# sujeetv/parquet-go

Hardware: AMD Instinct MI355X
Metric: decoded GB/s (uncompressed output) per GPU & node at 1/2/4/8; % HBM roofline (higher is better)
Workload: dtype int32; 1 GPU; C2: optional INT32, 100000000 rows x 7 dictionary widths (b=1,2,4,8,12,16,20), ~10% nulls, RLE_DICTIONARY (uniform indices), V1, UNCOMPRESSED, 20000 rows/page; bytes_in=821696760, bytes_out=3220121800, streams=2, parallelism=single GPU

## Files before the change

### parquet-go_amd/csrc/pqg_common.h

```cpp
#pragma once
#include <stdint.h>

#ifndef __HIPCC__
#ifndef __host__
#define __host__
#define __device__
#define __forceinline__ inline
#endif
#endif

namespace pqg {

enum : int32_t {
  kOK = 0,
  kEOF = -1,
  kTHRIFT = -2,
  kPAGE_HEADER = -3,
  kSIZE = -4,
  kSNAPPY = -5,
  kRLE = -6,
  kDICT_INDEX = -7,
  kBIT_WIDTH = -8,
  kDELTA = -9,
  kUNSUPPORTED = -10,
  kDICT_PAGE = -11,
  kBYTE_ARRAY = -12,
  kLEVELS = -13,
  kFIXED_LEN = -14,
  kGZIP = -15,
  kCAPACITY = -20,
  kCOMPLEX = -30,
};

struct PageHdr {
  int32_t type, usize, csize;
  int32_t num_values, encoding, def_enc, rep_enc;
  int32_t v2_def_len, v2_rep_len;
  int32_t has_dph, has_dict, has_v2;
  int32_t hlen;
};

struct PageDev {
  int64_t header_offset;
  int64_t payload_offset;
  int64_t slot_offset;
  int64_t value_offset;
  int64_t scratch_offset;
  const uint8_t* block;
  int64_t block_len;
  const uint8_t* rep;  int64_t rep_n;
  const uint8_t* def;  int64_t def_n;
  const uint8_t* val;  int64_t val_n;
  int32_t page_type, encoding, num_values, csize, usize;
  int32_t def_len, rep_len, def_enc, rep_enc;
  int32_t job;
  int32_t read_status;
  int32_t decode_status;
  int32_t not_null;
  int32_t flags;
  int32_t dict_width;
  int32_t hs_rep, hs_def, hs_val;
  int32_t vmode;
  int64_t run_off, blk_off;
  int64_t chars;
  int64_t char_offset;
  int64_t cstart;
  int32_t sn_hdr, sn_nsub, sn_sub_base, sn_nseg, sn_seg_base, sn_fallback;
  int64_t gz_len;
};
constexpr int32_t kPageBareBlock = 1 << 4;
constexpr int32_t kPageInflateRedo = 1 << 6;
constexpr int32_t kCodecSnappy = 1, kCodecGzip = 2;

constexpr int kSnapSub = 65536;
constexpr int kSnapSeg = 4096;
struct SnapSub {
  int32_t page;
  int32_t j;
  int32_t pos;
  int32_t out;
};

struct HStream {
  const uint8_t* p;
  int64_t n;
  int64_t run_base;
  int64_t blk_base;
  int32_t page;
  int32_t kind;
  int32_t w;
  int32_t count;
  int32_t n_runs;
  int32_t produced;
  int32_t status;
  int32_t n_blocks;
};

struct BlockDesc {
  uint32_t v0;
  uint32_t r0;
  uint32_t lo;
  uint16_t nbytes;
  uint16_t nr;
};

struct RunEnt {
  uint32_t start;
  uint32_t src;
};
constexpr uint32_t kRunBP = 0x80000000u;
constexpr int kHBlock = 512;
constexpr int kHBlockRuns = 64;
constexpr int kHBlockBytes = 1008;

struct VRec {
  uint8_t* out;
  const uint8_t* p;
  const RunEnt* runs;
  const BlockDesc* blks;
  const uint8_t* dict;
  int32_t n;
  int32_t w;
  int32_t nn;
  int32_t count;
  int32_t n_blocks;
  int32_t dcount;
  int32_t job;
  int32_t pidx;
  int32_t serr;
  int32_t produced;
};

struct JobDev {
  const uint8_t* data;
  int64_t data_len, tcs, data_page_offset;
  int32_t type, type_length, max_def, max_rep, codec, has_dict_off;
  int32_t value_width;
  int32_t page_cap;
  int64_t page_base;
  int64_t slot_cap, slot_base;
  int64_t value_cap, value_base;
  int64_t scratch_cap, scratch_base;
  int64_t offs_cap, offs_base;
  int32_t num_pages;
  int32_t dict_page;
  int32_t scan_status;
  int32_t status;
  int32_t error_page;
  int32_t n_out_pages;
  int64_t num_slots, num_values, values_bytes;
  int64_t need_scratch;
  const uint8_t* dict_data;
  int64_t dict_count, dict_len;
  const int64_t* dict_offs;
  int32_t flags;
  int32_t no_prewalk;
  int64_t doffs_cap, doffs_base;
  int64_t need_doffs;
  int64_t tile_base;
  int32_t n_tiles;
  int32_t scan_fallback;
  int32_t n_cands;
  int32_t n_ok;
  int32_t brk;
  int32_t first_dict;
  int64_t run_cap, run_base;
  int64_t blk_cap, blk_base;
  int64_t run_used, blk_used;
  int64_t item_base;
  int32_t n_items, pad2;
};

constexpr int kSplitMin = 65536;
constexpr int kPart = 4096;
constexpr int kLongLev = 32768;
constexpr int kLevPiece = 16384;
constexpr int kLongWalk = 16384;
constexpr int kCtrItems = 48;
constexpr int kCtrLongLev = 49;
constexpr int kCtrLevPieces = 50;
constexpr int kCtrLongWalk = 51;
constexpr int kCtrPartsCap = 52;

struct PartRec {
  int32_t pidx;
  int32_t p, np;
  uint32_t v0;
  int32_t b0;
  int32_t vmode;
  int64_t chars;
  int64_t cstart;
  int64_t prel;
};

struct LongLev {
  uint8_t* out;
  const uint8_t* p;
  const uint8_t* end;
  uint32_t count;
  uint32_t value;
  int32_t w;
  int32_t maxl;
  int32_t pidx;
  int32_t pad;
};
struct LevPiece {
  int32_t run;
  uint32_t v0, v1;
};

struct LongWalk {
  int64_t blk;
  uint32_t v0;
  uint32_t take;
  uint32_t run;
  uint32_t src;
  int32_t w, K;
};

#ifndef PQG_WALK_THREADS
#define PQG_WALK_THREADS 64
#endif
constexpr int kWalkThreads = PQG_WALK_THREADS;
#ifndef PQG_PW_THREADS
#define PQG_PW_THREADS 256
#endif
constexpr int kPwThreads = PQG_PW_THREADS;

constexpr int kQShards = 8;
constexpr int kQStride = 32;
constexpr int kQueueInts = kQShards * kQStride;
constexpr int kModePresentOff = 1024 + 9 * kQueueInts;
constexpr int kQueueSnapSerial = 10;
constexpr int kQueueStrDelta = 11;
constexpr int kQueueStrDba = 12;
constexpr int kQueueLevLong = 13;
constexpr int kQueueInflate = 14;
constexpr int kQueueLevGen = 15;
constexpr int kQueueDictBig = 16;
constexpr int kQueueInflateRedo = 17;
constexpr int kQueueSlots = 18;
constexpr int kPresentBigDict = 8;

constexpr int kScanTile = 16384;
constexpr int kPrewalkPages = 4;
constexpr int kCandPerTile = 64;

struct Cand {
  int64_t pos, next, payload;
  int64_t comp;
  int32_t type, encoding, num_values, csize, usize;
  int32_t def_len, rep_len, def_enc, rep_enc;
  int32_t status;
};

}
```

### parquet-go_amd/csrc/pqg_levels.hip

```cpp
#include <hip/hip_runtime.h>

#include "pqg_common.h"
#include "pqg_device.h"
#include "pqg_hybrid.h"
#include "pqg_levdec.h"
#include "pqg_lev1.h"
#include <type_traits>

namespace pqg {

#ifndef PQG_LEVELS_WPE
#define PQG_LEVELS_WPE 6
#endif

#ifdef PQG_PROFILE
int prof_read_levels(unsigned long long* out) {
  unsigned long long z[64] = {0};
  if (hipMemcpyFromSymbol(out, HIP_SYMBOL(pqg_prof), sizeof(z)) != hipSuccess) return -1;
  hipMemcpyToSymbol(HIP_SYMBOL(pqg_prof), z, sizeof(z));
  return 0;
}
#endif


#ifndef PQG_LANE_WIN
#define PQG_LANE_WIN 8
#endif
constexpr int kLaneWinG = PQG_LANE_WIN;
struct LaneWin {
  gcu8 p;
  uint32_t n;
  uint32_t base;
  PQG_L uint32_t* r;
  __device__ __forceinline__ void fill(uint32_t pos) {
    const uint32_t mis = (uint32_t)((uintptr_t)(p + pos) & 15);
    base = pos - mis;
    const uintptr_t a0 = (uintptr_t)(p + pos) - mis;
    const uintptr_t last = ((uintptr_t)(p + n) - 1) & ~(uintptr_t)15;
    uint4 g[kLaneWinG];
#pragma unroll
    for (int k = 0; k < kLaneWinG; k++) {
      const uintptr_t a = a0 + 16 * k;
      g[k] = ldg16(a <= last ? a : last);
    }
#pragma unroll
    for (int k = 0; k < kLaneWinG; k++) {
      const uint4 v = mask_tail(g[k], (int64_t)pos - mis + 16 * k, n);
      r[64 * (4 * k + 0)] = v.x;
      r[64 * (4 * k + 1)] = v.y;
      r[64 * (4 * k + 2)] = v.z;
      r[64 * (4 * k + 3)] = v.w;
    }
  }
  __device__ __forceinline__ void ensure(uint32_t pos) {
    if (pos - base > 16 * kLaneWinG - 16) fill(pos);
  }
  __device__ __forceinline__ void read12(uint32_t pos, uint32_t& a, uint32_t& b, uint32_t& c) const {
    const uint32_t off = pos - base;
    const uint32_t d = off >> 2, sh = (off & 3) * 8;
    const uint32_t x0 = r[64 * d], x1 = r[64 * (d + 1)], x2 = r[64 * (d + 2)], x3 = r[64 * (d + 3)];
    a = __builtin_amdgcn_alignbit(x1, x0, sh);
    b = __builtin_amdgcn_alignbit(x2, x1, sh);
    c = __builtin_amdgcn_alignbit(x3, x2, sh);
  }
  __device__ __forceinline__ void peek12(uint32_t pos, uint32_t& a, uint32_t& b, uint32_t& c) {
    ensure(pos);
    read12(pos, a, b, c);
  }
};

__device__ __forceinline__ void sync_ensure(LaneWin& w, bool reads, uint32_t rp) {
  const bool need = reads && rp - w.base > 16 * kLaneWinG - 16;
  if (__ballot(need) != 0 && reads) w.fill(rp);
}

__global__ void __launch_bounds__(kWalkThreads) k_hybrid_walk(const PageDev* pages, const int* list, const int* total,
                                                              HStream* streams, RunEnt* runs, BlockDesc* blks,
                                                              LongWalk* longs, int long_cap) {
  static_assert(kWalkThreads == 64, "LaneWin: dword k of lane L at buf[64 k + L]");
  __shared__ uint32_t buf[4 * kLaneWinG * kWalkThreads];
  const int nt = *total;
  int* const n_long = const_cast<int*>(total) + kCtrLongWalk;
  for (int g = blockIdx.x * kWalkThreads + threadIdx.x; g < nt; g += gridDim.x * kWalkThreads) {
    const PageDev& pg = pages[list[g]];
    const int hs = pg.hs_val;
    if (hs < 0) continue;
    HStream& S = streams[hs];
    const uint32_t w = (uint32_t)S.w;
    const uint32_t n = (uint32_t)S.n, count = (uint32_t)S.count;
    const uint32_t rb = (w + 7) >> 3;
    const uint64_t vmask = rb >= 4 ? 0xffffffffull : ((1ull << (8 * rb)) - 1);
    PQG_G uint32_t* R = (PQG_G uint32_t*)(gmut(runs) + S.run_base);
    PQG_G uint32_t* B = (PQG_G uint32_t*)(gmut(blks) + S.blk_base);
    LaneWin rd{gconst(S.p), n, 0xfffffff0u, lds_ptr(buf) + threadIdx.x};
    if (n > 0) rd.fill(0);
    uint32_t pos = 0, produced = 0, nr = 0;
    int status = kOK;
    uint32_t nb = 0, bv0 = 0, br0 = 0, bn = 0;
    uint64_t blo = ~0ull, bhi = 0;
    auto close_block = [&]() {
      if (bn == 0) return;
      const uint32_t lo = blo == ~0ull ? 0u : (uint32_t)blo;
      const uint32_t nbytes = blo == ~0ull ? 0u : (uint32_t)(bhi - blo);
      PQG_G uint32_t* d = B + 4 * nb;
      stg16((uintptr_t)d, make_uint4(bv0, br0, lo, (nbytes & 0xffff) | (bn << 16)));
      nb++;
    };
    while (produced < count) {
      if (pos >= n) { status = kEOF; break; }
      sync_ensure(rd, true, pos);
      uint32_t xa, xb, xc;
      rd.read12(pos, xa, xb, xc);
      uint64_t x = (uint64_t)xa | (uint64_t)xb << 32;
      uint32_t h, hl;
      if ((x & 0x80) == 0) {
        h = (uint32_t)x & 0x7f;
        hl = 1;
      } else {
        uint64_t v = 0;
        unsigned sft = 0;
        int e = kOK;
        hl = 0;
        for (uint32_t i = 0;; i++) {
          if (pos + i >= n) { e = kEOF; break; }
          uint32_t b;
          if (i < 8) {
            b = (uint32_t)(x >> (8 * i)) & 0xff;
          } else {
            uint32_t ya, yb, yc;
            rd.peek12(pos + i, ya, yb, yc);
            b = ya & 0xff;
          }
          if (b < 0x80) {
            if (i > 9 || (i == 9 && b > 1)) e = kRLE;
            else {
              v |= sft < 64 ? (uint64_t)b << sft : 0;
              if (v > 0x7fffffffull) e = kRLE;
            }
            hl = i + 1;
            break;
          }
          if (sft < 64) v |= (uint64_t)(b & 0x7f) << sft;
          sft += 7;
        }
        if (e) { status = e; break; }
        h = (uint32_t)v;
        {
          uint32_t ya, yb, yc;
          rd.peek12(pos + hl, ya, yb, yc);
          x = ((uint64_t)ya | (uint64_t)yb << 32) << 8;
        }
      }
      pos += hl;
      uint32_t take, st, src;
      const uint32_t left = count - produced;
      if (h & 1) {
        const uint32_t groups = h >> 1;
        if (groups == 0) { status = kRLE; break; }
        take = groups >= (left + 7) >> 3 ? left : groups * 8;
        const uint32_t need = (take + 7) >> 3;
        if ((uint64_t)pos + (uint64_t)(need - 1) * w >= n) {
          const uint32_t ok = pos < n ? (n - pos + w - 1) / w : 0;
          take = ok * 8;
          status = kEOF;
        }
        st = produced | kRunBP;
        src = pos;
        pos = (uint64_t)pos + (uint64_t)groups * w > 0xffffffffull ? 0xffffffffu : pos + groups * w;
      } else {
        const uint32_t cnt = h >> 1;
        if (cnt == 0) { status = kRLE; break; }
        if (pos >= n || n - pos < rb) { status = kEOF; break; }
        src = (uint32_t)((x >> 8) & vmask);
        pos += rb;
        if (w < 32 && (src >> w) != 0) { status = kRLE; break; }
        take = cnt < left ? cnt : left;
        st = produced;
      }
      if (take > 0) {
        stg8((uintptr_t)(R + 2 * nr), st, src);
        const uint32_t rend = produced + take;
        if ((st & kRunBP) && take > (uint32_t)kLongWalk) {
          const uint32_t K = min((uint32_t)kHBlock, ((8u * kHBlockBytes - 14u) / w) & ~7u);
          const uint32_t R = (take + K - 1) / K;
          const int li = atomicAdd(n_long, 1);
          if (li < long_cap) {
            close_block();
            LongWalk L;
            L.blk = S.blk_base + nb;
            L.v0 = produced;
            L.take = take;
            L.run = nr;
            L.src = src;
            L.w = (int32_t)w;
            L.K = (int32_t)K;
            longs[li] = L;
            nb += R;
            bv0 = rend;
            br0 = nr + 1;
            bn = 0;
            blo = ~0ull;
            bhi = 0;
            produced = rend;
            nr++;
            if (status) break;
            continue;
          }
        }
        for (uint32_t v = produced; v < rend;) {
          if (bn == kHBlockRuns || v >= bv0 + kHBlock) {
            close_block();
            bv0 = v;
            br0 = nr;
            bn = 0;
            blo = ~0ull;
            bhi = 0;
          }
          uint32_t pe = rend < bv0 + kHBlock ? rend : bv0 + kHBlock;
          if (st & kRunBP) {
            const uint64_t rbit = (uint64_t)src * 8;
            const uint64_t b0 = (rbit + (uint64_t)(v - produced) * w) >> 3;
            const uint64_t org = blo < b0 ? blo : b0;
            const uint64_t lim = (org + kHBlockBytes) * 8;
            const uint64_t fit = lim > rbit ? (lim - rbit) / w : 0;
            if (produced + fit <= v) {
              close_block();
              bv0 = v;
              br0 = nr;
              bn = 0;
              blo = ~0ull;
              bhi = 0;
              continue;
            }
            if (produced + fit < pe) pe = (uint32_t)(produced + fit);
            const uint64_t b1 = (rbit + (uint64_t)(pe - produced) * w + 7) >> 3;
            blo = org;
            bhi = b1 > bhi ? b1 : bhi;
          }
          bn++;
          v = pe;
        }
        produced = rend;
        nr++;
      }
      if (status) break;
    }
    close_block();
    S.n_runs = (int32_t)nr;
    S.produced = (int32_t)produced;
    S.status = status;
    S.n_blocks = (int32_t)nb;
  }
}

__global__ void __launch_bounds__(256) k_walk_long(const int* ctr, const LongWalk* longs, int long_cap,
                                                   BlockDesc* blks) {
  const int n = min(ctr[kCtrLongWalk], long_cap);
  const uint32_t tid = blockIdx.x * 256 + threadIdx.x, stride = gridDim.x * 256;
  for (int r = 0; r < n; r++) {
    const LongWalk L = longs[r];
    const uint32_t R = (L.take + (uint32_t)L.K - 1) / (uint32_t)L.K;
    for (uint32_t j = tid; j < R; j += stride) {
      const uint32_t a = j * (uint32_t)L.K;
      const uint32_t cnt = min((uint32_t)L.K, L.take - a);
      const uint64_t bit0 = (uint64_t)L.src * 8 + (uint64_t)a * (uint32_t)L.w;
      const uint64_t lo = bit0 >> 3, hi = (bit0 + (uint64_t)cnt * (uint32_t)L.w + 7) >> 3;
      stg16((uintptr_t)(blks + L.blk + j),
            make_uint4(L.v0 + a, L.run, (uint32_t)lo, (uint32_t)(hi - lo) | (1u << 16)));
    }
  }
}

__global__ void __launch_bounds__(64) k_level_long(PageDev* pages, const int* ctr, const LongLev* longs, int long_cap,
                                                   const LevPiece* pieces, int piece_cap, int* queue) {
  const int lane = lane_id();
  const int np = min(ctr[kCtrLevPieces], piece_cap);
  for (;;) {
    const int t = queue_next(queue);
    if (t >= np) return;
    const LevPiece pc = pieces[t];
    if (pc.run < 0 || pc.run >= long_cap) continue;
    const LongLev L = longs[pc.run];
    if (pages[L.pidx].decode_status != kOK) continue;
    const uintptr_t ob = (uintptr_t)L.out;
    const uint32_t mask = (1u << L.w) - 1;
    const int64_t navail = L.p ? (int64_t)(L.end - L.p) : 0;
    uint32_t nn = 0;
    const uintptr_t a0 = (ob + pc.v0) & ~(uintptr_t)15;
    for (uintptr_t a = a0 + 16 * (uintptr_t)lane; a < ob + pc.v1; a += 1024) {
      const int64_t i0 = (int64_t)(a - ob);
      uint32_t v[16];
      if (L.p) {
        const int64_t ib = i0 < 0 ? 0 : i0;
        const int64_t bit = ib * L.w;
        const gcu8 p = gconst(L.p);
        const uint64_t x0 = load_u64_masked(p, navail, bit >> 3, navail);
        const uint64_t x1 = load_u64_masked(p, navail, (bit >> 3) + 8, navail);
        const uint32_t sh = (uint32_t)(bit & 7);
        const int64_t shift0 = (i0 < 0 ? -i0 : 0) * L.w;
#pragma unroll
        for (int k = 0; k < 16; k++) {
          const int64_t b = (int64_t)sh + (int64_t)k * L.w - shift0;
          uint32_t x = 0;
          if (b >= 0) {
            x = b < 64 ? (uint32_t)(x0 >> b) | (b > 56 ? (uint32_t)(x1 << (64 - b)) : 0u) : (uint32_t)(x1 >> (b - 64));
          }
          v[k] = x & mask;
        }
      } else {
#pragma unroll
        for (int k = 0; k < 16; k++) v[k] = L.value;
      }
      uint32_t wv[4];
#pragma unroll
      for (int k = 0; k < 4; k++) wv[k] = v[4 * k] | v[4 * k + 1] << 8 | v[4 * k + 2] << 16 | v[4 * k + 3] << 24;
      if (i0 >= (int64_t)pc.v0 && i0 + 16 <= (int64_t)pc.v1) {
        stg16o(a, make_uint4(wv[0], wv[1], wv[2], wv[3]));
#pragma unroll
        for (int k = 0; k < 16; k++) nn += v[k] == (uint32_t)L.maxl;
      } else {
#pragma unroll
        for (int k = 0; k < 16; k++) {
          if (i0 + k >= (int64_t)pc.v0 && i0 + k < (int64_t)pc.v1) {
            *(PQG_G uint8_t*)(a + k) = (uint8_t)v[k];
            nn += v[k] == (uint32_t)L.maxl;
          }
        }
      }
    }
    const int64_t tot = wave_sum((int64_t)nn);
    if (lane == 0 && L.maxl <= 255 && tot) atomicAdd(&pages[L.pidx].not_null, (int32_t)tot);
  }
}

__device__ __forceinline__ bool w1_job(const JobDev& job) { return job.max_rep == 0 && job.max_def <= 1; }

union LevW1Shared {
  LevShared lev;
  Lev1Shared l1;
};
template <bool kW1>
using LevelsShared = typename std::conditional<kW1, LevW1Shared, LevShared>::type;
__device__ __forceinline__ LevShared& lev_sh(LevShared& s) { return s; }
__device__ __forceinline__ LevShared& lev_sh(LevW1Shared& s) { return s.lev; }

template <bool kW1>
__device__ __forceinline__ void page_levels(JobDev* jobs, PageDev* pages, const int* list, const int* total, int* queue,
                                            uint8_t* scratch, HStream* streams, uint8_t* def_arena, uint8_t* rep_arena,
                                            LongLev* longs, int long_cap, LevPiece* pieces, int piece_cap, int split_flags) {
  __shared__ __attribute__((aligned(16))) LevelsShared<kW1> shu;
  LevShared& sh = lev_sh(shu);
  const int split = split_flags & 1;
  const bool whole = kW1 && (split_flags & 2);
  const int lane = lane_id();
  const LongTables lt{longs, pieces, const_cast<int*>(total), long_cap, piece_cap};
  for (;;) {
    const int t = queue_next(queue);
    if (t >= *total) return;
    const int pidx = __builtin_amdgcn_readfirstlane(list[t]);
    const PageDev pg = pages[pidx];
    const JobDev job = jobs[pg.job];
    if (split && w1_job(job) != kW1) continue;
    if (lane == 0) {
      pages[pidx].hs_rep = pages[pidx].hs_def = pages[pidx].hs_val = -1;
      pages[pidx].vmode = -1;
    }
    if (pg.read_status != kOK || (pg.page_type != 0 && pg.page_type != 3)) continue;
    if (job.status == kCAPACITY) continue;
    const PageStreams ps = page_setup(job, pg, pidx, pages, streams, total, scratch, lane == 0);
    if (ps.e != kOK) continue;
    const int64_t n = pg.num_values;
    int64_t nn = 0;
    int de = kOK;
    if (n > 0) {
      if (!kW1 && job.max_rep > 0) {
        if (ps.rep_n < 0) de = kLEVELS;
        else {
          uint32_t unused;
          de = level_stream<kW1>(ps.rep, ps.rep_n, bits_len((uint32_t)job.max_rep), (uint32_t)n,
                                 gmut(rep_arena) + job.slot_base + pg.slot_offset, 0x100u, sh, &unused, lt, pidx);
        }
      }
      if (de == kOK) {
        if (job.max_def > 0) {
          if (ps.def_n < 0) de = kLEVELS;
          else {
            uint32_t c = 0;
            bool done = false;
            if constexpr (kW1) {
              if (whole && job.max_def == 1 && ps.def_n <= kL1MaxN)
                done = lev1_page(ps.def, (uint32_t)ps.def_n, (uint32_t)n,
                                 gmut(def_arena) + job.slot_base + pg.slot_offset, shu.l1, &c);
            }
            if (done) de = kOK;
            else
              de = level_stream<kW1>(ps.def, ps.def_n, bits_len((uint32_t)job.max_def), (uint32_t)n,
                                     gmut(def_arena) + job.slot_base + pg.slot_offset, (uint32_t)job.max_def, sh, &c,
                                     lt, pidx);
            nn = c;
          }
        } else {
          nn = n;
        }
      }
    }
    if (lane == 0) {
      pages[pidx].not_null = de == kOK ? (int32_t)nn : 0;
      if (de != kOK) pages[pidx].decode_status = de;
    }
  }
}

__global__ void __launch_bounds__(64, PQG_LEVELS_WPE) k_page_levels(JobDev* jobs, PageDev* pages, const int* list, const int* total,
                                                    int* queue, uint8_t* scratch, HStream* streams,
                                                    uint8_t* def_arena, uint8_t* rep_arena, LongLev* longs,
                                                    int long_cap, LevPiece* pieces, int piece_cap, int split) {
  page_levels<false>(jobs, pages, list, total, queue, scratch, streams, def_arena, rep_arena, longs, long_cap, pieces,
                     piece_cap, split);
}

#ifndef PQG_LEVELS_W1_WPE
#define PQG_LEVELS_W1_WPE 4
#endif
__global__ void __launch_bounds__(64, PQG_LEVELS_W1_WPE) k_page_levels_w1(JobDev* jobs, PageDev* pages, const int* list,
                                                       const int* total, int* queue, uint8_t* scratch,
                                                       HStream* streams, uint8_t* def_arena, uint8_t* rep_arena,
                                                       LongLev* longs, int long_cap, LevPiece* pieces, int piece_cap,
                                                       int split) {
  page_levels<true>(jobs, pages, list, total, queue, scratch, streams, def_arena, rep_arena, longs, long_cap, pieces,
                    piece_cap, split);
}

__device__ void plan_parts(JobDev& job, int np, bool fail, const PageDev* pp, const HStream* streams,
                           const BlockDesc* blks, int* ctr, PartRec* parts, int64_t cap, int64_t* part);

__device__ void resolve_dictionary(JobDev& job, PageDev* pages, uint8_t* scratch) {
  int np = job.num_pages < job.page_cap ? job.num_pages : job.page_cap;
  if (job.status == kCAPACITY) np = 0;
  if (job.dict_page < 0 || job.dict_page >= np) return;
  PageDev& dp = pages[job.page_base + job.dict_page];
  if (dp.read_status != kOK) return;
  const uint8_t* blk =
      dp.scratch_offset >= 0 ? scratch + job.scratch_base + dp.scratch_offset : job.data + dp.payload_offset;
  const int64_t blen = dp.usize;
  const int64_t cnt = dp.num_values;
  const int w = job.value_width;
  dp.block = blk;
  dp.block_len = blen;
  int st = kOK;
  int flags = 0;
  if (w > 0) {
    if (job.type == 3) {
      const int64_t full = blen / 12, rem = blen % 12;
      if (cnt > full + (rem > 0 ? 1 : 0)) st = kEOF;
      else if (cnt == full + 1 && rem > 0) flags = 1;
    } else if (cnt * w > blen) {
      st = kEOF;
    }
  } else {
    flags = 2;
    job.need_doffs = (cnt < blen / 4 ? cnt : blen / 4) + 2;
    if (job.need_doffs > job.doffs_cap) job.status = kCAPACITY;
  }
  if (st == kOK) {
    job.flags |= flags;
    job.dict_data = blk;
    job.dict_count = (flags & 2) ? 0 : cnt;
    job.dict_len = blen;
  } else {
    dp.read_status = st;
  }
}

__global__ void __launch_bounds__(256) k_dict_resolve(JobDev* jobs, int n_jobs, PageDev* pages, uint8_t* scratch) {
  const int j = blockIdx.x * 256 + threadIdx.x;
  if (j < n_jobs) resolve_dictionary(jobs[j], pages, scratch);
}

__device__ int nn_job_tail(JobDev& job, PageDev* pages, uint8_t* scratch, int np, int64_t carry, bool fail0) {
  int cap = fail0 || job.status == kCAPACITY;
  job.num_values = carry;
  const int64_t vb = job.value_width > 0 ? carry * job.value_width : 0;
  if (job.value_width > 0 && vb > job.value_cap) job.status = kCAPACITY, cap = 1;
  job.values_bytes = vb;
  return cap;
}

__device__ int64_t part_n(const PageDev& pg, const HStream* streams, int64_t* count, bool* hyb);
__device__ void plan_split_pages(JobDev& job, const PageDev* pp, const HStream* streams, const BlockDesc* blks,
                                 PartRec* parts, int64_t base, int nbig, const int* big, const int64_t* boff);
__device__ void plan_parts_from(JobDev& job, int np, const PageDev* pp, const HStream* streams, const BlockDesc* blks,
                                PartRec* parts, int64_t base);

constexpr int kNnFastSeg = 12;

__global__ void __launch_bounds__(1024) k_nn_scan(JobDev* jobs, PageDev* pages, uint8_t* scratch,
                                                  const HStream* streams, const BlockDesc* blks, int* ctr,
                                                  PartRec* parts, int64_t parts_cap) {
  __shared__ int64_t part[17];
  __shared__ int s_cap;
  JobDev& job = jobs[blockIdx.x];
  int np = job.num_pages < job.page_cap ? job.num_pages : job.page_cap;
  if (job.status == kCAPACITY) np = 0;
  if (np <= kNnFastSeg * 1024) {
    __shared__ int64_t s_base, s_res;
    __shared__ int s_big[256];
    __shared__ int64_t s_boff[256];
    __shared__ int s_nbig;
    const int seg = (np + 1023) / 1024;
    const int s0 = (int)threadIdx.x * seg;
    PageDev* pp = pages + job.page_base;
    int32_t nnv[kNnFastSeg], kv[kNnFastSeg];
    int8_t vm[kNnFastSeg];
    int64_t nsum = 0, ksum = 0;
    int32_t f_type[kNnFastSeg], f_nn[kNnFastSeg], f_rs[kNnFastSeg], f_ds[kNnFastSeg], f_enc[kNnFastSeg];
#pragma unroll
    for (int j = 0; j < kNnFastSeg; j++) {
      const int i = np > 0 ? (s0 + j < np ? s0 + j : np - 1) : 0;
      const PageDev& pg = pp[i];
      f_type[j] = pg.page_type;
      f_nn[j] = pg.not_null;
      f_rs[j] = pg.read_status;
      f_ds[j] = pg.decode_status;
      f_enc[j] = pg.encoding;
      vm[j] = (int8_t)pg.vmode;
    }
#pragma unroll
    for (int j = 0; j < kNnFastSeg; j++) {
      nnv[j] = kv[j] = 0;
      if (j < seg && s0 + j < np) {
        const bool data = f_type[j] == 0 || f_type[j] == 3;
        nnv[j] = data ? f_nn[j] : 0;
        int32_t k = 0;
        if (!data || vm[j] < 0) k = 0;
        else if (f_rs[j] != kOK || f_ds[j] != kOK || vm[j] == 3) k = 1;
        else if (vm[j] == 2 && f_enc[j] != 0 && f_enc[j] != 8) k = 1;
        else if (f_nn[j] <= kSplitMin) k = 1;
        else {
          int64_t c;
          bool h;
          k = (int32_t)part_n(pp[s0 + j], streams, &c, &h);
        }
        kv[j] = k;
      }
      nsum += nnv[j];
      ksum += kv[j];
    }
    int64_t carry, ktot;
    int64_t run = block_excl_scan<1024>(nsum, &carry, part);
    int64_t koff = block_excl_scan<1024>(ksum, &ktot, part);
    const bool fail0 = job.status == kCAPACITY;
    if (threadIdx.x == 0) {
      int cap = nn_job_tail(job, pages, scratch, np, carry, fail0);
      int64_t base = 0;
      if (!cap) {
        base = atomicAdd(ctr + kCtrItems, (int)ktot);
        if (base + ktot > parts_cap) {
          job.status = kCAPACITY;
          cap = 1;
        }
      }
      job.item_base = base;
      job.n_items = cap ? 0 : (int32_t)ktot;
      s_base = base;
      s_cap = cap;
      s_nbig = 0;
      s_res = fail0 ? 0 : ktot;
      if (blockIdx.x == 0) ctr[kCtrPartsCap] = (int)(parts_cap < INT32_MAX ? parts_cap : INT32_MAX);
    }
    __syncthreads();
    if (s_cap) {
      for (int64_t k = s_base + threadIdx.x; k < s_base + s_res && k < parts_cap; k += 1024) parts[k].vmode = -1;
    }
#pragma unroll
    for (int j = 0; j < kNnFastSeg; j++)
      if (j < seg && s0 + j < np) {
        pp[s0 + j].value_offset = run;
        run += nnv[j];
      }
    if (s_cap) return;
    const int64_t base = s_base;
    bool more = false;
#pragma unroll
    for (int j = 0; j < kNnFastSeg; j++) {
      if (j < seg && s0 + j < np) {
        if (kv[j] == 1) {
          PartRec r;
          r.pidx = (int32_t)(job.page_base + s0 + j);
          r.p = 0;
          r.np = 1;
          r.v0 = 0;
          r.b0 = 0;
          r.vmode = vm[j];
          r.chars = r.cstart = r.prel = 0;
          parts[base + koff] = r;
        } else if (kv[j] > 1) {
          const int slot = atomicAdd(&s_nbig, 1);
          if (slot < 256) {
            s_big[slot] = s0 + j;
            s_boff[slot] = koff;
          } else {
            more = true;
          }
        }
        koff += kv[j];
      }
    }
    const bool any_more = __syncthreads_or(more);
    const int nbig = s_nbig < 256 ? s_nbig : 256;
    if (!any_more) {
      plan_split_pages(job, pp, streams, blks, parts, base, nbig, s_big, s_boff);
      return;
    }
    __syncthreads();
    plan_parts_from(job, np, pp, streams, blks, parts, base);
    return;
  }
  const int seg = (np + 1023) / 1024;
  const int s0 = (int)threadIdx.x * seg, s1 = s0 + seg < np ? s0 + seg : np;
  PageDev* pp = pages + job.page_base;
  auto nn_of = [&](int i) -> int64_t {
    const PageDev& pg = pp[i];
    return (pg.page_type == 0 || pg.page_type == 3) ? (int64_t)pg.not_null : 0;
  };
  int64_t sum = 0;
#pragma unroll 8
  for (int i = s0; i < s1; i++) sum += nn_of(i);
  int64_t carry;
  int64_t run = block_excl_scan<1024>(sum, &carry, part);
#pragma unroll 8
  for (int i = s0; i < s1; i++) {
    pp[i].value_offset = run;
    run += nn_of(i);
  }
  const bool fail0 = job.status == kCAPACITY;
  if (threadIdx.x == 0) s_cap = nn_job_tail(job, pages, scratch, np, carry, fail0);
  __syncthreads();
  plan_parts(job, np, s_cap != 0, pp, streams, blks, ctr, parts, parts_cap, part);
}

}

namespace pqg {

__device__ __forceinline__ int64_t part_count(const PageDev& pg, const HStream* streams, bool* hyb) {
  *hyb = false;
  if ((pg.page_type != 0 && pg.page_type != 3) || pg.vmode < 0) return -1;
  if (pg.read_status != kOK || pg.decode_status != kOK || pg.vmode == 3) return 0;
  const int enc = pg.encoding;
  if (pg.vmode == 2 && enc != 0 && enc != 8) return 0;
  const int64_t nn = pg.not_null;
  if (enc == 0 || nn <= kSplitMin) return nn;
  if ((enc == 8 || enc == 3) && pg.hs_val >= 0) {
    const HStream& S = streams[pg.hs_val];
    *hyb = true;
    return nn < S.produced ? nn : S.produced;
  }
  return 0;
}

__device__ int64_t part_n(const PageDev& pg, const HStream* streams, int64_t* count, bool* hyb) {
  const int64_t c = part_count(pg, streams, hyb);
  *count = c;
  if (c < 0) return 0;
  return c > kSplitMin ? (c + kPart - 1) / kPart : 1;
}

__device__ void plan_split_pages(JobDev& job, const PageDev* pp, const HStream* streams, const BlockDesc* blks,
                                 PartRec* parts, int64_t base, int nbig, const int* big, const int64_t* boff) {
  for (int q = 0; q < nbig; q++) {
    const int pi = big[q];
    const int64_t poff = boff[q];
    int64_t cnt;
    bool hyb;
    const PageDev& pg = pp[pi];
    const int64_t P = part_n(pg, streams, &cnt, &hyb);
    PartRec r;
    r.pidx = (int32_t)(job.page_base + pi);
    r.np = (int32_t)P;
    r.vmode = pg.vmode;
    r.chars = r.cstart = r.prel = 0;
    if (!hyb) {
      for (int64_t p = threadIdx.x; p < P; p += blockDim.x) {
        r.p = (int32_t)p;
        r.v0 = (uint32_t)(p * kPart);
        r.b0 = 0;
        parts[base + poff + p] = r;
      }
    } else {
      const HStream& S = streams[pg.hs_val];
      const BlockDesc* B = blks + S.blk_base;
      const int nb = S.n_blocks;
      auto f = [&](int bi) -> int64_t {
        if (bi < 0) return -1;
        if (bi >= nb || (int64_t)B[bi].v0 >= cnt) return P;
        return (int64_t)B[bi].v0 / kPart;
      };
      for (int bi = threadIdx.x; bi <= nb; bi += blockDim.x) {
        const int64_t f1 = f(bi), f0 = f(bi - 1);
        for (int64_t p = f0 + 1; p <= f1 && p < P; p++) {
          r.p = (int32_t)p;
          r.v0 = p == 0 ? 0u : (bi < nb && (int64_t)B[bi].v0 < cnt ? B[bi].v0 : (uint32_t)cnt);
          r.b0 = bi;
          parts[base + poff + p] = r;
        }
      }
    }
  }
}

constexpr int kBigList = 256;
__device__ void plan_parts_from(JobDev& job, int np, const PageDev* pp, const HStream* streams, const BlockDesc* blks,
                                PartRec* parts, int64_t base) {
  __shared__ int64_t part2[17];
  __shared__ int s_big[kBigList];
  __shared__ int64_t s_boff[kBigList];
  __shared__ int s_nbig;
  const int seg = (np + 1023) / 1024;
  const int s0 = (int)threadIdx.x * seg, s1 = s0 + seg < np ? s0 + seg : np;
  int64_t sum = 0;
  for (int i = s0; i < s1; i++) {
    int64_t c;
    bool h;
    sum += part_n(pp[i], streams, &c, &h);
  }
  int64_t tot;
  int64_t off = block_excl_scan<1024>(sum, &tot, part2);
  int cur = s0;
  for (;;) {
    if (threadIdx.x == 0) s_nbig = 0;
    __syncthreads();
    for (; cur < s1; cur++) {
      int64_t c;
      bool h;
      const int64_t k = part_n(pp[cur], streams, &c, &h);
      if (k == 1) {
        PartRec r;
        r.pidx = (int32_t)(job.page_base + cur);
        r.p = 0;
        r.np = 1;
        r.v0 = 0;
        r.b0 = 0;
        r.vmode = pp[cur].vmode;
        r.chars = r.cstart = r.prel = 0;
        parts[base + off] = r;
      } else if (k > 1) {
        const int slot = atomicAdd(&s_nbig, 1);
        if (slot >= kBigList) break;
        s_big[slot] = cur;
        s_boff[slot] = off;
      }
      off += k;
    }
    __syncthreads();
    plan_split_pages(job, pp, streams, blks, parts, base, s_nbig < kBigList ? s_nbig : kBigList, s_big, s_boff);
    if (!__syncthreads_or(cur < s1)) break;
  }
}

__device__ void plan_parts(JobDev& job, int np, bool fail, const PageDev* pp, const HStream* streams,
                           const BlockDesc* blks, int* ctr, PartRec* parts, int64_t cap, int64_t* part) {
  __shared__ int64_t s_base;
  __shared__ int s_fail;
  if (fail) np = 0;
  const int seg = (np + 1023) / 1024;
  const int s0 = (int)threadIdx.x * seg, s1 = s0 + seg < np ? s0 + seg : np;
  int64_t sum = 0;
  for (int i = s0; i < s1; i++) {
    int64_t c;
    bool h;
    sum += part_n(pp[i], streams, &c, &h);
  }
  int64_t tot;
  block_excl_scan<1024>(sum, &tot, part);
  if (threadIdx.x == 0) {
    const int64_t base = fail ? 0 : atomicAdd(ctr + kCtrItems, (int)tot);
    s_fail = fail || base + tot > cap;
    if (!fail && s_fail) job.status = kCAPACITY;
    job.item_base = base;
    job.n_items = s_fail ? 0 : (int32_t)tot;
    s_base = base;
    if (blockIdx.x == 0) ctr[kCtrPartsCap] = (int)(cap < INT32_MAX ? cap : INT32_MAX);
  }
  __syncthreads();
  if (s_fail) {
    if (!fail)
      for (int64_t k = s_base + threadIdx.x; k < s_base + tot && k < cap; k += 1024) parts[k].vmode = -1;
    return;
  }
  plan_parts_from(job, np, pp, streams, blks, parts, s_base);
}

}
```

### parquet-go_amd/csrc/pqg_runtime.hip

```cpp
#include <hip/hip_runtime.h>
#include <cstdlib>

#include <algorithm>
#include <cstdio>
#include <map>
#include <cstring>
#include <mutex>
#include <vector>

#include "../../include/pqgpu.h"
#include "pqg_common.h"

namespace pqg {
int assemble_launch(hipStream_t s, const pqg_assemble_args* a, int64_t* seg_scratch, int64_t* tot);
int list_count_launch(hipStream_t s, const pqg_list_args* a, int64_t* seg_scratch, int64_t* tot);
int list_write_launch(hipStream_t s, const pqg_list_args* a, int64_t* seg_scratch);
int pack_levels_launch(hipStream_t s, const uint8_t* levels, int64_t n, int bw, uint8_t* packed);
}

namespace pqg {
__global__ void k_tile_jobs(const JobDev* jobs, int* tile_job);
__global__ void k_page_cands(JobDev* jobs, const int* tile_job, int* tile_count, int* tile_okc, int64_t* cand_pos,
                             int* cand_list, int* cand_total, int region);
__global__ void k_cand_parse(JobDev* jobs, const int* tile_job, const int* cand_list, const int* cand_total, int region,
                             int* tile_okc,
                             const int64_t* cand_pos, Cand* cands);
__global__ void k_tile_scan(JobDev* jobs, const int* tile_count, const int* tile_okc, int* tile_off, int* tile_okoff);
__global__ void k_cand_link(JobDev* jobs, const int* tile_job, int64_t total_tiles, const int* tile_count,
                            const int* tile_off, const int* tile_okoff, const Cand* cands, int* succ, int* idx2slot,
                            int* ok2slot);
__global__ void k_page_chain(JobDev* jobs, PageDev* pages, const Cand* cands, const int* succ,
                             const int* idx2slot, const int* ok2slot, int* order);
__global__ void k_scan_pages(JobDev* jobs, PageDev* pages, int n_jobs, int prewalk, int stride);
__global__ void k_page_list(JobDev* jobs, PageDev* pages, int n_jobs, int* list, int list_cap, int* total,
                            int* queues);
__global__ void k_snappy(JobDev* jobs, PageDev* pages, const int* list, const int* total, int* queue,
                         uint8_t* scratch);
__global__ void k_inflate(JobDev* jobs, PageDev* pages, const int* list, const int* total, int* queue,
                          uint8_t* scratch, int mode);
__global__ void k_inflate_s(JobDev* jobs, PageDev* pages, const int* list, const int* total, int* queue,
                            uint8_t* scratch);
__global__ void k_snap_plan(const JobDev* jobs, PageDev* pages, const int* list, const int* total, int* ctr,
                            SnapSub* subs, int sub_cap, int* seg_page, int seg_cap);
__global__ void k_snap_seg(const JobDev* jobs, const PageDev* pages, const int* seg_page, const int* seg_total,
                           int seg_cap, uint2* F);
__global__ void k_snap_link(const JobDev* jobs, PageDev* pages, const int* list, const int* total, SnapSub* subs,
                            const uint2* F);
__global__ void k_snap_decode(const JobDev* jobs, PageDev* pages, const SnapSub* subs, const int* sub_total,
                              int sub_cap, int* queue, uint8_t* scratch);
__global__ void k_page_levels(JobDev* jobs, PageDev* pages, const int* list, const int* total, int* queue,
                              uint8_t* scratch, HStream* streams, uint8_t* def_arena, uint8_t* rep_arena,
                              LongLev* longs, int long_cap, LevPiece* pieces, int piece_cap, int split);
__global__ void k_page_levels_w1(JobDev* jobs, PageDev* pages, const int* list, const int* total, int* queue,
                              uint8_t* scratch, HStream* streams, uint8_t* def_arena, uint8_t* rep_arena,
                              LongLev* longs, int long_cap, LevPiece* pieces, int piece_cap, int split);
__global__ void k_dict_resolve(JobDev* jobs, int n_jobs, PageDev* pages, uint8_t* scratch);
__global__ void k_level_long(PageDev* pages, const int* ctr, const LongLev* longs, int long_cap,
                             const LevPiece* pieces, int piece_cap, int* queue);
__global__ void k_hybrid_walk(const PageDev* pages, const int* list, const int* total, HStream* streams,
                              RunEnt* runs, BlockDesc* blks, LongWalk* longs, int long_cap);
__global__ void k_walk_long(const int* ctr, const LongWalk* longs, int long_cap, BlockDesc* blks);
__global__ void k_nn_scan(JobDev* jobs, PageDev* pages, uint8_t* scratch, const HStream* streams, const BlockDesc* blks,
                          int* ctr, PartRec* parts, int64_t parts_cap);
template <int Mode>
__global__ void k_values(JobDev* jobs, PageDev* pages, const PartRec* parts, const int* total, int* queue,
                         uint8_t* value_arena, const HStream* streams, const RunEnt* runs, const BlockDesc* blks);
__global__ void k_dict_plan(JobDev* jobs, PageDev* pages, const PartRec* parts, const int* total,
                            uint8_t* value_arena, const HStream* streams, const RunEnt* runs, const BlockDesc* blks,
                            VRec* recs);
__global__ void k_dict4(PageDev* pages, const int* total, int* queue, const VRec* recs, int big);
__global__ void k_dict4_big(PageDev* pages, const int* total, int* queue, const VRec* recs);
constexpr int kBigDictThreads = 512;
__global__ void k_finalize(JobDev* jobs, int n_jobs, PageDev* pages);
__global__ void k_str_dict(JobDev* jobs, PageDev* pages, int64_t* doffs_arena);
__global__ void k_str_count(JobDev* jobs, PageDev* pages, PartRec* parts, const int* total, int* queue,
                            int64_t* offs_arena, const HStream* streams, const RunEnt* runs, const BlockDesc* blks);
__global__ void k_str_plain(JobDev* jobs, PageDev* pages, const int* list, const int* total, int* queue,
                            int64_t* offs_arena);
__global__ void k_char_scan(JobDev* jobs, PageDev* pages, PartRec* parts, int64_t* offs_arena);
__global__ void k_str_delta(JobDev* jobs, PageDev* pages, const int* list, const int* total, int* queue,
                            int64_t* offs_arena);
__global__ void k_str_dba(JobDev* jobs, PageDev* pages, const int* list, const int* total, int* queue,
                          uint8_t* value_arena, int64_t* offs_arena);
__global__ void k_str_copy(JobDev* jobs, PageDev* pages, const PartRec* parts, const int* total, int* queue,
                           uint8_t* value_arena, int64_t* offs_arena);
}

#ifdef PQG_PROFILE
namespace pqg {
int prof_read_values(unsigned long long* out);
int prof_read_levels(unsigned long long* out);
int prof_read_strings(unsigned long long* out);
int prof_read_snappy(unsigned long long* out);
int prof_read_dict(unsigned long long* out);
int prof_read_inflate(unsigned long long* out);
}
#endif

using namespace pqg;

namespace {

struct DevBuf {
  void* p = nullptr;
  size_t cap = 0;
  int grow(size_t bytes) {
    if (bytes <= cap) return 0;
    if (p) hipFree(p);
    p = nullptr;
    cap = 0;
    size_t want = std::max(bytes, (size_t)256);
    want = (want + 0xFFFFF) & ~(size_t)0xFFFFF;
    if (hipMalloc(&p, want) != hipSuccess) {
      p = nullptr;
      return -1;
    }
    cap = want;
    return 0;
  }
  void release() {
    if (p) hipFree(p);
    p = nullptr;
    cap = 0;
  }
};

constexpr int kStages = 10;
constexpr int kWalkLanes = kWalkThreads;
constexpr int kMaxAttempts = 6;

struct Caps {
  int64_t pages = 0, slots = 0, scratch = 0, values = 0, runs = 0, blks = 0, doffs = 0;
};
struct JobKey {
  uintptr_t data;
  int64_t tcs, hint;
  bool operator<(const JobKey& o) const {
    return data != o.data ? data < o.data : tcs != o.tcs ? tcs < o.tcs : hint < o.hint;
  }
};

int64_t align_up(int64_t v, int64_t a) { return (v + a - 1) / a * a; }

unsigned qgrid(int64_t blocks) { return (unsigned)std::max<int64_t>(blocks, kQShards); }

int value_width_of(const pqg_column_desc& c) {
  switch (c.physical_type) {
    case PQG_BOOLEAN: return 1;
    case PQG_INT32: case PQG_FLOAT: return 4;
    case PQG_INT64: case PQG_DOUBLE: return 8;
    case PQG_INT96: return 12;
    case PQG_FIXED_LEN_BYTE_ARRAY: return c.type_length > 0 ? c.type_length : 0;
  }
  return 0;
}

}

struct pqg_ctx {
  int device = 0;
  hipStream_t stream = nullptr;
  int num_cus = 256;
  DevBuf vrecs;
  int dict4_per_cu = 2;
  int dict4_threads = 256;
  bool dict4 = true;
  bool stride = true;
  bool dict_big = true;
  bool lev1 = true;
  int seg_waves = 31;
  int levlong_waves = 28;
  int link_waves = 16;
  int snappy_per_cu = 2;
  int inflate_per_cu = 8;
  DevBuf jobs, pages, list, counters, def_arena, rep_arena, value_arena, scratch;
  DevBuf tile_job;
  DevBuf tile_count, tile_okc, tile_off, tile_okoff, cand_pos, cands, succ, idx2slot, ok2slot, order;
  DevBuf streams, runs, blks;
  DevBuf cand_list, vlists;
  DevBuf asm_seg;
  DevBuf offs_arena, doffs_arena;
  DevBuf page_stage;
  DevBuf blk_src, blk_dst, blk_meta, blk_subs, blk_segpage, blk_F;
  DevBuf sn_subs, sn_segpage, sn_F;
  int64_t sn_sub_cap = 0, sn_seg_cap = 0;
  DevBuf parts, lev_long, lev_pieces, walk_long;
  int64_t parts_cap = 0, lev_long_cap = 0, lev_piece_cap = 0, walk_long_cap = 0;
  int64_t total_tiles = 0;
  JobDev* h_jobs = nullptr;
  int h_jobs_cap = 0;
  std::vector<pqg_chunk_job> cur;
  std::vector<JobDev> plan;
  std::vector<Caps> force;
  std::map<JobKey, Caps> learned;
  std::map<JobKey, bool> many_pages;
  bool prewalk = true;
  int launches = 0;
  bool any_var = false;
  bool any_fixed_other = false;
  bool any_w4 = false;
  bool any_levels = false;
  int n_jobs = 0;
  int64_t list_cap = 0;
  hipEvent_t ev[kStages + 1];
  hipEvent_t ev_k8[4];
  float k8_ms = 0.f;
  bool timed = true;
  bool last_timed = false;
};

static int hip_ok(hipError_t e) { return e == hipSuccess ? PQG_OK : PQG_ERR_HIP; }

extern "C" {

const char* pqg_status_string(int s) {
  switch (s) {
    case PQG_OK: return "ok";
    case PQG_ERR_EOF: return "unexpected end of stream";
    case PQG_ERR_THRIFT: return "page header: thrift decode failed";
    case PQG_ERR_PAGE_HEADER: return "page header: missing or negative field";
    case PQG_ERR_SIZE: return "page size mismatch";
    case PQG_ERR_SNAPPY: return "snappy: corrupt input";
    case PQG_ERR_RLE: return "rle: invalid run";
    case PQG_ERR_DICT_INDEX: return "dict: invalid index";
    case PQG_ERR_BIT_WIDTH: return "invalid bit width";
    case PQG_ERR_DELTA: return "delta: invalid stream";
    case PQG_ERR_UNSUPPORTED: return "unsupported encoding/codec/type";
    case PQG_ERR_DICT_PAGE: return "there should be only one dictionary";
    case PQG_ERR_BYTE_ARRAY: return "bytearray/plain: len is negative";
    case PQG_ERR_LEVELS: return "level reader is not initialized";
    case PQG_ERR_FIXED_LEN: return "bytearray/delta: value length is not the fixed length";
    case PQG_ERR_GZIP: return "gzip: invalid data";
    case PQG_ERR_CAPACITY: return "capacity";
    case PQG_ERR_INVALID_ARG: return "invalid argument";
    case PQG_ERR_HIP: return "HIP runtime error";
    case PQG_ERR_METADATA: return "invalid file metadata";
  }
  return "unknown";
}

int pqg_ctx_create(int device, pqg_ctx** out) {
  if (!out) return PQG_ERR_INVALID_ARG;
  *out = nullptr;
  int n = 0;
  if (hipGetDeviceCount(&n) != hipSuccess || device < 0 || device >= n) return PQG_ERR_HIP;
  if (hipSetDevice(device) != hipSuccess) return PQG_ERR_HIP;
  pqg_ctx* c = new pqg_ctx();
  c->device = device;
  hipDeviceProp_t prop;
  if (hipGetDeviceProperties(&prop, device) == hipSuccess) c->num_cus = prop.multiProcessorCount;
  if (hipStreamCreateWithFlags(&c->stream, hipStreamNonBlocking) != hipSuccess) {
    delete c;
    return PQG_ERR_HIP;
  }
  for (auto& e : c->ev) hipEventCreate(&e);
  for (auto& e : c->ev_k8) hipEventCreate(&e);
  if (const char* e = getenv("PQG_DICT4")) c->dict4 = atoi(e) != 0;
  if (const char* e = getenv("PQG_DICT_BIG")) c->dict_big = atoi(e) != 0;
  if (const char* e = getenv("PQG_STRIDE")) c->stride = atoi(e) != 0;
  if (const char* e = getenv("PQG_LEV1")) c->lev1 = atoi(e) != 0;
  if (const char* e = getenv("PQG_SEG_WAVES")) c->seg_waves = atoi(e) > 0 ? atoi(e) : c->seg_waves;
  if (const char* e = getenv("PQG_LEVLONG_WAVES")) c->levlong_waves = atoi(e) > 0 ? atoi(e) : c->levlong_waves;
  if (const char* e = getenv("PQG_LINK_WAVES")) c->link_waves = atoi(e) > 0 ? atoi(e) : c->link_waves;
  {
    hipFuncAttributes fa;
    if (hipFuncGetAttributes(&fa, reinterpret_cast<const void*>(&k_dict4)) == hipSuccess && fa.maxThreadsPerBlock > 0)
      c->dict4_threads = fa.maxThreadsPerBlock;
    int o = 0;
    if (hipOccupancyMaxActiveBlocksPerMultiprocessor(&o, reinterpret_cast<const void*>(&k_dict4), c->dict4_threads, 0) ==
            hipSuccess && o > 0)
      c->dict4_per_cu = o;
  }
  int occ = 0;
  if (hipOccupancyMaxActiveBlocksPerMultiprocessor(&occ, reinterpret_cast<const void*>(&k_snappy), 64, 0) ==
          hipSuccess &&
      occ > 0)
    c->snappy_per_cu = occ;
  occ = 0;
  if (hipOccupancyMaxActiveBlocksPerMultiprocessor(&occ, reinterpret_cast<const void*>(&k_inflate_s), 64, 0) ==
          hipSuccess && occ > 0)
    c->inflate_per_cu = occ;
  if (c->counters.grow(sizeof(int) * (size_t)(1024 + kQueueSlots * kQueueInts))) {
    pqg_ctx_destroy(c);
    return PQG_ERR_HIP;
  }
  *out = c;
  return PQG_OK;
}

void pqg_ctx_destroy(pqg_ctx* c) {
  if (!c) return;
  hipSetDevice(c->device);
  hipStreamSynchronize(c->stream);
  for (auto& e : c->ev) hipEventDestroy(e);
  for (auto& e : c->ev_k8) hipEventDestroy(e);
  for (DevBuf* b : {&c->jobs, &c->pages, &c->list, &c->counters, &c->def_arena, &c->rep_arena, &c->value_arena,
                    &c->scratch, &c->streams, &c->runs, &c->blks, &c->cand_list, &c->vlists, &c->tile_count, &c->tile_okc, &c->tile_off, &c->tile_okoff, &c->cand_pos, &c->cands, &c->succ, &c->idx2slot,
                    &c->ok2slot, &c->order, &c->asm_seg, &c->offs_arena, &c->doffs_arena, &c->page_stage,
                    &c->blk_src, &c->blk_dst, &c->blk_meta, &c->tile_job, &c->sn_subs, &c->sn_segpage, &c->sn_F,
                    &c->blk_subs, &c->blk_segpage, &c->blk_F, &c->vrecs, &c->parts, &c->lev_long, &c->lev_pieces,
                    &c->walk_long})
    b->release();
  if (c->h_jobs) hipHostFree(c->h_jobs);
  hipStreamDestroy(c->stream);
  delete c;
}

int pqg_device_alloc(pqg_ctx* c, int64_t bytes, void** dptr) {
  if (!c || !dptr) return PQG_ERR_INVALID_ARG;
  hipSetDevice(c->device);
  return hip_ok(hipMalloc(dptr, (size_t)std::max<int64_t>(bytes, 1)));
}
int pqg_device_free(pqg_ctx* c, void* dptr) {
  if (!c) return PQG_ERR_INVALID_ARG;
  hipSetDevice(c->device);
  return hip_ok(hipFree(dptr));
}
int pqg_memcpy_h2d(pqg_ctx* c, void* dst, const void* src, int64_t bytes) {
  if (!c) return PQG_ERR_INVALID_ARG;
  hipSetDevice(c->device);
  int e = hip_ok(hipMemcpyAsync(dst, src, (size_t)bytes, hipMemcpyHostToDevice, c->stream));
  if (e) return e;
  return hip_ok(hipStreamSynchronize(c->stream));
}
int pqg_memcpy_d2h(pqg_ctx* c, void* dst, const void* src, int64_t bytes) {
  if (!c) return PQG_ERR_INVALID_ARG;
  hipSetDevice(c->device);
  int e = hip_ok(hipMemcpyAsync(dst, src, (size_t)bytes, hipMemcpyDeviceToHost, c->stream));
  if (e) return e;
  return hip_ok(hipStreamSynchronize(c->stream));
}

static int plan_batch(pqg_ctx* c) {
  const int n = c->n_jobs;
  if (c->h_jobs_cap < n) {
    if (c->h_jobs) hipHostFree(c->h_jobs);
    c->h_jobs_cap = std::max(n, 64);
    if (hipHostMalloc((void**)&c->h_jobs, sizeof(JobDev) * (size_t)c->h_jobs_cap) != hipSuccess) return PQG_ERR_HIP;
  }
  int64_t page_total = 0, slot_total = 0, value_total = 0, scratch_total = 0, tile_total = 0, run_total = 0,
          blk_total = 0, offs_total = 0, doffs_total = 0, seg_total = 0;
  c->plan.resize((size_t)n);
  for (int i = 0; i < n; i++) {
    const pqg_chunk_job& in = c->cur[(size_t)i];
    const Caps& f = c->force[(size_t)i];
    JobDev d;
    memset(&d, 0, sizeof(d));
    d.data = in.data;
    d.data_len = in.data_len;
    d.tcs = in.total_compressed_size;
    d.data_page_offset = in.data_page_offset;
    d.type = in.col.physical_type;
    d.type_length = in.col.type_length;
    d.max_def = in.col.max_def;
    d.max_rep = in.col.max_rep;
    d.codec = in.col.codec;
    d.has_dict_off = in.has_dict_page_offset;
    d.value_width = value_width_of(in.col);
    d.no_prewalk = c->many_pages.count(JobKey{(uintptr_t)in.data, in.total_compressed_size, in.num_values_hint}) ? 1 : 0;
    int64_t pcap = in.total_compressed_size / 256 + 16;
    if (f.pages > 0) pcap = f.pages;
    pcap = std::min<int64_t>(pcap, (int64_t)1 << 30);
    d.page_cap = (int32_t)pcap;
    d.page_base = page_total;
    page_total += pcap;
    int64_t scap = std::max<int64_t>(in.num_values_hint, 0) + 64;
    if (f.slots > 0) scap = f.slots;
    d.slot_cap = scap;
    d.slot_base = slot_total;
    slot_total += align_up(scap, 256);
    int64_t vcap = d.value_width > 0 ? scap * d.value_width
                                     : std::max<int64_t>(in.total_uncompressed_size, in.total_compressed_size) + 1024;
    if (f.values > 0) vcap = f.values;
    d.value_cap = vcap;
    d.value_base = value_total;
    value_total += align_up(vcap, 256);
    int64_t xcap = 0;
    if (in.col.codec != PQG_CODEC_UNCOMPRESSED)
      xcap = std::max<int64_t>(in.total_uncompressed_size, in.total_compressed_size) + pcap * 16 + 1024;
    if (f.scratch > 0) xcap = f.scratch;
    d.scratch_cap = xcap;
    d.scratch_base = scratch_total;
    scratch_total += align_up(xcap, 256);
    if (in.col.codec != PQG_CODEC_UNCOMPRESSED) seg_total += in.total_compressed_size / kSnapSeg + pcap;
    d.dict_page = -1;
    d.error_page = -1;
    const int64_t lim = std::max<int64_t>(0, std::min(in.total_compressed_size, in.data_len));
    int64_t rcap = (in.total_compressed_size + xcap) / 2 + 6 * pcap + 64;
    if (f.runs > 0) rcap = f.runs;
    d.run_cap = rcap;
    d.run_base = run_total;
    run_total += rcap;
    int64_t bcap = 3 * (scap / kHBlock + 3 * pcap) + rcap / kHBlockRuns + 2 * rcap / (kHBlockBytes / 2) + 64;
    if (f.blks > 0) bcap = f.blks;
    d.blk_cap = bcap;
    d.blk_base = blk_total;
    blk_total += bcap;
    if (d.value_width == 0 || d.type == PQG_FIXED_LEN_BYTE_ARRAY) {
      d.offs_cap = scap + 1;
      d.offs_base = offs_total;
      offs_total += align_up(scap + 1, 32);
    }
    if (d.value_width == 0) {
      int64_t dcap = std::min<int64_t>(std::max<int64_t>(in.total_uncompressed_size, 0) / 4, 1 << 17) + 64;
      if (f.doffs > 0) dcap = f.doffs;
      d.doffs_cap = dcap;
      d.doffs_base = doffs_total;
      doffs_total += align_up(dcap, 32);
    }
    d.tile_base = tile_total;
    d.n_tiles = (int32_t)((lim + kScanTile - 1) / kScanTile);
    tile_total += d.n_tiles;
    c->plan[(size_t)i] = d;
    c->h_jobs[i] = d;
  }
  c->list_cap = page_total;
  c->parts_cap = page_total + slot_total / kPart + n + 64;
  c->lev_long_cap = 2 * slot_total / kLongLev + 64;
  c->lev_piece_cap = 2 * slot_total / kLevPiece + 2 * c->lev_long_cap + 64;
  c->walk_long_cap = slot_total / kLongWalk + 64;
  if (c->parts.grow(sizeof(PartRec) * (size_t)c->parts_cap) || c->lev_long.grow(sizeof(LongLev) * (size_t)c->lev_long_cap) ||
      c->lev_pieces.grow(sizeof(LevPiece) * (size_t)c->lev_piece_cap) ||
      c->walk_long.grow(sizeof(LongWalk) * (size_t)c->walk_long_cap))
    return PQG_ERR_HIP;
  c->sn_sub_cap = scratch_total / kSnapSub + page_total + 64;
  c->sn_seg_cap = seg_total + 64;
  if (c->sn_subs.grow(sizeof(SnapSub) * (size_t)c->sn_sub_cap) || c->sn_segpage.grow(sizeof(int) * (size_t)c->sn_seg_cap) ||
      c->sn_F.grow(sizeof(uint2) * 64 * (size_t)c->sn_seg_cap))
    return PQG_ERR_HIP;
  if (c->jobs.grow(sizeof(JobDev) * (size_t)n) || c->pages.grow(sizeof(PageDev) * (size_t)page_total) ||
      c->list.grow(sizeof(int) * (size_t)std::max<int64_t>(page_total, 1)) || c->def_arena.grow((size_t)slot_total + 64) ||
      c->rep_arena.grow((size_t)slot_total + 64) || c->value_arena.grow((size_t)value_total + 64) ||
      c->scratch.grow((size_t)scratch_total + 64) || c->tile_count.grow(sizeof(int) * (size_t)tile_total + 64) ||
      c->tile_off.grow(sizeof(int) * (size_t)tile_total + 64) || c->tile_okc.grow(sizeof(int) * (size_t)tile_total + 64) ||
      c->tile_okoff.grow(sizeof(int) * (size_t)tile_total + 64) || c->tile_job.grow(sizeof(int) * (size_t)tile_total + 64) ||
      c->ok2slot.grow(sizeof(int) * (size_t)tile_total * kCandPerTile + 64) ||
      c->cand_pos.grow(sizeof(int64_t) * (size_t)tile_total * kCandPerTile + 64) ||
      c->cand_list.grow(sizeof(int) * (size_t)(tile_total + kQShards) * kCandPerTile + 64) ||
      c->vlists.grow(sizeof(int) * 3 * (size_t)page_total + 64) ||
      c->cands.grow(sizeof(Cand) * (size_t)tile_total * kCandPerTile + 64) ||
      c->succ.grow(sizeof(int) * (size_t)tile_total * kCandPerTile + 64) ||
      c->idx2slot.grow(sizeof(int) * (size_t)tile_total * kCandPerTile + 64) ||
      c->order.grow(sizeof(int) * (size_t)page_total + 64) ||
      c->streams.grow(sizeof(HStream) * 3 * (size_t)page_total + 64) ||
      c->runs.grow(sizeof(RunEnt) * (size_t)run_total + 8192) || c->blks.grow(sizeof(BlockDesc) * (size_t)blk_total + 8192) ||
      c->vrecs.grow(sizeof(VRec) * (size_t)std::max<int64_t>(c->parts_cap, 1)) ||
      c->offs_arena.grow(sizeof(int64_t) * (size_t)offs_total + 64) ||
      c->doffs_arena.grow(sizeof(int64_t) * (size_t)doffs_total + 64))
    return PQG_ERR_HIP;
  c->total_tiles = tile_total;
  return hip_ok(hipMemcpyAsync(c->jobs.p, c->h_jobs, sizeof(JobDev) * (size_t)n, hipMemcpyHostToDevice, c->stream));
}

struct SnapTables {
  SnapSub* subs;
  int sub_cap;
  int* segpage;
  int seg_cap;
  uint2* F;
};
static void launch_snappy(pqg_ctx* c, hipStream_t s, JobDev* jobs, PageDev* pages, const int* list, const int* total,
                          int64_t list_cap, int* sctr, int* q_split, int* q_serial, uint8_t* scratch,
                          const SnapTables& T) {
  const int waves = c->num_cus * c->snappy_per_cu;
  hipMemsetAsync(sctr, 0, 2 * sizeof(int), s);
  hipLaunchKernelGGL(k_snap_plan, dim3((unsigned)std::max<int64_t>(1, std::min<int64_t>((list_cap + 255) / 256, c->num_cus * 4))),
                     dim3(256), 0, s, jobs, pages, list, total, sctr, T.subs, T.sub_cap, T.segpage, T.seg_cap);
  hipLaunchKernelGGL(k_snap_seg, dim3(c->num_cus * c->seg_waves), dim3(64), 0, s, jobs, pages, T.segpage, sctr + 1, T.seg_cap, T.F);
  hipLaunchKernelGGL(k_snap_link, dim3(c->num_cus * c->link_waves), dim3(64), 0, s, jobs, pages, list, total, T.subs, T.F);
  hipLaunchKernelGGL(k_snap_decode, dim3(qgrid(waves)), dim3(64), 0, s, jobs, pages, T.subs, sctr, T.sub_cap, q_split,
                     scratch);
  hipLaunchKernelGGL(k_snappy, dim3(qgrid(waves)), dim3(64), 0, s, jobs, pages, list, total, q_serial, scratch);
}

static int launch_pipeline(pqg_ctx* c) {
  const int n = c->n_jobs;
  c->launches++;
  c->last_timed = c->timed;
  JobDev* jobs = (JobDev*)c->jobs.p;
  PageDev* pages = (PageDev*)c->pages.p;
  int* list = (int*)c->list.p;
  int* ctr = (int*)c->counters.p;
  auto Q = [&](int k) { return ctr + 1024 + k * kQueueInts; };
  uint8_t* scratch = (uint8_t*)c->scratch.p;
  const int waves = c->num_cus * 20;
  hipStream_t s = c->stream;
  if (c->timed) hipEventRecord(c->ev[0], s);
  hipMemsetAsync(Q(0), 0, sizeof(int) * kQueueSlots * kQueueInts, s);
  const int64_t nt = c->total_tiles;
  int* tcount = (int*)c->tile_count.p;
  int* toff = (int*)c->tile_off.p;
  Cand* cands = (Cand*)c->cands.p;
  int* tokc = (int*)c->tile_okc.p;
  int* tokoff = (int*)c->tile_okoff.p;
  if (c->prewalk) hipLaunchKernelGGL(k_scan_pages, dim3(n), dim3(64), 0, s, jobs, pages, n, kPrewalkPages, (int)c->stride);
  if (nt > 0) {
    int64_t* cpos = (int64_t*)c->cand_pos.p;
    int* clist = (int*)c->cand_list.p;
    const int region = (int)((nt + kQShards - 1) / kQShards) * kCandPerTile;
    hipLaunchKernelGGL(k_tile_jobs, dim3(n), dim3(256), 0, s, jobs, (int*)c->tile_job.p);
    hipLaunchKernelGGL(k_page_cands, dim3((unsigned)nt), dim3(256), 0, s, jobs, (const int*)c->tile_job.p, tcount, tokc,
                       cpos, clist, Q(7),
                       region);
    hipLaunchKernelGGL(k_cand_parse, dim3((unsigned)std::min<int64_t>((nt * kCandPerTile + 255) / 256, c->num_cus * 4)),
                       dim3(256), 0, s, jobs, (const int*)c->tile_job.p, clist, Q(7), region, tokc, cpos, cands);
  }
  hipLaunchKernelGGL(k_tile_scan, dim3(n), dim3(1024), 0, s, jobs, tcount, tokc, toff, tokoff);
  if (nt > 0)
    hipLaunchKernelGGL(k_cand_link, dim3((unsigned)((nt * kCandPerTile + 255) / 256)), dim3(256), 0, s, jobs,
                       (const int*)c->tile_job.p, nt,
                       tcount, toff, tokoff, cands, (int*)c->succ.p, (int*)c->idx2slot.p, (int*)c->ok2slot.p);
  hipLaunchKernelGGL(k_page_chain, dim3(n), dim3(1024), 0, s, jobs, pages, cands, (const int*)c->succ.p,
                     (const int*)c->idx2slot.p, (const int*)c->ok2slot.p, (int*)c->order.p);
  hipLaunchKernelGGL(k_scan_pages, dim3(n), dim3(64), 0, s, jobs, pages, n, 0, 0);
  if (c->timed) hipEventRecord(c->ev[1], s);
  hipLaunchKernelGGL(k_page_list, dim3(n), dim3(1024), 0, s, jobs, pages, n, list,
                     (int)std::min<int64_t>(c->list_cap, INT32_MAX), ctr, ctr + 8);
  if (c->timed) hipEventRecord(c->ev[2], s);
  bool any_snappy = false, any_gzip = false;
  for (int i = 0; i < n; i++) {
    any_snappy |= c->cur[(size_t)i].col.codec == PQG_CODEC_SNAPPY;
    any_gzip |= c->cur[(size_t)i].col.codec == PQG_CODEC_GZIP;
  }
  if (any_snappy) {
    const SnapTables T{(SnapSub*)c->sn_subs.p, (int)std::min<int64_t>(c->sn_sub_cap, INT32_MAX), (int*)c->sn_segpage.p,
                       (int)std::min<int64_t>(c->sn_seg_cap, INT32_MAX), (uint2*)c->sn_F.p};
    launch_snappy(c, s, jobs, pages, list, ctr, c->list_cap, ctr + 32, Q(0), Q(kQueueSnapSerial), scratch, T);
  }
  if (any_gzip) {
    hipLaunchKernelGGL(k_inflate_s, dim3(qgrid(c->num_cus * c->inflate_per_cu)), dim3(64), 0, s, jobs, pages, list, ctr,
                       Q(kQueueInflate), scratch);
    hipLaunchKernelGGL(k_inflate, dim3(qgrid(c->num_cus * 4)), dim3(64), 0, s, jobs, pages, list, ctr,
                       Q(kQueueInflateRedo), scratch, 1);
  }
  if (c->timed) hipEventRecord(c->ev[3], s);
  HStream* streams = (HStream*)c->streams.p;
  RunEnt* runs = (RunEnt*)c->runs.p;
  BlockDesc* blks = (BlockDesc*)c->blks.p;
  LongLev* llong = (LongLev*)c->lev_long.p;
  LevPiece* lpieces = (LevPiece*)c->lev_pieces.p;
  const int llc = (int)std::min<int64_t>(c->lev_long_cap, INT32_MAX), lpc = (int)std::min<int64_t>(c->lev_piece_cap, INT32_MAX);
  hipLaunchKernelGGL(k_dict_resolve, dim3((unsigned)((n + 255) / 256)), dim3(256), 0, s, jobs, n, pages, scratch);
  bool any_w1 = false, any_gen = false;
  for (int i = 0; i < n; i++) {
    const pqg_column_desc& d = c->cur[(size_t)i].col;
    (d.max_rep == 0 && d.max_def <= 1 ? any_w1 : any_gen) = true;
  }
  const int split = any_w1 && any_gen;
  if (any_w1)
    hipLaunchKernelGGL(k_page_levels_w1, dim3(qgrid(c->num_cus * 32)), dim3(64), 0, s, jobs, pages, list, ctr, Q(1),
                       scratch, streams, (uint8_t*)c->def_arena.p, (uint8_t*)c->rep_arena.p, llong, llc, lpieces, lpc,
                       split | (c->lev1 ? 2 : 0));
  if (any_gen)
    hipLaunchKernelGGL(k_page_levels, dim3(qgrid(c->num_cus * 24)), dim3(64), 0, s, jobs, pages, list, ctr,
                       Q(split ? kQueueLevGen : 1), scratch, streams, (uint8_t*)c->def_arena.p,
                       (uint8_t*)c->rep_arena.p, llong, llc, lpieces, lpc, split);
  if (c->any_levels)
    hipLaunchKernelGGL(k_level_long, dim3(qgrid(c->num_cus * c->levlong_waves)), dim3(64), 0, s, pages, ctr, llong, llc, lpieces, lpc,
                       Q(kQueueLevLong));
  if (c->timed) hipEventRecord(c->ev[4], s);
  const unsigned walk_blocks = (unsigned)std::max<int64_t>(
      1, std::min<int64_t>((c->list_cap + kWalkLanes - 1) / kWalkLanes, c->num_cus * (2048 / kWalkLanes)));
  LongWalk* wlong = (LongWalk*)c->walk_long.p;
  const int wlc = (int)std::min<int64_t>(c->walk_long_cap, INT32_MAX);
  hipLaunchKernelGGL(k_hybrid_walk, dim3(walk_blocks), dim3(kWalkLanes), 0, s, pages, list, ctr, streams, runs, blks,
                     wlong, wlc);
  hipLaunchKernelGGL(k_walk_long, dim3(c->num_cus * 2), dim3(256), 0, s, ctr, wlong, wlc, blks);
  if (c->timed) hipEventRecord(c->ev[5], s);
  if (c->timed) hipEventRecord(c->ev[6], s);
  PartRec* parts = (PartRec*)c->parts.p;
  hipLaunchKernelGGL(k_nn_scan, dim3(n), dim3(1024), 0, s, jobs, pages, scratch, streams, blks, ctr, parts, c->parts_cap);
  if (c->timed) hipEventRecord(c->ev[7], s);
  const int64_t items_cap = c->parts_cap;
  if (!c->any_w4) {
  } else if (c->dict4) {
    VRec* recs = (VRec*)c->vrecs.p;
    hipLaunchKernelGGL(k_dict_plan, dim3((unsigned)std::max<int64_t>(1, std::min<int64_t>((items_cap + 255) / 256, c->num_cus * 4))),
                       dim3(256), 0, s, jobs, pages, parts, ctr, (uint8_t*)c->value_arena.p, streams, runs, blks, recs);
    hipLaunchKernelGGL(k_dict4, dim3(qgrid(c->num_cus * c->dict4_per_cu)), dim3(c->dict4_threads), 0, s, pages, ctr, Q(3),
                       recs, (int)c->dict_big);
    if (c->dict_big)
      hipLaunchKernelGGL(k_dict4_big, dim3(qgrid(c->num_cus)), dim3(kBigDictThreads), 0, s, pages, ctr,
                         Q(kQueueDictBig), recs);
  } else
    hipLaunchKernelGGL(k_values<1>, dim3(qgrid(waves)), dim3(64), 0, s, jobs, pages, parts, ctr, Q(3),
                       (uint8_t*)c->value_arena.p, streams, runs, blks);
  if (c->any_fixed_other) {
    hipLaunchKernelGGL(k_values<0>, dim3(qgrid(waves)), dim3(64), 0, s, jobs, pages, parts, ctr, Q(2),
                       (uint8_t*)c->value_arena.p, streams, runs, blks);
    hipLaunchKernelGGL(k_values<3>, dim3(qgrid(waves)), dim3(64), 0, s, jobs, pages, parts, ctr, Q(8),
                       (uint8_t*)c->value_arena.p, streams, runs, blks);
  }
  if (c->timed) hipEventRecord(c->ev[8], s);
  if (c->any_var) {
    int64_t* offs = (int64_t*)c->offs_arena.p;
    hipLaunchKernelGGL(k_str_dict, dim3(n), dim3(512), 0, s, jobs, pages, (int64_t*)c->doffs_arena.p);
    hipLaunchKernelGGL(k_str_plain, dim3(qgrid(c->num_cus * 4 * 512 / kPwThreads)), dim3(kPwThreads), 0, s, jobs, pages, list, ctr, Q(5), offs);
    hipLaunchKernelGGL(k_str_count, dim3(qgrid(waves)), dim3(64), 0, s, jobs, pages, parts, ctr, Q(4), offs, streams,
                       runs, blks);
    hipLaunchKernelGGL(k_str_delta, dim3(qgrid(c->num_cus * 8)), dim3(64), 0, s, jobs, pages, list, ctr,
                       Q(kQueueStrDelta), offs);
    hipLaunchKernelGGL(k_char_scan, dim3(n), dim3(256), 0, s, jobs, pages, parts, offs);
    hipLaunchKernelGGL(k_str_copy, dim3(qgrid(c->num_cus * 4)), dim3(512), 0, s, jobs, pages, parts, ctr, Q(6),
                       (uint8_t*)c->value_arena.p, offs);
    hipLaunchKernelGGL(k_str_dba, dim3(qgrid(c->num_cus * 6)), dim3(64), 0, s, jobs, pages, list, ctr,
                       Q(kQueueStrDba), (uint8_t*)c->value_arena.p, offs);
  }
  if (c->timed) hipEventRecord(c->ev[9], s);
  hipLaunchKernelGGL(k_finalize, dim3(n), dim3(1024), 0, s, jobs, n, pages);
  if (c->timed) hipEventRecord(c->ev[10], s);
  return hip_ok(hipGetLastError());
}

int pqg_decode_chunks_async(pqg_ctx* c, const pqg_chunk_job* jobs, int n_jobs) {
  if (!c || (!jobs && n_jobs) || n_jobs < 0) return PQG_ERR_INVALID_ARG;
  hipSetDevice(c->device);
  for (int i = 0; i < n_jobs; i++) {
    const pqg_column_desc& d = jobs[i].col;
    if (d.max_def < 0 || d.max_def > 255 || d.max_rep < 0 || d.max_rep > 255) return PQG_ERR_INVALID_ARG;
    if (jobs[i].data_len < 0 || jobs[i].total_compressed_size < 0 || (!jobs[i].data && jobs[i].data_len > 0))
      return PQG_ERR_INVALID_ARG;
    if (jobs[i].quirks != 0) return PQG_ERR_INVALID_ARG;
  }
  c->cur.assign(jobs, jobs + n_jobs);
  c->n_jobs = n_jobs;
  c->launches = 0;
  c->force.assign((size_t)n_jobs, Caps());
  c->any_var = false;
  c->any_fixed_other = false;
  c->any_w4 = false;
  c->any_levels = false;
  c->prewalk = false;
  for (int i = 0; i < n_jobs; i++) {
    const JobKey key{(uintptr_t)jobs[i].data, jobs[i].total_compressed_size, jobs[i].num_values_hint};
    auto it = c->learned.find(key);
    if (it != c->learned.end()) c->force[(size_t)i] = it->second;
    c->prewalk |= c->many_pages.find(key) == c->many_pages.end();
    c->any_var |= value_width_of(jobs[i].col) == 0 || jobs[i].col.physical_type == PQG_FIXED_LEN_BYTE_ARRAY;
    c->any_fixed_other |= value_width_of(jobs[i].col) != 0;
    c->any_w4 |= value_width_of(jobs[i].col) == 4;
    c->any_levels |= jobs[i].col.max_def > 0 || jobs[i].col.max_rep > 0;
  }
  if (n_jobs == 0) return PQG_OK;
  int e = plan_batch(c);
  if (e) return e;
  return launch_pipeline(c);
}

int pqg_sync(pqg_ctx* c, pqg_chunk_result* results, int n_jobs) {
  if (!c || n_jobs != c->n_jobs) return PQG_ERR_INVALID_ARG;
  hipSetDevice(c->device);
  const int n = c->n_jobs;
  if (n == 0) return PQG_OK;
  for (int attempt = 0;; attempt++) {
    if (hipMemcpyAsync(c->h_jobs, c->jobs.p, sizeof(JobDev) * (size_t)n, hipMemcpyDeviceToHost, c->stream) !=
            hipSuccess ||
        hipStreamSynchronize(c->stream) != hipSuccess)
      return PQG_ERR_HIP;
    bool retry = false;
    for (int i = 0; i < n; i++) {
      const JobDev& d = c->h_jobs[i];
      if (d.status != PQG_ERR_CAPACITY) continue;
      retry = true;
      Caps& f = c->force[(size_t)i];
      f.pages = std::max<int64_t>((int64_t)d.num_pages + 16, d.page_cap);
      f.slots = std::max<int64_t>(d.num_slots + 64, d.slot_cap);
      f.scratch = std::max<int64_t>(d.need_scratch + 1024, d.scratch_cap);
      if (d.value_width > 0) {
        const int64_t nv = std::max<int64_t>(d.num_values, d.num_slots);
        f.values = std::max<int64_t>(nv * d.value_width + 64, d.value_cap);
      } else {
        f.values = std::max<int64_t>(d.values_bytes + 1024, d.value_cap);
      }
      f.runs = std::max<int64_t>(d.run_used + 64, d.run_cap);
      f.blks = std::max<int64_t>(d.blk_used + 64, d.blk_cap);
      f.doffs = std::max<int64_t>(d.need_doffs + 64, d.doffs_cap);
      const pqg_chunk_job& in = c->cur[(size_t)i];
      c->learned[JobKey{(uintptr_t)in.data, in.total_compressed_size, in.num_values_hint}] = f;
    }
    if (!retry || attempt + 1 >= kMaxAttempts) break;
    int e = plan_batch(c);
    if (e) return e;
    e = launch_pipeline(c);
    if (e) return e;
  }
  for (int i = 0; i < n; i++) {
    const JobDev& d = c->h_jobs[i];
    if (d.status != PQG_ERR_CAPACITY && d.scan_fallback != 2) {
      if (c->many_pages.size() >= 65536) c->many_pages.clear();
      const pqg_chunk_job& in = c->cur[(size_t)i];
      c->many_pages[JobKey{(uintptr_t)in.data, in.total_compressed_size, in.num_values_hint}] = true;
    }
    pqg_chunk_result& r = results[i];
    memset(&r, 0, sizeof(r));
    r.status = d.status;
    r.error_page = d.error_page;
    r.num_pages = d.status == PQG_ERR_CAPACITY ? 0 : d.n_out_pages;
    r.value_width = d.value_width;
    r.col_flags = c->cur[(size_t)i].col.flags;
    r.num_slots = d.num_slots;
    r.num_values = d.num_values;
    r.values_bytes = d.values_bytes;
    r.def_levels = d.max_def > 0 ? (uint8_t*)c->def_arena.p + d.slot_base : nullptr;
    r.rep_levels = d.max_rep > 0 ? (uint8_t*)c->rep_arena.p + d.slot_base : nullptr;
    r.values = (uint8_t*)c->value_arena.p + d.value_base;
    r.offsets = d.value_width == 0 ? (int64_t*)c->offs_arena.p + d.offs_base : nullptr;
  }
  return PQG_OK;
}

int pqg_assemble(pqg_ctx* c, pqg_assemble_args* a) {
  if (!c || !a || a->num_slots < 0 || a->max_def < 0 || a->max_def > 255 || a->boundary_level < 0)
    return PQG_ERR_INVALID_ARG;
  if (a->values_spaced && (a->value_width <= 0 || (!a->values && a->num_slots > 0))) return PQG_ERR_INVALID_ARG;
  hipSetDevice(c->device);
  const int64_t nseg = (a->num_slots + 4095) / 4096;
  if (c->asm_seg.grow((size_t)(2 * nseg + 2) * sizeof(int64_t))) return PQG_ERR_HIP;
  int64_t* seg = (int64_t*)c->asm_seg.p;
  int64_t* tot = seg + 2 * nseg;
  hipEventRecord(c->ev_k8[0], c->stream);
  int e = pqg::assemble_launch(c->stream, a, seg, tot);
  if (e) return e;
  hipEventRecord(c->ev_k8[1], c->stream);
  int64_t h[2] = {0, 0};
  if (hipMemcpyAsync(h, tot, sizeof(h), hipMemcpyDeviceToHost, c->stream) != hipSuccess ||
      hipStreamSynchronize(c->stream) != hipSuccess)
    return PQG_ERR_HIP;
  hipEventElapsedTime(&c->k8_ms, c->ev_k8[0], c->ev_k8[1]);
  a->num_valid = h[0];
  a->null_count = a->num_slots - h[0];
  a->num_boundaries = h[1];
  return PQG_OK;
}

int pqg_assemble_list(pqg_ctx* c, pqg_list_args* a) {
  if (!c || !a || a->num_slots < 0 || !a->def_levels || a->max_def < 0 || a->max_def > 255 || a->value_width < 0)
    return PQG_ERR_INVALID_ARG;
  if (a->elem_values && (a->value_width <= 0 || (!a->values && a->num_slots > 0))) return PQG_ERR_INVALID_ARG;
  hipSetDevice(c->device);
  const int64_t nseg = (a->num_slots + 4095) / 4096;
  if (c->asm_seg.grow((size_t)(4 * nseg + 4) * sizeof(int64_t))) return PQG_ERR_HIP;
  int64_t* seg = (int64_t*)c->asm_seg.p;
  int64_t* tot = seg + 4 * nseg;
  hipEventRecord(c->ev_k8[0], c->stream);
  int e = pqg::list_count_launch(c->stream, a, seg, tot);
  if (e) return e;
  hipEventRecord(c->ev_k8[1], c->stream);
  int64_t h[4] = {0, 0, 0, 0};
  if (hipMemcpyAsync(h, tot, sizeof(h), hipMemcpyDeviceToHost, c->stream) != hipSuccess ||
      hipStreamSynchronize(c->stream) != hipSuccess)
    return PQG_ERR_HIP;
  a->num_rows = h[0];
  a->num_elements = h[1];
  a->num_valid = h[2];
  a->null_lists = h[3];
  if (h[1] > INT32_MAX) return PQG_ERR_INVALID_ARG;
  hipEventRecord(c->ev_k8[2], c->stream);
  e = pqg::list_write_launch(c->stream, a, seg);
  if (e) return e;
  hipEventRecord(c->ev_k8[3], c->stream);
  e = hip_ok(hipStreamSynchronize(c->stream));
  float m0 = 0.f, m1 = 0.f;
  hipEventElapsedTime(&m0, c->ev_k8[0], c->ev_k8[1]);
  hipEventElapsedTime(&m1, c->ev_k8[2], c->ev_k8[3]);
  c->k8_ms = m0 + m1;
  return e;
}

int pqg_last_assemble_ms(pqg_ctx* c, float* ms) {
  if (!c || !ms) return PQG_ERR_INVALID_ARG;
  *ms = c->k8_ms;
  return PQG_OK;
}

int pqg_decode_chunks(pqg_ctx* c, const pqg_chunk_job* jobs, int n_jobs, pqg_chunk_result* results) {
  int e = pqg_decode_chunks_async(c, jobs, n_jobs);
  if (e) return e;
  return pqg_sync(c, results, n_jobs);
}

int pqg_decode_page(pqg_ctx* c, const pqg_page_job* pj, pqg_chunk_result* result) {
  if (!c || !pj || !result || !pj->page || pj->page_len <= 0 || pj->dict_page_len < 0 ||
      (pj->dict_page_len > 0 && !pj->dict_page))
    return PQG_ERR_INVALID_ARG;
  hipSetDevice(c->device);
  const int64_t dl = pj->dict_page ? pj->dict_page_len : 0, total = dl + pj->page_len;
  if (c->page_stage.grow((size_t)total + 64)) return PQG_ERR_HIP;
  uint8_t* st = (uint8_t*)c->page_stage.p;
  if ((dl && hipMemcpyAsync(st, pj->dict_page, (size_t)dl, hipMemcpyDeviceToDevice, c->stream) != hipSuccess) ||
      hipMemcpyAsync(st + dl, pj->page, (size_t)pj->page_len, hipMemcpyDeviceToDevice, c->stream) != hipSuccess)
    return PQG_ERR_HIP;
  pqg_chunk_job job;
  memset(&job, 0, sizeof(job));
  job.col = pj->col;
  job.data = st;
  job.data_len = total;
  job.total_compressed_size = total;
  job.data_page_offset = dl;
  job.total_uncompressed_size = total;
  return pqg_decode_chunks(c, &job, 1, result);
}

static int inflate_pass(pqg_ctx* c, int64_t n, int64_t store, PageDev* out) {
  if (c->blk_dst.grow((size_t)store + 64)) return PQG_ERR_HIP;
  JobDev jd;
  memset(&jd, 0, sizeof(jd));
  jd.data = (const uint8_t*)c->blk_src.p;
  jd.data_len = n;
  jd.tcs = n;
  jd.codec = PQG_CODEC_GZIP;
  jd.scratch_cap = store + 16;
  PageDev pd;
  memset(&pd, 0, sizeof(pd));
  pd.page_type = PQG_PAGE_DICTIONARY;
  pd.flags = kPageBareBlock;
  pd.csize = (int32_t)n;
  pd.usize = (int32_t)store;
  pd.read_status = kOK;
  uint8_t* meta = (uint8_t*)c->blk_meta.p;
  JobDev* djob = (JobDev*)meta;
  PageDev* dpage = (PageDev*)(meta + sizeof(JobDev));
  int* ints = (int*)(meta + sizeof(JobDev) + sizeof(PageDev));
  int hi[2] = {0, 1};
  if (hipMemcpyAsync(djob, &jd, sizeof(jd), hipMemcpyHostToDevice, c->stream) != hipSuccess ||
      hipMemcpyAsync(dpage, &pd, sizeof(pd), hipMemcpyHostToDevice, c->stream) != hipSuccess ||
      hipMemcpyAsync(ints, hi, sizeof(hi), hipMemcpyHostToDevice, c->stream) != hipSuccess ||
      hipMemsetAsync(ints + 4, 0, sizeof(int) * kQueueInts, c->stream) != hipSuccess)
    return PQG_ERR_HIP;
  hipLaunchKernelGGL(k_inflate, dim3(qgrid(1)), dim3(64), 0, c->stream, djob, dpage, ints, ints + 1, ints + 4,
                     (uint8_t*)c->blk_dst.p, 0);
  if (hipGetLastError() != hipSuccess) return PQG_ERR_HIP;
  if (hipMemcpyAsync(out, dpage, sizeof(PageDev), hipMemcpyDeviceToHost, c->stream) != hipSuccess ||
      hipStreamSynchronize(c->stream) != hipSuccess)
    return PQG_ERR_HIP;
  return PQG_OK;
}

static int block_inflate(pqg_ctx* c, const uint8_t* src, int64_t n, uint8_t* dst, int64_t cap, int64_t* out_len) {
  constexpr int64_t kInflateFirst = 64 << 20;
  hipSetDevice(c->device);
  if (c->blk_src.grow((size_t)n + 64) ||
      c->blk_meta.grow(sizeof(JobDev) + sizeof(PageDev) + (4 + 2 * kQueueInts) * sizeof(int)))
    return PQG_ERR_HIP;
  if (n && hipMemcpyAsync(c->blk_src.p, src, (size_t)n, hipMemcpyHostToDevice, c->stream) != hipSuccess)
    return PQG_ERR_HIP;
  int64_t store = std::min<int64_t>(std::max<int64_t>(cap, 0), kInflateFirst);
  PageDev pd;
  int e = inflate_pass(c, n, store, &pd);
  if (e) return e;
  if (pd.read_status != kOK) return pd.read_status;
  *out_len = pd.gz_len;
  if (pd.gz_len > cap) return PQG_ERR_CAPACITY;
  if (pd.gz_len > INT32_MAX) return PQG_ERR_UNSUPPORTED;
  if (pd.gz_len > store) {
    store = pd.gz_len;
    e = inflate_pass(c, n, store, &pd);
    if (e) return e;
    if (pd.read_status != kOK) return pd.read_status;
    if (pd.gz_len != store) return PQG_ERR_HIP;
  }
  if (pd.gz_len && (hipMemcpyAsync(dst, c->blk_dst.p, (size_t)pd.gz_len, hipMemcpyDeviceToHost, c->stream) != hipSuccess ||
                    hipStreamSynchronize(c->stream) != hipSuccess))
    return PQG_ERR_HIP;
  return PQG_OK;
}

int pqg_block_decompress(pqg_ctx* c, int codec, const uint8_t* src, int64_t n, uint8_t* dst, int64_t cap,
                         int64_t* out_len) {
  if (!c || (!src && n > 0) || n < 0 || n > INT32_MAX || !out_len) return PQG_ERR_INVALID_ARG;
  *out_len = 0;
  if (codec == PQG_CODEC_UNCOMPRESSED) {
    *out_len = n;
    if (n > cap) return PQG_ERR_CAPACITY;
    if (n) memcpy(dst, src, (size_t)n);
    return PQG_OK;
  }
  if (codec == PQG_CODEC_GZIP) return block_inflate(c, src, n, dst, cap, out_len);
  if (codec != PQG_CODEC_SNAPPY) return PQG_ERR_UNSUPPORTED;
  uint64_t v = 0;
  int hl = 0;
  for (unsigned sft = 0;; hl++, sft += 7) {
    if (hl >= n) return PQG_ERR_SNAPPY;
    const uint8_t b = src[hl];
    if (b < 0x80) {
      if (hl > 9 || (hl == 9 && b > 1)) return PQG_ERR_SNAPPY;
      v |= sft < 64 ? (uint64_t)b << sft : 0;
      hl++;
      break;
    }
    if (sft < 64) v |= (uint64_t)(b & 0x7f) << sft;
  }
  if (v > 0xffffffffull || v > (uint64_t)INT32_MAX) return PQG_ERR_SNAPPY;
  *out_len = (int64_t)v;
  if ((int64_t)v > cap) return PQG_ERR_CAPACITY;
  hipSetDevice(c->device);
  if (c->blk_src.grow((size_t)n + 64) || c->blk_dst.grow((size_t)v + 64) ||
      c->blk_meta.grow(sizeof(JobDev) + sizeof(PageDev) + (4 + 2 * kQueueInts) * sizeof(int)))
    return PQG_ERR_HIP;
  const int64_t bsub = (int64_t)v / kSnapSub + 2, bseg = n / kSnapSeg + 2;
  if (c->blk_subs.grow(sizeof(SnapSub) * (size_t)bsub) || c->blk_segpage.grow(sizeof(int) * (size_t)bseg) ||
      c->blk_F.grow(sizeof(uint2) * 64 * (size_t)bseg))
    return PQG_ERR_HIP;
  JobDev jd;
  memset(&jd, 0, sizeof(jd));
  jd.data = (const uint8_t*)c->blk_src.p;
  jd.data_len = n;
  jd.tcs = n;
  jd.codec = PQG_CODEC_SNAPPY;
  jd.scratch_cap = (int64_t)v + 16;
  PageDev pd;
  memset(&pd, 0, sizeof(pd));
  pd.page_type = PQG_PAGE_DICTIONARY;
  pd.csize = (int32_t)n;
  pd.usize = (int32_t)v;
  pd.payload_offset = 0;
  pd.scratch_offset = 0;
  pd.read_status = kOK;
  uint8_t* meta = (uint8_t*)c->blk_meta.p;
  JobDev* djob = (JobDev*)meta;
  PageDev* dpage = (PageDev*)(meta + sizeof(JobDev));
  int* ints = (int*)(meta + sizeof(JobDev) + sizeof(PageDev));
  int hi[2] = {0, 1};
  if (hipMemcpyAsync(c->blk_src.p, src, (size_t)n, hipMemcpyHostToDevice, c->stream) != hipSuccess ||
      hipMemcpyAsync(djob, &jd, sizeof(jd), hipMemcpyHostToDevice, c->stream) != hipSuccess ||
      hipMemcpyAsync(dpage, &pd, sizeof(pd), hipMemcpyHostToDevice, c->stream) != hipSuccess ||
      hipMemcpyAsync(ints, hi, sizeof(hi), hipMemcpyHostToDevice, c->stream) != hipSuccess ||
      hipMemsetAsync(ints + 4, 0, sizeof(int) * 2 * kQueueInts, c->stream) != hipSuccess)
    return PQG_ERR_HIP;
  const SnapTables T{(SnapSub*)c->blk_subs.p, (int)bsub, (int*)c->blk_segpage.p, (int)bseg, (uint2*)c->blk_F.p};
  launch_snappy(c, c->stream, djob, dpage, ints, ints + 1, 1, ints + 2, ints + 4, ints + 4 + kQueueInts,
                (uint8_t*)c->blk_dst.p, T);
  if (hipGetLastError() != hipSuccess) return PQG_ERR_HIP;
  if (hipMemcpyAsync(&pd, dpage, sizeof(pd), hipMemcpyDeviceToHost, c->stream) != hipSuccess ||
      hipStreamSynchronize(c->stream) != hipSuccess)
    return PQG_ERR_HIP;
  if (pd.read_status != kOK) return pd.read_status;
  if (v && (hipMemcpyAsync(dst, c->blk_dst.p, (size_t)v, hipMemcpyDeviceToHost, c->stream) != hipSuccess ||
            hipStreamSynchronize(c->stream) != hipSuccess))
    return PQG_ERR_HIP;
  return PQG_OK;
}

int pqg_pack_levels(pqg_ctx* c, const uint8_t* levels, int64_t n, int max_level, uint8_t* packed) {
  if (!c || n < 0 || max_level < 0 || max_level > 255 || (n > 0 && (!levels || !packed))) return PQG_ERR_INVALID_ARG;
  hipSetDevice(c->device);
  int bw = 0;
  while ((max_level >> bw) != 0) bw++;
  int e = pqg::pack_levels_launch(c->stream, levels, n, bw, packed);
  if (e) return e;
  return hip_ok(hipStreamSynchronize(c->stream));
}

int pqg_get_pages(pqg_ctx* c, int job, pqg_page_info* out, int cap) {
  if (!c || job < 0 || job >= c->n_jobs) return PQG_ERR_INVALID_ARG;
  hipSetDevice(c->device);
  const JobDev& d = c->h_jobs[job];
  int np = std::min<int>(d.n_out_pages, d.page_cap);
  if (d.status == PQG_ERR_CAPACITY) np = 0;
  std::vector<PageDev> tmp((size_t)np);
  if (np > 0) {
    if (hipMemcpyAsync(tmp.data(), (PageDev*)c->pages.p + d.page_base, sizeof(PageDev) * (size_t)np,
                       hipMemcpyDeviceToHost, c->stream) != hipSuccess ||
        hipStreamSynchronize(c->stream) != hipSuccess)
      return PQG_ERR_HIP;
  }
  int k = 0;
  for (int i = 0; i < np && i < cap; i++, k++) {
    const PageDev& p = tmp[(size_t)i];
    pqg_page_info& o = out[i];
    memset(&o, 0, sizeof(o));
    o.header_offset = p.header_offset;
    o.payload_offset = p.payload_offset;
    o.slot_offset = p.slot_offset;
    o.value_offset = p.value_offset;
    o.page_type = p.page_type;
    o.encoding = p.encoding;
    o.num_values = p.num_values;
    o.not_null = p.not_null;
    o.compressed_size = p.csize;
    o.uncompressed_size = p.usize;
    o.def_len = p.def_len;
    o.rep_len = p.rep_len;
    o.def_encoding = p.def_enc;
    o.rep_encoding = p.rep_enc;
    o.status = p.read_status != PQG_OK ? p.read_status : p.decode_status;
    o.flags = p.flags | (p.sn_fallback ? PQG_PAGE_FLAG_SNAPPY_SERIAL | (p.sn_fallback << 8) : 0);
  }
  return k;
}

int pqg_debug_counters(pqg_ctx* c, uint64_t* out, int cap) {
  if (!c || !out) return PQG_ERR_INVALID_ARG;
#ifdef PQG_PROFILE
  hipSetDevice(c->device);
  hipStreamSynchronize(c->stream);
  unsigned long long a[64], b[64], c3[64], d4[64], e5[64], f6[64];
  if (pqg::prof_read_values(a) || pqg::prof_read_levels(b) || pqg::prof_read_strings(c3) ||
      pqg::prof_read_snappy(d4) || pqg::prof_read_dict(e5) || pqg::prof_read_inflate(f6))
    return PQG_ERR_HIP;
  int k = 0;
  for (; k < 192 && k < cap; k++)
    out[k] = k < 32    ? a[k]
             : k < 64  ? b[k - 32]
             : k < 96  ? c3[k - 64]
             : k < 128 ? d4[k - 96]
             : k < 160 ? e5[k - 128]
                       : f6[k - 160];
  return k;
#else
  return 0;
#endif
}

int pqg_debug_job(pqg_ctx* c, int job, int64_t* out, int cap) {
  if (!c || !out || job < 0 || job >= c->n_jobs) return PQG_ERR_INVALID_ARG;
  const JobDev& d = c->h_jobs[job];
  const int64_t v[5] = {d.scan_fallback, d.n_cands, d.num_pages, d.need_scratch, c->launches};
  int k = 0;
  for (; k < 5 && k < cap; k++) out[k] = v[k];
  return k;
}

int pqg_set_timing(pqg_ctx* c, int on) {
  if (!c) return PQG_ERR_INVALID_ARG;
  c->timed = on != 0;
  return PQG_OK;
}

int pqg_last_timings(pqg_ctx* c, float* out, int cap) {
  if (!c || !out) return PQG_ERR_INVALID_ARG;
  if (!c->last_timed) return 0;
  int k = 0;
  float tot = 0;
  hipEventElapsedTime(&tot, c->ev[0], c->ev[kStages]);
  if (k < cap) out[k++] = tot;
  for (int i = 0; i < kStages && k < cap; i++) {
    float ms = 0;
    hipEventElapsedTime(&ms, c->ev[i], c->ev[i + 1]);
    out[k++] = ms;
  }
  return k;
}

int pqg_bench_decode(pqg_ctx* c, const pqg_chunk_job* jobs, int n_jobs, int iters, float* ms_total, float* ms_stage,
                     int stage_cap) {
  if (!c || iters < 1) return PQG_ERR_INVALID_ARG;
  hipSetDevice(c->device);
  std::vector<pqg_chunk_result> res((size_t)std::max(n_jobs, 1));
  int e = pqg_decode_chunks(c, jobs, n_jobs, res.data());
  if (e) return e;
  for (int i = 0; i < n_jobs; i++) {
    Caps& f = c->force[(size_t)i];
    const JobDev& d = c->h_jobs[i];
    f.pages = d.page_cap;
    f.slots = d.slot_cap;
    f.scratch = d.scratch_cap;
    f.values = d.value_cap;
    f.runs = d.run_cap;
    f.blks = d.blk_cap;
    f.doffs = d.doffs_cap;
  }
  e = plan_batch(c);
  if (e) return e;
  hipEvent_t a, b;
  hipEventCreate(&a);
  hipEventCreate(&b);
  std::vector<float> stage_acc(kStages, 0.f);
  hipEventRecord(a, c->stream);
  for (int it = 0; it < iters; it++) {
    e = launch_pipeline(c);
    if (e) break;
  }
  hipEventRecord(b, c->stream);
  hipStreamSynchronize(c->stream);
  float ms = 0;
  hipEventElapsedTime(&ms, a, b);
  if (ms_total) *ms_total = ms / (float)iters;
  if (ms_stage) {
    for (int i = 0; i < kStages && i < stage_cap; i++) {
      float x = 0;
      hipEventElapsedTime(&x, c->ev[i], c->ev[i + 1]);
      ms_stage[i] = x;
    }
  }
  hipEventDestroy(a);
  hipEventDestroy(b);
  return e;
}

}
```

### parquet-go_amd/csrc/pqg_scan.hip

```cpp
#include <hip/hip_runtime.h>

#include "pqg_common.h"
#include "pqg_device.h"
#include "pqg_thrift.h"

namespace pqg {

struct WinSrc {
  Window w;
  __device__ __forceinline__ int get(int64_t i) { return w.get(i); }
};



__device__ __forceinline__ int classify_page(const JobDev& job, const PageHdr& h, int e, int64_t payload, bool dict_seen,
                             PageDev& pg, int64_t* next, int64_t* comp) {
  *comp = 0;
  *next = payload;
  pg.page_type = h.type;
  pg.encoding = h.encoding;
  pg.num_values = 0;
  pg.csize = h.csize;
  pg.usize = h.usize;
  pg.def_len = h.v2_def_len;
  pg.rep_len = h.v2_rep_len;
  pg.def_enc = h.def_enc;
  pg.rep_enc = h.rep_enc;
  if (e != kOK) return e;
  if (h.type == 2) {
    pg.num_values = h.has_dict ? h.num_values : 0;
    if (dict_seen) e = kDICT_PAGE;
    else if (job.type == 0 || (job.type == 7 && job.type_length < 0)) e = kUNSUPPORTED;
    else if (!h.has_dict || h.num_values < 0) e = kPAGE_HEADER;
    else if (h.encoding != 0 && h.encoding != 2) e = kUNSUPPORTED;
    else if (h.csize < 0 || h.usize < 0) e = kPAGE_HEADER;
    else if (job.data_len - payload < (int64_t)h.csize) e = kSIZE;
    else if (job.codec == 0) { if (h.csize != h.usize) e = kSIZE; }
    else if (job.codec == kCodecSnappy || job.codec == kCodecGzip) *comp = ((int64_t)h.usize + 15) & ~(int64_t)15;
    else e = kUNSUPPORTED;
    *next = payload + h.csize;
    if (e == kOK && job.has_dict_off) *next = job.data_page_offset;
    if (e != kOK) *comp = 0;
  } else if (h.type == 0) {
    pg.num_values = h.has_dph ? h.num_values : 0;
    int enc = h.encoding == 2 ? 8 : h.encoding;
    pg.encoding = enc;
    if (!h.has_dph) e = kPAGE_HEADER;
    else if (job.max_rep > 0 && h.rep_enc != 3) e = kUNSUPPORTED;
    else if (job.max_def > 0 && h.def_enc != 3) e = kUNSUPPORTED;
    else if (h.num_values < 0) e = kPAGE_HEADER;
    else if (h.csize < 0 || h.usize < 0) e = kPAGE_HEADER;
    else if (job.data_len - payload < (int64_t)h.csize) e = kSIZE;
    else if (job.codec == 0 && h.csize != h.usize) e = kSIZE;
    else if (job.codec != 0 && job.codec != kCodecSnappy && job.codec != kCodecGzip) e = kUNSUPPORTED;
    else if (job.codec == 0 && !values_supported(job.type, job.type_length, enc)) e = kUNSUPPORTED;
    if (e == kOK && job.codec != 0) *comp = ((int64_t)h.usize + 15) & ~(int64_t)15;
    *next = payload + h.csize;
  } else if (h.type == 3) {
    pg.num_values = h.has_v2 ? h.num_values : 0;
    int enc = h.encoding == 2 ? 8 : h.encoding;
    pg.encoding = enc;
    int32_t levels = (int32_t)((uint32_t)h.v2_rep_len + (uint32_t)h.v2_def_len);
    int32_t cs = (int32_t)((uint32_t)h.csize - (uint32_t)levels);
    int32_t us = (int32_t)((uint32_t)h.usize - (uint32_t)levels);
    int64_t body = payload + (levels > 0 ? levels : 0);
    if (!h.has_v2) e = kPAGE_HEADER;
    else if (h.num_values < 0 || h.v2_rep_len < 0 || h.v2_def_len < 0) e = kPAGE_HEADER;
    else if (!values_supported(job.type, job.type_length, enc)) e = kUNSUPPORTED;
    else if (levels > 0 && job.data_len - payload < (int64_t)levels) e = kEOF;
    else if (cs < 0 || us < 0) e = kPAGE_HEADER;
    else if (job.data_len - body < (int64_t)cs) e = kSIZE;
    else if (job.codec == 0 && cs != us) e = kSIZE;
    else if (job.codec != 0 && job.codec != kCodecSnappy && job.codec != kCodecGzip) e = kUNSUPPORTED;
    if (e == kOK && job.codec != 0) *comp = ((int64_t)us + 15) & ~(int64_t)15;
    *next = body + cs;
  } else {
    e = kUNSUPPORTED;
  }
  return e;
}

__device__ __forceinline__ void init_page(PageDev& pg, int j, int64_t pos, int64_t payload) {
  pg.header_offset = pos;
  pg.payload_offset = payload;
  pg.slot_offset = 0;
  pg.value_offset = 0;
  pg.scratch_offset = -1;
  pg.block = nullptr;
  pg.block_len = 0;
  pg.rep = pg.def = pg.val = nullptr;
  pg.rep_n = pg.def_n = pg.val_n = 0;
  pg.job = j;
  pg.read_status = kOK;
  pg.decode_status = kOK;
  pg.not_null = 0;
  pg.flags = 0;
  pg.dict_width = 0;
  pg.vmode = -1;
  pg.run_off = pg.blk_off = 0;
  pg.chars = 0;
  pg.char_offset = 0;
}

__device__ __forceinline__ void init_job_results(JobDev& job) {
  job.num_pages = 0;
  job.dict_page = -1;
  job.scan_status = kOK;
  job.need_scratch = 0;
  job.num_slots = 0;
  job.dict_data = nullptr;
  job.dict_count = 0;
  job.dict_len = 0;
  job.dict_offs = nullptr;
  job.need_doffs = 0;
  job.status = kOK;
  job.error_page = -1;
  job.flags = 0;
  job.run_used = 0;
  job.blk_used = 0;
}

constexpr int64_t kCandParseBytes = 1024;
struct CandSrc {
  const PQG_L uint8_t* win;
  int64_t wlo, limit, n;
  bool hit;
  __device__ __forceinline__ int get(int64_t i) {
    if (i >= limit) {
      hit |= i < n;
      return -1;
    }
    return win[i - wlo];
  }
};

__device__ __forceinline__ bool has_byte_15(uint32_t x) {
  uint32_t y = x ^ 0x15151515u;
  return ((y - 0x01010101u) & ~y & 0x80808080u) != 0;
}

constexpr int kCandFrames = 4, kCandLast = 8;
constexpr int kCandSteps = 40;

constexpr int kCandWin = 10;
__device__ __forceinline__ void parse_candidate(const JobDev& job, int64_t p, SkipFrame* frames, int16_t* lasts,
                                             PQG_L uint8_t* win, Cand* out) {
  Compact<CandSrc> c;
  {
    const uintptr_t a0 = (uintptr_t)(job.data + p) & ~(uintptr_t)15;
    const int64_t lo = p - (int64_t)((uintptr_t)(job.data + p) - a0);
    uint4 g[kCandWin];
#pragma unroll
    for (int k = 0; k < kCandWin; k++) g[k] = ldg16(lo + 16 * k < job.data_len ? a0 + 16 * k : a0);
#pragma unroll
    for (int k = 0; k < kCandWin; k++) sts16(win + 16 * k, lo + 16 * k < job.data_len ? g[k] : make_uint4(0, 0, 0, 0));
    const int64_t whi = lo + 16 * kCandWin < job.data_len ? lo + 16 * kCandWin : job.data_len;
    const int64_t lim = p + kCandParseBytes < whi ? p + kCandParseBytes : whi;
    c.src = CandSrc{win, lo, lim, job.data_len, false};
  }
  {
    int64_t q = p + 3;
    int b = 0x80;
    for (int k = 0; k < 5 && (b & 0x80); k++) b = c.src.get(q++);
    if (b < 0 || (b & 0x80) || c.src.get(q) != 0x15) {
      Cand cd;
      cd.pos = p;
      cd.next = p;
      cd.payload = p;
      cd.comp = 0;
      cd.type = cd.encoding = cd.num_values = cd.csize = cd.usize = 0;
      cd.def_len = cd.rep_len = cd.def_enc = cd.rep_enc = 0;
      cd.status = kCOMPLEX;
      *out = cd;
      return;
    }
  }
  c.pos = p;
  c.frames = frames;
  c.last = lasts;
  c.nlast = 0;
  c.last_id = 0;
  c.bool_set = c.bool_val = false;
  c.fcap = kCandFrames;
  c.lcap = kCandLast;
  c.budget = kCandSteps;
  PageHdr h;
  int e = c.read_page_header(&h);
  PageDev pg;
  int64_t next, comp;
  e = classify_page(job, h, e, c.pos, false, pg, &next, &comp);
  if (c.overflow || c.src.hit) e = kCOMPLEX;
  Cand cd;
  cd.pos = p;
  cd.next = next;
  cd.payload = c.pos;
  cd.comp = comp;
  cd.type = pg.page_type;
  cd.encoding = pg.encoding;
  cd.num_values = pg.num_values;
  cd.csize = pg.csize;
  cd.usize = pg.usize;
  cd.def_len = pg.def_len;
  cd.rep_len = pg.rep_len;
  cd.def_enc = pg.def_enc;
  cd.rep_enc = pg.rep_enc;
  cd.status = e;
  *out = cd;
}

__global__ void __launch_bounds__(256) k_tile_jobs(const JobDev* jobs, int* tile_job) {
  const JobDev& job = jobs[blockIdx.x];
  for (int64_t t = threadIdx.x; t < job.n_tiles; t += 256) tile_job[job.tile_base + t] = (int)blockIdx.x;
}

__global__ void __launch_bounds__(256) k_page_cands(JobDev* jobs, const int* tile_job, int* tile_count, int* tile_okc,
                                                    int64_t* cand_pos, int* cand_list, int* cand_total, int region) {
  __shared__ int cnt;
  __shared__ int job_s;
  __shared__ int64_t loc[kCandPerTile];
  const int tid = threadIdx.x;
  const int64_t tile = blockIdx.x;
  if (tid == 0) {
    cnt = 0;
    job_s = tile_job[tile];
  }
  __syncthreads();
  const JobDev& job = jobs[job_s];
  if (job.scan_fallback == 2) {
    if (tid == 0) {
      tile_count[tile] = 0;
      tile_okc[tile] = 0;
    }
    return;
  }
  const int64_t lim = job.tcs < job.data_len ? job.tcs : job.data_len;
  const int64_t t0 = (tile - job.tile_base) * kScanTile;
  const int64_t t1 = t0 + kScanTile < lim ? t0 + kScanTile : lim;
  const gcu8 base = gconst(job.data);
  const int64_t data_len = job.data_len;
  const uintptr_t a0 = (uintptr_t)(base + t0) & ~(uintptr_t)15;
  constexpr int kG = kScanTile / (256 * 16) + 1;
  uint4 vv[kG];
#pragma unroll
  for (int it = 0; it < kG; it++) {
    const uintptr_t a = a0 + (int64_t)tid * 16 + (int64_t)it * 256 * 16;
    const int64_t p0 = (int64_t)(a - (uintptr_t)base);
    vv[it] = ldg16(p0 < t1 ? a : a0);
  }
#pragma unroll
  for (int it = 0; it < kG; it++) {
    const uintptr_t a = a0 + (int64_t)tid * 16 + (int64_t)it * 256 * 16;
    const int64_t p0 = (int64_t)(a - (uintptr_t)base);
    if (p0 >= t1) break;
    const uint4 v = vv[it];
    if (!(has_byte_15(v.x) || has_byte_15(v.y) || has_byte_15(v.z) || has_byte_15(v.w))) continue;
    uint32_t nx = 0xffffu;
    if (((v.w >> 16) & 0xff) == 0x15 || (v.w >> 24) == 0x15) {
      const int64_t q = p0 + 16;
      nx = (q < data_len ? (uint32_t)base[q] : 0xffu) | (q + 1 < data_len ? (uint32_t)base[q + 1] : 0xffu) << 8;
    }
    const uint32_t w5[5] = {v.x, v.y, v.z, v.w, nx};
    uint32_t mask = 0;
#pragma unroll
    for (int k = 0; k < 16; k++) {
      const uint32_t c0 = (w5[k >> 2] >> (8 * (k & 3))) & 0xff;
      const uint32_t c1 = (w5[(k + 1) >> 2] >> (8 * ((k + 1) & 3))) & 0xff;
      const uint32_t c2 = (w5[(k + 2) >> 2] >> (8 * ((k + 2) & 3))) & 0xff;
      mask |= (uint32_t)(c0 == 0x15 && (c1 & 0xf9) == 0 && c2 == 0x15) << k;
    }
    while (mask) {
      const int k = __builtin_ctz(mask);
      mask &= mask - 1;
      const int64_t p = p0 + k;
      if (p < t0 || p >= t1) continue;
      const int slot = atomicAdd(&cnt, 1);
      if (slot < kCandPerTile) loc[slot] = p;
    }
  }
  __syncthreads();
  const int n = cnt;
  if (tid == 0) {
    tile_count[tile] = n > kCandPerTile ? kCandPerTile + 1 : n;
    tile_okc[tile] = 0;
  }
  __shared__ int list_base;
  if (tid == 0 && n > 0 && n <= kCandPerTile) {
    const int sh = (int)(tile & (kQShards - 1));
    list_base = sh * region + atomicAdd(cand_total + sh * kQStride, n);
  }
  __syncthreads();
  if (n <= kCandPerTile && tid < n) {
    const int64_t me = loc[tid];
    int rank = 0;
    for (int k = 0; k < n; k++) rank += loc[k] < me;
    cand_pos[tile * kCandPerTile + rank] = me;
    cand_list[list_base + tid] = (int)(tile * kCandPerTile + rank);
  }
}

__global__ void __launch_bounds__(256) k_cand_parse(JobDev* jobs, const int* tile_job, const int* cand_list,
                                                    const int* cand_total, int region, int* tile_okc,
                                                    const int64_t* cand_pos, Cand* cands) {
  __shared__ SkipFrame frames[256][kCandFrames];
  __shared__ int16_t lasts[256][kCandLast];
  __shared__ __attribute__((aligned(16))) uint8_t wins[256][16 * kCandWin];
  int pre[kQShards + 1];
  pre[0] = 0;
#pragma unroll
  for (int k = 0; k < kQShards; k++) pre[k + 1] = pre[k] + cand_total[k * kQStride];
  const int nc = pre[kQShards];
  for (int i = blockIdx.x * 256 + threadIdx.x; i < nc; i += gridDim.x * 256) {
    int sh = 0;
#pragma unroll
    for (int k = 1; k < kQShards; k++) sh += i >= pre[k];
    const int slot = cand_list[sh * region + (i - pre[sh])];
    const int64_t tile = slot / kCandPerTile;
    const int lo = tile_job[tile];
    Cand* out = &cands[slot];
    parse_candidate(jobs[lo], cand_pos[slot], frames[threadIdx.x], lasts[threadIdx.x], lds_ptr(wins[threadIdx.x]), out);
    if (out->status == kOK) atomicAdd(&tile_okc[tile], 1);
  }
}

__global__ void __launch_bounds__(1024) k_tile_scan(JobDev* jobs, const int* tile_count, const int* tile_okc,
                                                    int* tile_off, int* tile_okoff) {
  __shared__ int64_t part[17];
  __shared__ int ovf;
  JobDev& job = jobs[blockIdx.x];
  const int tid = threadIdx.x;
  if (job.scan_fallback == 2) return;
  if (tid == 0) ovf = 0;
  __syncthreads();
  const int nt = job.n_tiles;
  const int64_t tb = job.tile_base;
  const int seg = (nt + 1023) / 1024;
  const int s0 = tid * seg, s1 = min(nt, s0 + seg);
  int64_t sum = 0, oks = 0;
  bool bad = false;
  for (int t = s0; t < s1; t++) {
    int c = tile_count[tb + t];
    bad |= c > kCandPerTile;
    sum += c;
    oks += tile_okc[tb + t];
  }
  if (bad) ovf = 1;
  int64_t total, ok_total;
  int64_t ex = block_excl_scan<1024>(sum, &total, part);
  int64_t exo = block_excl_scan<1024>(oks, &ok_total, part);
  for (int t = s0; t < s1; t++) {
    tile_off[tb + t] = (int)ex;
    tile_okoff[tb + t] = (int)exo;
    ex += tile_count[tb + t];
    exo += tile_okc[tb + t];
  }
  if (tid == 0) {
    init_job_results(job);
    job.n_cands = (int32_t)min(total, (int64_t)INT32_MAX);
    job.n_ok = (int32_t)min(ok_total, (int64_t)INT32_MAX);
    job.scan_fallback = (ovf || total > INT32_MAX / 2) ? 1 : 0;
    job.brk = INT32_MAX;
    job.first_dict = INT32_MAX;
  }
}

constexpr int kSuccEnd = -1;
constexpr int kSuccTerm = -2;
constexpr int kSuccMissing = -3;
constexpr int kSuccComplex = -4;

__global__ void __launch_bounds__(256) k_cand_link(JobDev* jobs, const int* tile_job, int64_t total_tiles,
                                                   const int* tile_count, const int* tile_off,
                                                   const int* tile_okoff, const Cand* cands, int* succ,
                                                   int* idx2slot, int* ok2slot) {
  const int64_t g = (int64_t)blockIdx.x * 256 + threadIdx.x;
  const int64_t tile = g / kCandPerTile;
  const int s = (int)(g % kCandPerTile);
  if (tile >= total_tiles) return;
  const int cntv = tile_count[tile];
  if (s >= cntv || cntv > kCandPerTile) return;
  JobDev& job = jobs[tile_job[tile]];
  if (job.scan_fallback) return;
  const Cand& cd = cands[tile * kCandPerTile + s];
  const int64_t tb = job.tile_base;
  const int i = tile_off[tile] + s;
  const int slot = (int)((tile - tb) * kCandPerTile + s);
  idx2slot[tb * kCandPerTile + i] = slot;
  const bool ok = cd.status == kOK;
  int okr = 0;
  for (int k = 0; k < s; k++) okr += cands[tile * kCandPerTile + k].status == kOK;
  const int r = tile_okoff[tile] + okr;
  if (ok) ok2slot[tb * kCandPerTile + r] = slot;
  int code;
  bool next_rank = false;
  if (cd.status == kCOMPLEX) code = kSuccComplex;
  else if (!ok) code = kSuccTerm;
  else if (job.tcs - cd.next <= 0) code = kSuccEnd;
  else {
    code = kSuccMissing;
    const int64_t q = cd.next;
    const int64_t lim = job.tcs < job.data_len ? job.tcs : job.data_len;
    if (q >= 0 && q < lim) {
      const int64_t tq = tb + q / kScanTile;
      const int c2 = tile_count[tq];
      const Cand* tc = cands + tq * kCandPerTile;
      int lo2 = 0, hi2 = (c2 < kCandPerTile ? c2 : kCandPerTile) - 1;
      while (lo2 < hi2) {
        int mid = (lo2 + hi2) >> 1;
        if (tc[mid].pos < q) lo2 = mid + 1; else hi2 = mid;
      }
      if (hi2 >= 0 && tc[lo2].pos == q) {
        code = tile_off[tq] + lo2;
        if (tc[lo2].status == kOK) {
          int okt = 0;
          for (int k = 0; k < lo2; k++) okt += tc[k].status == kOK;
          next_rank = tile_okoff[tq] + okt == r + 1;
        }
      }
    }
  }
  succ[tile * kCandPerTile + s] = code;
  if (i == 0 && cd.pos != 0) atomicOr(&job.scan_fallback, 1);
  if (ok && !next_rank) atomicMin(&job.brk, r);
  if (ok && cd.type == 2) atomicMin(&job.first_dict, r);
}

__device__ __forceinline__ bool dict_again(const Cand& c, bool dict_seen) {
  return dict_seen && c.type == 2 && c.status != kTHRIFT;
}

__global__ void __launch_bounds__(1024) k_page_chain(JobDev* jobs, PageDev* pages, const Cand* cands,
                                                     const int* succ, const int* idx2slot, const int* ok2slot,
                                                     int* order) {
  __shared__ int64_t part[17];
  __shared__ int s_n, s_mode, s_cut, s_status, s_dict, s_extra, s_nok;
  const int j = blockIdx.x;
  JobDev& job = jobs[j];
  const int tid = threadIdx.x;
  const int64_t lim = job.tcs < job.data_len ? job.tcs : job.data_len;
  if (job.scan_fallback) return;
  if (job.tcs <= 0) return;
  if (lim <= 0 || job.n_cands == 0) {
    if (tid == 0) job.scan_fallback = 1;
    return;
  }
  const int64_t cb = job.tile_base * kCandPerTile;
  const int* i2s = idx2slot + cb;
  const int* o2s = ok2slot + cb;
  const int b = job.brk;
  const int d1 = job.first_dict;
  const Cand& head = cands[cb + i2s[0]];
  if (tid == 0) {
    s_cut = INT32_MAX;
    s_mode = 0;
    s_dict = -1;
    s_extra = -1;
    s_nok = 0;
  }
  __syncthreads();
  if (head.status == kOK && d1 < b) {
    for (int r = d1 + 1 + tid; r <= b; r += 1024)
      if (cands[cb + o2s[r]].type == 2) atomicMin(&s_cut, r);
  }
  __syncthreads();
  if (tid == 0) {
    int n = 0, mode = 0;
    if (head.status == kCOMPLEX) {
      mode = 2;
    } else if (head.status != kOK) {
      n = 1;
      s_extra = i2s[0];
    } else {
      if (d1 <= b) s_dict = d1;
      if (s_cut != INT32_MAX) {
        n = s_cut + 1;
        s_nok = n;
      } else {
        const int code = succ[cb + o2s[b]];
        s_nok = b + 1;
        n = b + 1;
        if (code == kSuccMissing || code == kSuccComplex) {
          mode = 2;
        } else if (code >= 0) {
          const int ts = i2s[code];
          const Cand& t = cands[cb + ts];
          if (t.status == kCOMPLEX) {
            mode = 2;
          } else if (t.status != kOK) {
            s_extra = ts;
            if (dict_again(t, d1 <= b)) s_cut = n;
            n++;
          } else {
            int* ord = order + job.page_base;
            for (int r = 0; r <= b && r < job.page_cap; r++) ord[r] = o2s[r];
            bool dict_seen = d1 <= b;
            int k = b + 1, cur = code;
            mode = 1;
            for (;;) {
              if (k >= job.page_cap) { mode = 2; break; }
              const int sl = i2s[cur];
              const Cand& cd = cands[cb + sl];
              if (cd.status == kCOMPLEX) { mode = 2; break; }
              ord[k++] = sl;
              if (dict_again(cd, dict_seen)) { s_cut = k - 1; break; }
              if (cd.type == 2 && cd.status == kOK) {
                dict_seen = true;
                s_dict = k - 1;
              }
              const int c2 = succ[cb + sl];
              if (c2 == kSuccEnd || c2 == kSuccTerm) break;
              if (c2 < 0) { mode = 2; break; }
              cur = c2;
            }
            n = k;
          }
        }
      }
    }
    if (mode == 2) job.scan_fallback = 1;
    s_n = n;
    s_mode = mode;
    s_status = kOK;
  }
  __syncthreads();
  if (s_mode == 2) return;
  const int n = s_n, mode = s_mode, cut = s_cut, nok = s_nok, extra = s_extra;
  const int nw = n < job.page_cap ? n : job.page_cap;
  int64_t slot_carry = 0, scratch_carry = 0;
  auto fetch = [&](int k, Cand& c) {
    const int kk = k < n ? k : n - 1;
    const int sl = mode == 1 ? order[job.page_base + kk] : (kk < nok ? o2s[kk] : extra);
    c = cands[cb + sl];
  };
  Cand cur;
  if (n > 0) fetch(tid, cur);
  for (int b0 = 0; b0 < n; b0 += 1024) {
    const int k = b0 + tid;
    int64_t nv = 0, cp = 0;
    int st = kOK;
    if (k < n) {
      st = (k == cut) ? kDICT_PAGE : cur.status;
      cp = (k == cut) ? 0 : cur.comp;
      if ((cur.type == 0 || cur.type == 3) && st == kOK) nv = cur.num_values;
      if (st != kOK) s_status = st;
    }
    int64_t tot_nv, tot_cp;
    const int64_t ex_nv = block_excl_scan<1024>(nv, &tot_nv, part);
    const int64_t ex_cp = block_excl_scan<1024>(cp, &tot_cp, part);
    Cand nxt;
    if (b0 + 1024 < n) fetch(b0 + 1024 + tid, nxt);
    if (k < nw) {
      PageDev pg;
      init_page(pg, j, cur.pos, cur.payload);
      pg.page_type = cur.type;
      pg.encoding = cur.encoding;
      pg.num_values = cur.num_values;
      pg.csize = cur.csize;
      pg.usize = cur.usize;
      pg.def_len = cur.def_len;
      pg.rep_len = cur.rep_len;
      pg.def_enc = cur.def_enc;
      pg.rep_enc = cur.rep_enc;
      pg.read_status = st;
      pg.slot_offset = slot_carry + ex_nv;
      if (cp > 0) pg.scratch_offset = scratch_carry + ex_cp;
      pages[job.page_base + k] = pg;
    }
    slot_carry += tot_nv;
    scratch_carry += tot_cp;
    cur = nxt;
  }
  __syncthreads();
  if (tid == 0) {
    job.num_pages = n;
    job.dict_page = s_dict;
    job.scan_status = s_status;
    job.need_scratch = scratch_carry;
    job.num_slots = slot_carry;
    if (n > job.page_cap || slot_carry > job.slot_cap || scratch_carry > job.scratch_cap) job.status = kCAPACITY;
  }
}

struct ScanShared {
  uint8_t win[kWin];
  SkipFrame frames[kMaxFrames];
  int16_t last[kMaxLast];
  __attribute__((aligned(16))) uint8_t cw[64][16 * kCandWin];
  SkipFrame cf[64][kCandFrames];
  int16_t cl[64][kCandLast];
};

__device__ bool stride_walk(JobDev& job, int j, PageDev* pages, int64_t spos, int64_t slen, int np0, int64_t slots0,
                            int64_t scratch0, ScanShared& sh) {
  const int lane = lane_id();
  const int64_t tcs = job.tcs;
  if (slen <= 0 || tcs - spos <= 0) return false;
  Cand c0;
  parse_candidate(job, spos, sh.cf[lane], sh.cl[lane], lds_ptr(sh.cw[lane]), &c0);
  const int64_t hl = c0.payload - spos;
  if (c0.status != kOK || !(c0.type == 0 || c0.type == 3) || c0.next - spos != slen || hl <= 0 || hl > 64)
    return false;
  const gcu8 base = gconst(job.data);
  constexpr int kHG = 5;
  {
    const uintptr_t a0 = (uintptr_t)(base + spos) & ~(uintptr_t)15;
    const int64_t at = (int64_t)(a0 + 16 * (uintptr_t)lane - (uintptr_t)base);
    const uint4 g = ldg16(lane < kHG && at < job.data_len ? a0 + 16 * lane : a0);
    if (lane < kHG) sts16(lds_ptr(sh.win) + 16 * lane, g);
  }
  __builtin_amdgcn_wave_barrier();
  const uint32_t off0 = (uint32_t)((uintptr_t)(base + spos) & 15);
  const int64_t npages = (tcs - spos + slen - 1) / slen;
  int64_t slots = slots0, scratch = scratch0;
  const int64_t nv0 = c0.num_values, cp0 = c0.comp;
  for (int64_t k0 = 0; k0 < npages; k0 += 64) {
    const int64_t k = k0 + lane;
    const bool live = k < npages;
    const int64_t q = spos + (live ? k : 0) * slen;
    const uintptr_t a = (uintptr_t)(base + q) & ~(uintptr_t)15;
    uint4 g[kHG];
#pragma unroll
    for (int t = 0; t < kHG; t++) {
      const int64_t at = (int64_t)(a + 16 * t - (uintptr_t)base);
      g[t] = ldg16(at < job.data_len ? a + 16 * t : a);
    }
    PQG_L uint32_t* W = (PQG_L uint32_t*)lds_ptr(sh.cw[lane]);
#pragma unroll
    for (int t = 0; t < kHG; t++) sts16((PQG_L uint8_t*)W + 16 * t, g[t]);
    __builtin_amdgcn_wave_barrier();
    const uint32_t offk = (uint32_t)((uintptr_t)(base + q) & 15);
    const PQG_L uint32_t* W0 = (const PQG_L uint32_t*)lds_ptr(sh.win);
    bool same = live;
    for (int i = 0; i < (int)hl; i += 4) {
      const uint32_t ok_ = offk + (uint32_t)i, o0 = off0 + (uint32_t)i;
      const uint32_t x = __builtin_amdgcn_alignbit(W[(ok_ >> 2) + 1], W[ok_ >> 2], (ok_ & 3) * 8);
      const uint32_t y = __builtin_amdgcn_alignbit(W0[(o0 >> 2) + 1], W0[o0 >> 2], (o0 & 3) * 8);
      const int r = (int)hl - i;
      const uint32_t m = r >= 4 ? 0xffffffffu : ((1u << (8 * r)) - 1);
      same &= ((x ^ y) & m) == 0;
    }
    same &= q + hl <= tcs;
    __builtin_amdgcn_wave_barrier();
    const bool lastp = live && k == npages - 1;
    Cand ck = c0;
    bool ok = same;
    if (live && !same) {
      if (lastp) {
        parse_candidate(job, q, sh.cf[lane], sh.cl[lane], lds_ptr(sh.cw[lane]), &ck);
        ok = ck.status == kOK && (ck.type == 0 || ck.type == 3) && ck.next >= tcs;
      }
    } else if (same) {
      ck.pos = q;
      ck.payload = c0.payload + (q - spos);
      ck.next = c0.next + (q - spos);
      ok = ck.next <= job.data_len && (!lastp || ck.next >= tcs);
    }
    const uint64_t lb = __ballot(live), okb = __ballot(live && ok);
    if (okb != lb) return false;
    const int nl = __popcll(lb);
    const bool mine = live;
    const int64_t nv = mine ? ck.num_values : 0, cp = mine ? ck.comp : 0;
    const int64_t inv = (int64_t)wave_incl_scan_u64((uint64_t)nv), icp = (int64_t)wave_incl_scan_u64((uint64_t)cp);
    if (mine && np0 + k < job.page_cap) {
      PageDev pg;
      init_page(pg, j, q, ck.payload);
      pg.page_type = ck.type;
      pg.encoding = ck.encoding;
      pg.num_values = ck.num_values;
      pg.csize = ck.csize;
      pg.usize = ck.usize;
      pg.def_len = ck.def_len;
      pg.rep_len = ck.rep_len;
      pg.def_enc = ck.def_enc;
      pg.rep_enc = ck.rep_enc;
      pg.read_status = kOK;
      pg.slot_offset = slots + inv - nv;
      if (cp > 0) pg.scratch_offset = scratch + icp - cp;
      pages[job.page_base + np0 + k] = pg;
    }
    auto lane64 = [](int64_t v, int l) {
      return (int64_t)((uint64_t)(uint32_t)__builtin_amdgcn_readlane((int)(uint32_t)v, l) |
                       (uint64_t)(uint32_t)__builtin_amdgcn_readlane((int)(uint32_t)((uint64_t)v >> 32), l) << 32);
    };
    slots += lane64(inv, nl - 1);
    scratch += lane64(icp, nl - 1);
  }
  (void)nv0;
  (void)cp0;
  if (lane == 0) {
    const int np = np0 + (int)npages;
    init_job_results(job);
    job.scan_fallback = 2;
    job.num_pages = np;
    job.scan_status = kOK;
    job.need_scratch = scratch;
    job.num_slots = slots;
    if (np > job.page_cap || slots > job.slot_cap || scratch > job.scratch_cap) job.status = kCAPACITY;
  }
  return true;
}

__global__ void __launch_bounds__(64) k_scan_pages(JobDev* jobs, PageDev* pages, int n_jobs, int prewalk, int stride) {
  __shared__ __attribute__((aligned(16))) ScanShared sh;
  int j = blockIdx.x;
  if (j >= n_jobs) return;
  JobDev& job = jobs[j];
  const int64_t tcs = job.tcs;
  if (prewalk > 0) {
    if (job.scan_fallback || tcs <= 0 || job.no_prewalk) return;
    Window win{gconst(job.data), job.data_len, kFarAway, lds_ptr(sh.win)};
    int64_t pos = 0;
    bool dict_seen = false, done = false;
    int64_t spos = -1, slen = 0;
    int snp = 0;
    for (int np = 0;; np++) {
      if (tcs - pos <= 0) {
        done = true;
        break;
      }
      if (np == prewalk) break;
      Compact<WinSrc> c;
      c.src.w = win;
      c.pos = pos;
      c.frames = sh.frames;
      c.last = sh.last;
      c.nlast = 0;
      c.last_id = 0;
      c.bool_set = false;
      c.bool_val = false;
      PageHdr h;
      int e = c.read_page_header(&h);
      win = c.src.w;
      PageDev pg;
      init_page(pg, j, pos, c.pos);
      int64_t next, comp;
      e = classify_page(job, h, e, c.pos, dict_seen, pg, &next, &comp);
      if (e != kOK) {
        done = true;
        break;
      }
      if (h.type != 2 && next - pos < tcs / 8) {
        spos = pos;
        slen = next - pos;
        snp = np;
        break;
      }
      if (h.type == 2) dict_seen = true;
      pos = next;
    }
    if (!done) {
      if (spos < 0 || !stride) return;
      Window w2{gconst(job.data), job.data_len, kFarAway, lds_ptr(sh.win)};
      int64_t p2 = 0, slots = 0, scratch = 0;
      int dict_page = -1;
      bool ds2 = false;
      for (int k = 0; k < snp; k++) {
        Compact<WinSrc> c;
        c.src.w = w2;
        c.pos = p2;
        c.frames = sh.frames;
        c.last = sh.last;
        c.nlast = 0;
        c.last_id = 0;
        c.bool_set = false;
        c.bool_val = false;
        PageHdr h;
        int e = c.read_page_header(&h);
        w2 = c.src.w;
        PageDev pg;
        init_page(pg, j, p2, c.pos);
        pg.slot_offset = slots;
        int64_t next, comp;
        e = classify_page(job, h, e, c.pos, ds2, pg, &next, &comp);
        if (comp > 0) {
          pg.scratch_offset = scratch;
          scratch += comp;
        }
        pg.read_status = e;
        if (k < job.page_cap && lane_id() == 0) pages[job.page_base + k] = pg;
        if (h.type == 0 || h.type == 3) slots += pg.num_values;
        if (h.type == 2) {
          ds2 = true;
          dict_page = k;
        }
        p2 = next;
      }
      if (stride_walk(job, j, pages, spos, slen, snp, slots, scratch, sh) && lane_id() == 0) job.dict_page = dict_page;
      return;
    }
  } else if (job.scan_fallback != 1) {
    return;
  }
  Window win{gconst(job.data), job.data_len, kFarAway, lds_ptr(sh.win)};
  int64_t pos = 0;
  int np = 0;
  int status = kOK;
  bool dict_seen = false;
  int dict_page = -1;
  int64_t scratch = 0;
  int64_t slots = 0;
  const int lane = lane_id();
  while (tcs - pos > 0) {
    Compact<WinSrc> c;
    c.src.w = win;
    c.pos = pos;
    c.frames = sh.frames;
    c.last = sh.last;
    c.nlast = 0;
    c.last_id = 0;
    c.bool_set = false;
    c.bool_val = false;
    PageHdr h;
    int e = c.read_page_header(&h);
    win = c.src.w;
    PageDev pg;
    init_page(pg, j, pos, c.pos);
    pg.slot_offset = slots;
    int64_t next, comp;
    e = classify_page(job, h, e, c.pos, dict_seen, pg, &next, &comp);
    if (comp > 0) {
      pg.scratch_offset = scratch;
      scratch += comp;
    }
    pg.read_status = e;
    if (np < job.page_cap && lane == 0) pages[job.page_base + np] = pg;
    if (h.type == 0 || h.type == 3) slots += (e == kOK) ? pg.num_values : 0;
    if (e == kOK && h.type == 2) {
      dict_seen = true;
      dict_page = np;
    }
    np++;
    if (e != kOK) {
      status = e;
      break;
    }
    pos = next;
  }
  if (lane == 0) {
    init_job_results(job);
    if (prewalk > 0) job.scan_fallback = 2;
    job.num_pages = np;
    job.dict_page = dict_page;
    job.scan_status = status;
    job.need_scratch = scratch;
    job.num_slots = slots;
    if (np > job.page_cap || slots > job.slot_cap || scratch > job.scratch_cap) job.status = kCAPACITY;
  }
}

__global__ void __launch_bounds__(1024) k_page_list(JobDev* jobs, PageDev* pages, int n_jobs, int* list, int list_cap,
                                                    int* total, int* queues) {
  __shared__ int64_t part[17];
  __shared__ int s_off;
  const int j = blockIdx.x;
  auto pages_of = [&](int i) {
    int n = jobs[i].num_pages;
    if (n > jobs[i].page_cap) n = jobs[i].page_cap;
    if (jobs[i].status == kCAPACITY) n = 0;
    return n;
  };
  if (threadIdx.x == 0) {
    int off = 0;
    for (int i = 0; i < j; i++) off += pages_of(i);
    s_off = off;
    if (j == n_jobs - 1) {
      const int all = off + pages_of(j);
      *total = all < list_cap ? all : list_cap;
      for (int q = 0; q < 16; q++) queues[q] = 0;
      for (int q = kCtrItems; q <= kCtrLongWalk; q++) queues[q - 8] = 0;
    }
  }
  __syncthreads();
  const int off = s_off;
  JobDev& job = jobs[j];
  const int n = pages_of(j);
  int64_t rc = 0, bc = 0;
  struct F { int32_t type, usize, csize, nv; int64_t so; };
  auto fetch = [&](int i, F& f) {
    const PageDev& pg = pages[job.page_base + (i < n ? i : n - 1)];
    f.type = pg.page_type;
    f.usize = pg.usize;
    f.csize = pg.csize;
    f.nv = pg.num_values;
    f.so = pg.scratch_offset;
  };
  F cur;
  if (n > 0) fetch((int)threadIdx.x, cur);
  for (int b = 0; b < n; b += 1024) {
    const int i = b + threadIdx.x;
    int64_t nr = 0, nb = 0;
    if (i < n && (cur.type == 0 || cur.type == 3)) {
      const int64_t B = cur.so >= 0 ? (int64_t)(uint32_t)cur.usize : (int64_t)(uint32_t)cur.csize;
      nr = B / 2 + 2;
      nb = (int64_t)(uint32_t)cur.nv / kHBlock + nr / kHBlockRuns + B / (kHBlockBytes / 2) + 3;
    }
    int64_t tr, tb;
    const int64_t er = block_excl_scan<1024>(nr, &tr, part);
    const int64_t eb = block_excl_scan<1024>(nb, &tb, part);
    F nxt;
    if (b + 1024 < n) fetch(b + 1024 + (int)threadIdx.x, nxt);
    if (i < n) {
      if (off + i < list_cap) list[off + i] = (int)(job.page_base + i);
      pages[job.page_base + i].run_off = rc + er;
      pages[job.page_base + i].blk_off = bc + eb;
    }
    rc += tr;
    bc += tb;
    cur = nxt;
  }
  if (threadIdx.x == 0) {
    job.run_used = rc;
    job.blk_used = bc;
    if (rc > job.run_cap || bc > job.blk_cap) job.status = kCAPACITY;
  }
}

}
```

### parquet-go_amd/csrc/pqg_values.hip

```cpp
#include <hip/hip_runtime.h>

#include "pqg_common.h"
#include "pqg_device.h"
#include "pqg_hybrid.h"

namespace pqg {

#ifndef PQG_DBP_WPE
#define PQG_DBP_WPE 4
#endif
#ifndef PQG_VALUES_WPE
#define PQG_VALUES_WPE 1
#endif

#ifdef PQG_PROFILE
int prof_read_values(unsigned long long* out) {
  unsigned long long z[64] = {0};
  if (hipMemcpyFromSymbol(out, HIP_SYMBOL(pqg_prof), sizeof(z)) != hipSuccess) return -1;
  hipMemcpyToSymbol(HIP_SYMBOL(pqg_prof), z, sizeof(z));
  return 0;
}
#endif

template <int W>
struct DictSink {
  gu8 out;
  gcu8 dict;
  int64_t count;
  int64_t bad;
  int64_t nil_key;
  int w;
  bool fast = false;
  uint32_t gv4[kGroup][8];
  __device__ __forceinline__ void prepare(const uint32_t (&v)[kGroup][8], const uint32_t (&i0)[kGroup],
                                          const int (&cnt)[kGroup]) {
    if (W != 4) return;
    uint32_t mx = 0;
#pragma unroll
    for (int b = 0; b < kGroup; b++)
#pragma unroll
      for (int q = 0; q < 8; q++) mx = q < cnt[b] && v[b][q] > mx ? v[b][q] : mx;
    fast = !__ballot((int64_t)mx >= count);
    if (!fast) return;
    const PQG_G uint32_t* d = (const PQG_G uint32_t*)dict;
#ifdef PQG_EXP_NOGATHER
#pragma unroll
    for (int b = 0; b < kGroup; b++)
#pragma unroll
      for (int q = 0; q < 8; q++) gv4[b][q] = v[b][q];
    (void)d;
#else
#pragma unroll
    for (int b = 0; b < kGroup; b++)
#pragma unroll
      for (int q = 0; q < 8; q++) gv4[b][q] = d[q < cnt[b] ? v[b][q] : 0u];
#endif
  }
  __device__ __forceinline__ void group(const uint32_t (&v)[kGroup][8], const uint32_t (&i0)[kGroup],
                                        const int (&cnt)[kGroup]) {
    if (W == 4 && fast) {
#ifdef PQG_EXP_NOSTORE
      uint32_t x = 0;
#pragma unroll
      for (int b = 0; b < kGroup; b++)
#pragma unroll
        for (int q = 0; q < 8; q++) x ^= gv4[b][q];
      if (x == 0x9e3779b9u) *(PQG_G uint32_t*)out = x;
      return;
#endif
#pragma unroll
      for (int b = 0; b < kGroup; b++) {
        if (!__ballot(cnt[b] > 0)) continue;
        const uint32_t v0 = (uint32_t)__builtin_amdgcn_readfirstlane(i0[b]);
        if (count > 65536) store_run_aligned<8, true>((uintptr_t)(out + (int64_t)v0 * 4), gv4[b], cnt[b]);
        else
          store_run_aligned<8>((uintptr_t)(out + (int64_t)v0 * 4), gv4[b], cnt[b]);
      }
      return;
    }
    bool ok[kGroup][8];
#pragma unroll
    for (int b = 0; b < kGroup; b++)
#pragma unroll
      for (int q = 0; q < 8; q++) {
        ok[b][q] = q < cnt[b] && (int64_t)v[b][q] < count;
        if (q < cnt[b] && !ok[b][q]) bad = (int64_t)(i0[b] + q) < bad ? (int64_t)(i0[b] + q) : bad;
      }
    if (W == 4) {
      uint32_t gv[kGroup][8];
      const PQG_G uint32_t* d = (const PQG_G uint32_t*)dict;
#pragma unroll
      for (int b = 0; b < kGroup; b++)
#pragma unroll
        for (int q = 0; q < 8; q++) gv[b][q] = d[ok[b][q] ? v[b][q] : 0u];
#pragma unroll
      for (int b = 0; b < kGroup; b++) {
        if (cnt[b] == 0) continue;
        const uintptr_t o = (uintptr_t)(out + (int64_t)i0[b] * 4);
        if (cnt[b] == 8 && (o & 15) == 0 && ok[b][0] && ok[b][1] && ok[b][2] && ok[b][3] && ok[b][4] && ok[b][5] &&
            ok[b][6] && ok[b][7]) {
          stg16o(o, make_uint4(gv[b][0], gv[b][1], gv[b][2], gv[b][3]));
          stg16o(o + 16, make_uint4(gv[b][4], gv[b][5], gv[b][6], gv[b][7]));
        } else {
#pragma unroll
          for (int q = 0; q < 8; q++)
            if (ok[b][q]) ((PQG_G uint32_t*)o)[q] = gv[b][q];
        }
      }
    } else if (W == 8) {
      u32x2_t gv[kGroup][8];
      const PQG_G u32x2_t* d = (const PQG_G u32x2_t*)dict;
#pragma unroll
      for (int b = 0; b < kGroup; b++)
#pragma unroll
        for (int q = 0; q < 8; q++) gv[b][q] = d[ok[b][q] ? v[b][q] : 0u];
#pragma unroll
      for (int b = 0; b < kGroup; b++) {
        if (cnt[b] == 0) continue;
        const uintptr_t o = (uintptr_t)(out + (int64_t)i0[b] * 8);
#pragma unroll
        for (int q = 0; q < 8; q++)
          if (ok[b][q]) stg8(o + 8 * q, gv[b][q].x, gv[b][q].y);
      }
    } else {
#pragma unroll
      for (int b = 0; b < kGroup; b++)
#pragma unroll
        for (int q = 0; q < 8; q++) {
          if (!ok[b][q]) continue;
          const int64_t key = v[b][q], i = (int64_t)i0[b] + q;
          gcu8 s = dict + key * w;
          for (int c = 0; c < w; c++) out[i * w + c] = (key == nil_key) ? 0 : s[c];
        }
    }
  }
};

struct BoolSink {
  gu8 out;
  __device__ __forceinline__ void prepare(const uint32_t (&)[kGroup][8], const uint32_t (&)[kGroup], const int (&)[kGroup]) {}
  __device__ __forceinline__ void group(const uint32_t (&v)[kGroup][8], const uint32_t (&i0)[kGroup],
                                        const int (&cnt)[kGroup]) {
    for (int b = 0; b < kGroup; b++)
      for (int q = 0; q < cnt[b]; q++) out[i0[b] + q] = v[b][q] == 1;
  }
};

constexpr int kBlocks = 64;
constexpr int kMaxMb = 8;

#ifndef PQG_DBP_STAGE
#define PQG_DBP_STAGE 4096
#endif
constexpr int kDStage = PQG_DBP_STAGE;
struct DbpShared {
  uint8_t stage[kDStage + 32];
  uint8_t win[kWin];
  int64_t body[kBlocks];
  uint64_t mind[kBlocks];
  uint64_t wpk[kBlocks];
  uint32_t sbody[kBlocks];
  uint8_t widths[kBlocks][kMaxMb];
  int64_t mb_off[kBlocks][kMaxMb];
  uint8_t gwidths[256];
  uint64_t gvals[8];
};

__device__ __forceinline__ void dbp_restage(gcu8 s, int64_t n, PQG_L uint8_t* stb, int64_t at, int64_t& st_lo,
                                            int64_t& st_hi) {
  const int lane = lane_id();
  st_lo = at - (int64_t)(((uintptr_t)(s + at)) & 15);
  uint4 g[kDStage / 1024];
  const uintptr_t safe = (uintptr_t)s & ~(uintptr_t)15;
#pragma unroll
  for (int k = 0; k < kDStage / 1024; k++) {
    const int64_t o = st_lo + 16 * (int64_t)(lane + 64 * k);
    g[k] = ldg16((o < n && o + 16 > 0) ? (uintptr_t)(s + o) : safe);
  }
#pragma unroll
  for (int k = 0; k < kDStage / 1024; k++) {
    const int64_t o = st_lo + 16 * (int64_t)(lane + 64 * k);
    sts16(stb + 16 * (lane + 64 * k), (o < n && o + 16 > 0) ? mask_tail(g[k], o, n) : make_uint4(0u, 0u, 0u, 0u));
  }
  st_hi = st_lo + kDStage;
  __builtin_amdgcn_wave_barrier();
}
__device__ __forceinline__ int dbp_st_uvarint(const PQG_L uint8_t* stb, int64_t st_lo, int64_t n, int64_t& q,
                                              uint64_t* out) {
  uint64_t x = 0;
  unsigned sft = 0;
  for (int i = 0;; i++) {
    if (q >= n) return kEOF;
    const uint32_t bt = stb[q - st_lo];
    q++;
    if (bt < 0x80) {
      if (i > 9 || (i == 9 && bt > 1)) return kRLE;
      *out = x | (sft < 64 ? (uint64_t)bt << sft : 0);
      return kOK;
    }
    if (sft < 64) x |= (uint64_t)(bt & 0x7f) << sft;
    sft += 7;
  }
}

__device__ __forceinline__ int dbp_decode_rest(gcu8 s, int64_t n, int64_t readable, bool is64, int64_t nn, gu8 out, DbpShared& sh,
                               int64_t P, int64_t p0, int64_t blk_pos, uint64_t carry, int32_t bs, int32_t mbc,
                               int32_t mbvc, int32_t total, bool pow2, int bs_sh, int mb_sh) {
  const int lane = lane_id();
  const int maxw = is64 ? 64 : 32;
  Window win{s, n, kFarAway, lds_ptr(sh.win)};
  int e;
  bool first_block = true;
  while (p0 < P) {
    int nb = 0;
    int64_t p_end = p0;
    while (nb < kBlocks && p_end < P) {
      int64_t hp = blk_pos;
      uint64_t md;
      if ((e = read_signed(win, hp, is64, &md))) return e;
      if (n - hp < mbc) return kEOF;
      int64_t off = hp + mbc;
      for (int m = 0; m < mbc; m++) {
        int wv = win.get(hp + m);
        if (wv > maxw) return kBIT_WIDTH;
        if (lane == 0) {
          sh.widths[nb][m] = (uint8_t)wv;
          sh.mb_off[nb][m] = off;
        }
        off += (int64_t)(mbvc / 8) * wv;
      }
      int64_t bp0 = p_end;
      int64_t bp1 = bp0 + bs < P ? bp0 + bs : P;
      int64_t last_group_pos = ((bp1 - 1) / 8) * 8;
      int64_t rel = last_group_pos - bp0;
      int m_last = (int)(rel / mbvc);
      int64_t g_in_mb = (rel % mbvc) / 8;
      int wl = win.get(hp + m_last);
      int64_t g_end = 0;
      {
        int64_t mo = hp + mbc;
        for (int m = 0; m < m_last; m++) mo += (int64_t)(mbvc / 8) * win.get(hp + m);
        g_end = mo + (g_in_mb + 1) * wl;
      }
      if (g_end > n) return kEOF;
      if (lane == 0) {
        sh.body[nb] = hp + mbc;
        sh.mind[nb] = md;
      }
      nb++;
      p_end = bp1;
      blk_pos = off;
      first_block = false;
    }
    (void)first_block;
    __builtin_amdgcn_wave_barrier();
    for (int64_t t0 = p0; t0 < p_end; t0 += 256) {
      uint64_t d[4];
      uint64_t local = 0;
      const int64_t pb = t0 + lane * 4;
      const uint32_t rel = (uint32_t)(pb - p0);
      uint32_t b, r2, m, j;
      if (pow2) {
        b = rel >> bs_sh;
        r2 = rel & (uint32_t)(bs - 1);
        m = r2 >> mb_sh;
        j = r2 & (uint32_t)(mbvc - 1);
      } else {
        b = rel / (uint32_t)bs;
        r2 = rel - b * (uint32_t)bs;
        m = r2 / (uint32_t)mbvc;
        j = r2 - m * (uint32_t)mbvc;
      }
      const bool any = pb < p_end;
      const int wv = any ? sh.widths[b][m] : 0;
      const int64_t bit0 = any ? sh.mb_off[b][m] * 8 + (int64_t)j * wv : 0;
      const uint64_t mnd = any ? sh.mind[b] : 0;
#pragma unroll
      for (int k = 0; k < 4; k++) {
        uint64_t dv = 0;
        if (pb + k < p_end) dv = extract_bits64(s, readable, n, bit0 + (int64_t)k * wv, wv) + mnd;
        d[k] = dv;
        local += dv;
      }
      uint64_t incl = wave_incl_scan_u64(local);
      uint64_t run = carry + (incl - local);
      const int nvp = pb >= p_end ? 0 : (p_end - pb >= 4 ? 4 : (int)(p_end - pb));
      if (is64) {
        uint32_t dw[8];
#pragma unroll
        for (int k = 0; k < 4; k++) {
          dw[2 * k] = (uint32_t)run;
          dw[2 * k + 1] = (uint32_t)(run >> 32);
          run += d[k];
        }
        store_run_aligned<8>((uintptr_t)(out + t0 * 8), dw, 2 * nvp);
      } else {
        uint32_t dw[4];
#pragma unroll
        for (int k = 0; k < 4; k++) {
          dw[k] = (uint32_t)run;
          run += d[k];
        }
        store_run_aligned<4>((uintptr_t)(out + t0 * 4), dw, nvp);
      }
      carry += __shfl(incl, 63, 64);
    }
    __builtin_amdgcn_wave_barrier();
    p0 = p_end;
  }
  if (nn > total) return kEOF;
  return kOK;
}

template <bool Full>
__device__ __forceinline__ void store_run64(uintptr_t base, const uint64_t (&v)[4], int nv) {
  const int lane = lane_id();
  const bool shifted = __builtin_amdgcn_readfirstlane((int)(base & 8)) != 0;
  const uintptr_t o = base + 32 * (uintptr_t)lane;
  if (!shifted) {
    if (Full || nv == 4) {
      stg16(o, make_uint4((uint32_t)v[0], (uint32_t)(v[0] >> 32), (uint32_t)v[1], (uint32_t)(v[1] >> 32)));
      stg16(o + 16, make_uint4((uint32_t)v[2], (uint32_t)(v[2] >> 32), (uint32_t)v[3], (uint32_t)(v[3] >> 32)));
    } else {
#pragma unroll
      for (int k = 0; k < 4; k++)
        if (k < nv) stg8(o + 8 * k, (uint32_t)v[k], (uint32_t)(v[k] >> 32));
    }
    return;
  }
  const uint32_t n0 = (uint32_t)__builtin_amdgcn_update_dpp(0, (int)(uint32_t)v[0], 0x130, 0xf, 0xf, true);
  const uint32_t n1 = (uint32_t)__builtin_amdgcn_update_dpp(0, (int)(uint32_t)(v[0] >> 32), 0x130, 0xf, 0xf, true);
  const int nxv = Full ? 4 : __builtin_amdgcn_update_dpp(0, nv, 0x130, 0xf, 0xf, true);
  if (Full ? lane < 63 : (nv == 4 && nxv >= 1)) {
    stg16(o + 8, make_uint4((uint32_t)v[1], (uint32_t)(v[1] >> 32), (uint32_t)v[2], (uint32_t)(v[2] >> 32)));
    stg16(o + 24, make_uint4((uint32_t)v[3], (uint32_t)(v[3] >> 32), n0, n1));
  } else {
#pragma unroll
    for (int k = 1; k < 4; k++)
      if (k < nv) stg8(o + 8 * k, (uint32_t)v[k], (uint32_t)(v[k] >> 32));
    if (nxv >= 1 && (Full || nv == 4) && lane < 63) stg8(o + 32, n0, n1);
  }
  if (lane == 0 && nv >= 1) stg8(o, (uint32_t)v[0], (uint32_t)(v[0] >> 32));
}

template <bool Full>
__device__ __forceinline__ uint64_t dbp_tile(const DbpShared& sh, const PQG_L uint32_t* stw, int64_t t0, int64_t p0,
                                             int64_t p_end, bool pow2, int bs_sh, int mb_sh, int32_t bs, int32_t mbvc,
                                             uint64_t carry, bool is64, gu8 out) {
  const int lane = lane_id();
  const int64_t pb = t0 + lane * 4;
  const int nvp = Full ? 4 : (pb >= p_end ? 0 : (p_end - pb >= 4 ? 4 : (int)(p_end - pb)));
  const uint32_t rl = Full || nvp > 0 ? (uint32_t)(pb - p0) : 0u;
  uint32_t b, r2, m, j;
  if (pow2) {
    b = rl >> bs_sh;
    r2 = rl & (uint32_t)(bs - 1);
    m = r2 >> mb_sh;
    j = r2 & (uint32_t)(mbvc - 1);
  } else {
    b = rl / (uint32_t)bs;
    r2 = rl - b * (uint32_t)bs;
    m = r2 / (uint32_t)mbvc;
    j = r2 - m * (uint32_t)mbvc;
  }
  const PQG_L DbpShared* S = lds_ptr(&sh);
  const uint64_t wpk = S->wpk[b];
  const int wv = (int)(wpk >> (8 * m)) & 0xff;
  uint64_t lw = wpk & ((1ull << (8 * m)) - 1);
  lw = (lw & 0x00ff00ff00ff00ffull) + ((lw >> 8) & 0x00ff00ff00ff00ffull);
  lw += lw >> 16;
  lw += lw >> 32;
  const uint32_t bit0 = (S->sbody[b] + (uint32_t)(mbvc / 8) * ((uint32_t)lw & 0xffff)) * 8 + j * (uint32_t)wv;
  const uint64_t mnd = S->mind[b];
  const uint64_t wmask = wv == 64 ? ~0ull : ((1ull << wv) - 1);
  uint64_t d[4], local = 0;
  if (!__ballot(wv > 32)) {
#pragma unroll
    for (int k = 0; k < 4; k++) {
      const uint32_t bt = bit0 + (uint32_t)(k * wv);
      const uint32_t dw = bt >> 5, sh5 = bt & 31;
      const uint64_t lo = (uint64_t)stw[dw] | ((uint64_t)stw[dw + 1] << 32);
      const uint64_t dv = ((lo >> sh5) & wmask) + mnd;
      d[k] = Full || k < nvp ? dv : 0;
      local += d[k];
    }
  } else {
#pragma unroll
    for (int k = 0; k < 4; k++) {
      const uint32_t bt = bit0 + (uint32_t)(k * wv);
      const uint32_t dw = bt >> 5, sh5 = bt & 31;
      const uint64_t lo = (uint64_t)stw[dw] | ((uint64_t)stw[dw + 1] << 32);
      const uint64_t x = (lo >> sh5) | (((uint64_t)stw[dw + 2] << (63 - sh5)) << 1);
      const uint64_t dv = (x & wmask) + mnd;
      d[k] = Full || k < nvp ? dv : 0;
      local += d[k];
    }
  }
  const uint64_t incl = wave_incl_scan_u64(local);
  uint64_t run = carry + (incl - local);
  if (is64) {
    uint64_t v[4];
#pragma unroll
    for (int k = 0; k < 4; k++) {
      v[k] = run;
      run += d[k];
    }
    store_run64<Full>((uintptr_t)(out + t0 * 8), v, nvp);
  } else {
    uint32_t dw4[4];
#pragma unroll
    for (int k = 0; k < 4; k++) {
      dw4[k] = (uint32_t)run;
      run += d[k];
    }
    store_run_aligned<4>((uintptr_t)(out + t0 * 4), dw4, nvp);
  }
  const uint64_t tot = (uint64_t)(uint32_t)__builtin_amdgcn_readlane((int)(uint32_t)incl, 63) |
                       (uint64_t)(uint32_t)__builtin_amdgcn_readlane((int)(uint32_t)(incl >> 32), 63) << 32;
  return carry + tot;
}

__device__ __forceinline__ int dbp_decode(gcu8 s, int64_t n, int64_t readable, bool is64, int64_t nn, gu8 out,
                          DbpShared& sh, int stage ) {
  const int lane = lane_id();
  Window win{s, n, kFarAway, lds_ptr(sh.win)};
  int64_t pos = 0;
  int32_t bs, mbc, total;
  uint64_t first;
  int e;
  if ((e = read_u32var_delta(win, pos, &bs))) return e;
  if (bs <= 0 && bs % 128 != 0) return kDELTA;
  if ((e = read_u32var_delta(win, pos, &mbc))) return e;
  if (mbc <= 0 || bs % mbc != 0) return kDELTA;
  int32_t mbvc = bs / mbc;
  if (mbvc == 0) return kDELTA;
  if ((e = read_u32var_delta(win, pos, &total))) return e;
  if ((e = read_signed(win, pos, is64, &first))) return e;
  bs = __builtin_amdgcn_readfirstlane(bs);
  mbc = __builtin_amdgcn_readfirstlane(mbc);
  mbvc = __builtin_amdgcn_readfirstlane(mbvc);
  total = __builtin_amdgcn_readfirstlane(total);
  pos = (int64_t)((uint64_t)(uint32_t)__builtin_amdgcn_readfirstlane((int)(uint32_t)pos) |
                  (uint64_t)(uint32_t)__builtin_amdgcn_readfirstlane((int)(uint32_t)((uint64_t)pos >> 32)) << 32);
  first = (uint64_t)(uint32_t)__builtin_amdgcn_readfirstlane((int)(uint32_t)first) |
          (uint64_t)(uint32_t)__builtin_amdgcn_readfirstlane((int)(uint32_t)(first >> 32)) << 32;
  const int maxw = is64 ? 64 : 32;
  {
    int64_t p = pos;
    uint64_t md;
    if ((e = read_signed(win, p, is64, &md))) return e;
    if (n - p < mbc) return kEOF;
    for (int m = 0; m < mbc; m++)
      if (win.get(p + m) > maxw) return kBIT_WIDTH;
  }
  if (stage == 0) return kOK;
  const int64_t P = nn < total ? nn : total;
  const bool regular = (mbvc % 8 == 0) && mbc <= kMaxMb && bs <= (1 << 24);
  const bool pow2 = (bs & (bs - 1)) == 0 && (mbvc & (mbvc - 1)) == 0;
  const int bs_sh = __builtin_ctz((uint32_t)bs), mb_sh = __builtin_ctz((uint32_t)mbvc);
  if (!regular) {
    int64_t rp = pos;
    int32_t cur_mb = mbc;
    uint64_t mind = 0, prev = first;
    uint8_t* widths = sh.gwidths;
    uint64_t* vals = sh.gvals;
    int32_t cw = 0, mbpos = 0;
    for (int k = 0; k < 8; k++) vals[k] = 0;
    {
      if ((e = read_signed(win, rp, is64, &mind))) return e;
      for (int m = 0; m < mbc && m < 256; m++) widths[m] = (uint8_t)win.get(rp + m);
      if (mbc > 256) return kUNSUPPORTED;
      rp += mbc;
      cur_mb = 0;
    }
    for (int64_t p = 0; p < nn; p++) {
      if (p >= total) return kEOF;
      if (p % 8 == 0) {
        if (p % mbvc == 0) {
          if (cur_mb >= mbc) {
            if ((e = read_signed(win, rp, is64, &mind))) return e;
            if (n - rp < mbc) return kEOF;
            for (int m = 0; m < mbc; m++) {
              int wv = win.get(rp + m);
              if (wv > maxw) return kBIT_WIDTH;
              widths[m] = (uint8_t)wv;
            }
            rp += mbc;
            cur_mb = 0;
          }
          cw = widths[cur_mb];
          mbpos = 0;
          cur_mb++;
        }
        if (n - rp < cw) return kEOF;
        for (int k = 0; k < 8; k++) vals[k] = extract_bits64(s, readable, n, rp * 8 + (int64_t)k * cw, cw);
        rp += cw;
        mbpos += cw;
        if (p + 8 >= total) {
          int64_t l = (int64_t)(mbvc / 8) * cw - mbpos;
          if (l < 0) return kDELTA;
          rp += l;
          if (rp > n) rp = n;
        }
      }
      if (lane == 0) {
        if (is64) stg8((uintptr_t)(out + p * 8), (uint32_t)prev, (uint32_t)(prev >> 32));
        else *(PQG_G uint32_t*)(out + p * 4) = (uint32_t)prev;
      }
      prev = prev + vals[p % 8] + mind;
      if (!is64) prev = (uint32_t)prev;
    }
    return kOK;
  }
  uint64_t carry = first;
  int64_t blk_pos = pos;
  int64_t p0 = 0;
  int64_t st_lo = kFarAway, st_hi = kFarAway;
  PQG_L uint8_t* const stb = lds_ptr(sh.stage);
  const PQG_L uint32_t* const stw = (const PQG_L uint32_t*)stb;
  const uint64_t wmask_mbc = mbc >= 8 ? ~0ull : (1ull << (8 * mbc)) - 1;
  const uint64_t wadd = 0x0101010101010101ull * (uint64_t)(127 - maxw);
  const int32_t mb_bytes_per_w = mbvc / 8;
  int64_t spec_len = 0;
#ifdef PQG_PROFILE
  uint64_t pf_rs = 0, pf_walk = 0, pf_tile = 0, pf_nrs = 0, pf_nb = 0;
#define PQG_DBP_RS(...) { PQG_T(ra_); __VA_ARGS__; PQG_T(rb_); pf_rs += rb_ - ra_; pf_nrs++; }
#else
#define PQG_DBP_RS(...) { __VA_ARGS__; }
#endif
  while (p0 < P) {
#ifdef PQG_PROFILE
    PQG_T(tw0_);
    const uint64_t rs0_ = pf_rs;
#endif
    int nb = 0;
    int64_t p_end = p0;
    bool fresh = false;
    while (nb < kBlocks && p_end < P) {
      if (!(blk_pos >= st_lo && blk_pos + 10 + mbc <= st_hi)) {
        if (nb > 0) break;
        PQG_DBP_RS(dbp_restage(s, n, stb, blk_pos, st_lo, st_hi));
        fresh = true;
      }
      if (spec_len > 0) {
        const int64_t q = blk_pos + (int64_t)lane * spec_len;
        bool ok = q + spec_len <= st_hi && q + 10 + mbc <= st_hi && q + spec_len <= n && nb + lane < kBlocks &&
                  p_end + (int64_t)(lane + 1) * bs <= P;
        const uint32_t hr = (uint32_t)((ok ? q : blk_pos) - st_lo);
        uint32_t h[7];
#pragma unroll
        for (int k = 0; k < 7; k++) h[k] = stw[(hr >> 2) + k];
        const uint32_t hs = (hr & 3) * 8;
        uint64_t x0 = (uint64_t)h[0] | (uint64_t)h[1] << 32, x1 = (uint64_t)h[2] | (uint64_t)h[3] << 32;
        const uint64_t x2 = (uint64_t)h[4] | (uint64_t)h[5] << 32;
        if (hs) {
          x0 = (x0 >> hs) | (x1 << (64 - hs));
          x1 = (x1 >> hs) | (x2 << (64 - hs));
        }
        const uint64_t cont = ~x0 & 0x8080808080808080ull;
        ok = ok && cont != 0;
        const int vl = cont ? (int)(__builtin_ctzll(cont) >> 3) + 1 : 1;
        uint64_t t = x0 & 0x7f7f7f7f7f7f7f7full;
        t = (t & 0x007f007f007f007full) | ((t & 0x7f007f007f007f00ull) >> 1);
        t = (t & 0x00003fff00003fffull) | ((t & 0x3fff00003fff0000ull) >> 2);
        t = (t & 0x000000000fffffffull) | ((t & 0x0fffffff00000000ull) >> 4);
        const uint64_t ux = vl == 8 ? t : t & ((1ull << (7 * vl)) - 1);
        int64_t mdv = (int64_t)(ux >> 1);
        if (ux & 1) mdv = ~mdv;
        if (!is64 && (mdv > 2147483647LL || mdv < -2147483648LL)) ok = false;
        const uint32_t vs = (uint32_t)vl * 8;
        uint64_t wpk = vs < 64 ? (x0 >> vs) | (x1 << (64 - vs)) : x1;
        wpk &= wmask_mbc;
        if (((wpk | ((wpk & 0x7f7f7f7f7f7f7f7full) + wadd)) & 0x8080808080808080ull) != 0) ok = false;
        uint64_t sw = (wpk & 0x00ff00ff00ff00ffull) + ((wpk >> 8) & 0x00ff00ff00ff00ffull);
        sw += sw >> 16;
        sw += sw >> 32;
        const int64_t body = q + vl + mbc;
        ok = ok && body + (int64_t)mb_bytes_per_w * (int64_t)((uint32_t)sw & 0xffff) == q + spec_len;
        const uint64_t fail = __ballot(!ok);
        const int k = fail ? __ffsll((long long)fail) - 1 : 64;
        if (k > 0) {
          if (lane < k) {
            sh.mind[nb + lane] = (uint64_t)mdv;
            sh.wpk[nb + lane] = wpk;
            sh.sbody[nb + lane] = (uint32_t)(body - st_lo);
          }
          nb += k;
          p_end += (int64_t)k * bs;
          blk_pos += (int64_t)k * spec_len;
          continue;
        }
      }
      const uint32_t hr = (uint32_t)(blk_pos - st_lo);
      uint32_t h[7];
#pragma unroll
      for (int k = 0; k < 7; k++) h[k] = __builtin_amdgcn_readfirstlane(stw[(hr >> 2) + k]);
      const uint32_t hs = (hr & 3) * 8;
      uint64_t x0 = (uint64_t)h[0] | (uint64_t)h[1] << 32, x1 = (uint64_t)h[2] | (uint64_t)h[3] << 32;
      uint64_t x2 = (uint64_t)h[4] | (uint64_t)h[5] << 32;
      if (hs) {
        x0 = (x0 >> hs) | (x1 << (64 - hs));
        x1 = (x1 >> hs) | (x2 << (64 - hs));
        x2 = (x2 >> hs) | ((uint64_t)h[6] << (64 - hs));
      }
      uint64_t ux = 0;
      int vl = 0;
      const uint64_t cont = ~x0 & 0x8080808080808080ull;
      if (cont) {
        vl = (int)(__builtin_ctzll(cont) >> 3) + 1;
        if (blk_pos + vl > n) return kEOF;
        uint64_t t = x0 & 0x7f7f7f7f7f7f7f7full;
        t = (t & 0x007f007f007f007full) | ((t & 0x7f007f007f007f00ull) >> 1);
        t = (t & 0x00003fff00003fffull) | ((t & 0x3fff00003fff0000ull) >> 2);
        t = (t & 0x000000000fffffffull) | ((t & 0x0fffffff00000000ull) >> 4);
        ux = vl == 8 ? t : t & ((1ull << (7 * vl)) - 1);
      } else {
        for (;; vl++) {
          if (vl == 10) break;
          if (blk_pos + vl >= n) return kEOF;
          const uint32_t bt = (uint32_t)((vl < 8 ? x0 >> (8 * vl) : x1 >> (8 * (vl - 8))) & 0xff);
          if (bt < 0x80) {
            if (vl == 9 && bt > 1) return kDELTA;
            ux |= (uint64_t)bt << (7 * vl);
            vl++;
            break;
          }
          ux |= (uint64_t)(bt & 0x7f) << (7 * vl);
        }
        if (vl == 10 && ((x1 >> 8) & 0x80)) {
          if (nb > 0) break;
          return dbp_decode_rest(s, n, readable, is64, nn, out, sh, P, p0, blk_pos, carry, bs, mbc, mbvc, total,
                                 pow2, bs_sh, mb_sh);
        }
      }
      int64_t mdv = (int64_t)(ux >> 1);
      if (ux & 1) mdv = ~mdv;
      if (!is64 && (mdv > 2147483647LL || mdv < -2147483648LL)) return kDELTA;
      const uint64_t md = (uint64_t)mdv;
      const int64_t hp = blk_pos + vl;
      if (n - hp < mbc) return kEOF;
      const uint32_t vs = (uint32_t)vl * 8;
      uint64_t wpk = vs == 0 ? x0 : vs < 64 ? (x0 >> vs) | (x1 << (64 - vs)) : vs == 64 ? x1
                                                                          : (x1 >> (vs - 64)) | (x2 << (128 - vs));
      wpk &= wmask_mbc;
      if (((wpk | ((wpk & 0x7f7f7f7f7f7f7f7full) + wadd)) & 0x8080808080808080ull) != 0) return kBIT_WIDTH;
      uint64_t sw = (wpk & 0x00ff00ff00ff00ffull) + ((wpk >> 8) & 0x00ff00ff00ff00ffull);
      sw += sw >> 16;
      sw += sw >> 32;
      const uint32_t sumw = (uint32_t)sw & 0xffff;
      const int64_t body = hp + mbc;
      const int64_t off = body + (int64_t)mb_bytes_per_w * sumw;
      const int64_t bp0 = p_end;
      const int64_t bp1 = bp0 + bs < P ? bp0 + bs : P;
      int64_t g_end = off;
      if (bp1 - bp0 < bs) {
        const int64_t rel = ((bp1 - 1) / 8) * 8 - bp0;
        const int m_last = (int)(rel / mbvc);
        const int64_t g_in_mb = (rel % mbvc) / 8;
        int64_t mo = body;
        for (int m = 0; m < m_last; m++) mo += (int64_t)(mbvc / 8) * ((wpk >> (8 * m)) & 0xff);
        g_end = mo + (g_in_mb + 1) * (int64_t)((wpk >> (8 * m_last)) & 0xff);
      }
      if (g_end > n) return kEOF;
      if (g_end > st_hi) {
        if (nb > 0) break;
        if (fresh) return dbp_decode_rest(s, n, readable, is64, nn, out, sh, P, p0, blk_pos, carry, bs, mbc, mbvc,
                                          total, pow2, bs_sh, mb_sh);
        PQG_DBP_RS(dbp_restage(s, n, stb, blk_pos, st_lo, st_hi));
        fresh = true;
        continue;
      }
      if (lane == 0) {
        sh.mind[nb] = md;
        sh.wpk[nb] = wpk;
        sh.sbody[nb] = (uint32_t)(body - st_lo);
      }
      nb++;
      spec_len = bp1 - bp0 == bs ? off - blk_pos : 0;
      p_end = bp1;
      blk_pos = off;
    }
    __builtin_amdgcn_wave_barrier();
#ifdef PQG_PROFILE
    PQG_T(tw1_);
    pf_walk += (tw1_ - tw0_) - (pf_rs - rs0_);
    pf_nb += nb;
#endif
    int64_t t0 = p0;
    for (; t0 + 256 <= p_end; t0 += 256)
      carry = dbp_tile<true>(sh, stw, t0, p0, p_end, pow2, bs_sh, mb_sh, bs, mbvc, carry, is64, out);
    if (t0 < p_end) carry = dbp_tile<false>(sh, stw, t0, p0, p_end, pow2, bs_sh, mb_sh, bs, mbvc, carry, is64, out);
    __builtin_amdgcn_wave_barrier();
#ifdef PQG_PROFILE
    PQG_T(tw2_);
    pf_tile += tw2_ - tw1_;
#endif
    p0 = p_end;
  }
#ifdef PQG_PROFILE
  PQG_ACC(20, 0, pf_walk);
  PQG_ACC(21, 0, pf_rs);
  PQG_ACC(22, 0, pf_tile);
  PQG_ACC(23, 0, pf_nrs);
  PQG_ACC(24, 0, pf_nb);
#endif
#undef PQG_DBP_RS
  if (nn > total) return kEOF;
  return kOK;
}

union ValuesShared {
  ExpandShared ex;
  DbpShared dbp;
};

template <int Mode>
__global__ void __launch_bounds__(64, Mode == 3 ? PQG_DBP_WPE : PQG_VALUES_WPE) k_values(JobDev* jobs, PageDev* pages, const PartRec* parts, const int* total,
                                               int* queue, uint8_t* value_arena, const HStream* streams,
                                               const RunEnt* runs, const BlockDesc* blks) {
  __shared__ __attribute__((aligned(16))) ValuesShared sh;
  const int lane = lane_id();
  if (total[kModePresentOff + Mode] == 0) return;
  const int n_items = min(total[kCtrItems], total[kCtrPartsCap]);
  for (;;) {
    PQG_T(tp0);
    const int t = queue_next(queue);
    if (t >= n_items) return;
    const PartRec pr = parts[t];
    if (pr.vmode != Mode) continue;
    const int pidx = __builtin_amdgcn_readfirstlane(pr.pidx);
    const PageDev pg = pages[pidx];
    if (pg.read_status != kOK || (pg.page_type != 0 && pg.page_type != 3) || pg.vmode != Mode) continue;
    const JobDev job = jobs[pg.job];
    if (job.status == kCAPACITY) continue;
    const bool last = pr.p + 1 >= pr.np;
    const uint32_t nx_v0 = last ? 0u : parts[t + 1].v0;
    const int nx_b0 = last ? -1 : parts[t + 1].b0;
    const gcu8 val = gconst(pg.val);
    const int64_t vn = pg.val_n;
    int64_t readable = (pg.scratch_offset >= 0) ? vn : job.data_len - (pg.val - job.data);
    const int enc = pg.encoding;
    const int64_t nn = pg.not_null;
    const int64_t v_lo = pr.v0, v_hi = last ? nn : (int64_t)nx_v0;
    PQG_T(tpa);
    PQG_ACC(10 + Mode, tp0, tpa);
    const int w = job.value_width;
    const gu8 out = gmut(value_arena) + job.value_base + pg.value_offset * (int64_t)w;
    int re = kOK;
    int dict_w = 0;
    if ((Mode == 0 || Mode == 1) && enc == 8) {
      if (vn < 1) re = kEOF;
      else {
        dict_w = val[0];
        if (dict_w > 32) re = kBIT_WIDTH;
      }
    } else if (Mode == 3 && enc == 5) {
      re = dbp_decode(val, vn, readable, job.type == 2, 0, nullptr, sh.dbp, 0);
    } else if (Mode == 0 && enc == 3 && job.type == 0) {
      if (vn < 4) re = kEOF;
    }
    if (re != kOK) {
      if (lane == 0) pages[pidx].read_status = re;
      continue;
    }
    if (pg.decode_status != kOK || nn == 0) continue;
    int de = kOK;
    if (Mode == 0 && enc == 0) {
      if (job.type == 0) {
        if ((nn + 7) / 8 > vn) de = kEOF;
        else
          for (int64_t i = v_lo + lane; i < v_hi; i += 64) out[i] = (val[i >> 3] >> (i & 7)) & 1;
      } else if (job.type == 3) {
        int64_t full = vn / 12, rem = vn % 12;
        if (nn > full + (rem > 0 ? 1 : 0)) de = kEOF;
        else {
          const int64_t whole = nn < full ? nn : full;
          const int64_t w_hi = v_hi < whole ? v_hi : whole;
          if (nn == full + 1 && rem > 0 && lane == 0 && whole >= v_lo && whole < v_hi) atomicOr(&pages[pidx].flags, 1);
          if (w_hi > v_lo) wave_copy(out + v_lo * 12, val + v_lo * 12, (w_hi - v_lo) * 12);
          if (whole >= v_lo && whole < v_hi && lane < 12) out[whole * 12 + lane] = 0;
        }
      } else if (w > 0) {
        if (nn * w > vn) de = kEOF;
        else wave_copy(out + v_lo * w, val + v_lo * w, (v_hi - v_lo) * w);
      } else {
        de = kUNSUPPORTED;
      }
    } else if ((Mode == 0 || Mode == 1) && enc == 8) {
      const gcu8 dict = gconst(job.dict_data);
      const int64_t dcount = job.dict_data ? job.dict_count : 0;
      const int64_t nil_key = (job.flags & 1) ? dcount - 1 : -1;
      if (w == 0) {
        de = kUNSUPPORTED;
      } else if (dict_w == 0) {
        if (dcount < 1) de = kDICT_INDEX;
        else
          for (int64_t b = lane; b < nn * w; b += 64) out[b] = (0 == nil_key) ? 0 : dict[b % w];
      } else {
        const HStream S = streams[pg.hs_val];
        const int serr = (S.status != kOK && S.produced < nn) ? S.status : kOK;
        int64_t bad = nn;
        const gcu8 dsafe = dict ? dict : (gcu8)out;
        const int blo = pr.b0, bhi = nx_b0;
        if (Mode == 1 || w == 4) {
          DictSink<4> sk{out, dsafe, dcount, nn, nil_key, 4};
          hybrid_expand(S, runs, blks, v_hi, sh.ex, sk, blo, bhi);
          bad = wave_min(sk.bad);
        } else if (Mode == 0 && w == 8) {
          DictSink<8> sk{out, dsafe, dcount, nn, nil_key, 8};
          hybrid_expand(S, runs, blks, v_hi, sh.ex, sk, blo, bhi);
          bad = wave_min(sk.bad);
        } else if (Mode == 0) {
          DictSink<0> sk{out, dsafe, dcount, nn, nil_key, w};
          hybrid_expand(S, runs, blks, v_hi, sh.ex, sk, blo, bhi);
          bad = wave_min(sk.bad);
        }
        if (bad < nn && (serr == kOK || bad < S.produced)) de = kDICT_INDEX;
        else de = serr;
      }
    } else if (Mode == 3 && enc == 5) {
      de = dbp_decode(val, vn, readable, job.type == 2, nn, out, sh.dbp, 1);
    } else if (Mode == 0 && enc == 3 && job.type == 0) {
      const HStream S = streams[pg.hs_val];
      BoolSink sk{out};
      hybrid_expand(S, runs, blks, v_hi, sh.ex, sk, pr.b0, nx_b0);
      de = (S.status != kOK && S.produced < nn) ? S.status : kOK;
    } else {
      de = kUNSUPPORTED;
    }
    if (lane == 0 && de != kOK) atomicMin(&pages[pidx].decode_status, de);
    PQG_T(tp1);
    PQG_ACC(8 + Mode, tp0, tp1);
  }
}

template __global__ void k_values<0>(JobDev*, PageDev*, const PartRec*, const int*, int*, uint8_t*, const HStream*,
                                    const RunEnt*, const BlockDesc*);
template __global__ void k_values<1>(JobDev*, PageDev*, const PartRec*, const int*, int*, uint8_t*, const HStream*,
                                    const RunEnt*, const BlockDesc*);
template __global__ void k_values<3>(JobDev*, PageDev*, const PartRec*, const int*, int*, uint8_t*, const HStream*,
                                    const RunEnt*, const BlockDesc*);

__global__ void __launch_bounds__(1024) k_finalize(JobDev* jobs, int n_jobs, PageDev* pages) {
  __shared__ int s_read, s_dec;
  JobDev& job = jobs[blockIdx.x];
  if (job.status == kCAPACITY) return;
  const int np = job.num_pages < job.page_cap ? job.num_pages : job.page_cap;
  if (threadIdx.x == 0) {
    s_read = INT32_MAX;
    s_dec = INT32_MAX;
  }
  __syncthreads();
  const PageDev* pg = pages + job.page_base;
  int r = INT32_MAX, d = INT32_MAX;
#pragma unroll 8
  for (int i = threadIdx.x; i < np; i += 1024) {
    if (pg[i].read_status != kOK && i < r) r = i;
    if ((pg[i].page_type == 0 || pg[i].page_type == 3) && pg[i].decode_status != kOK && i < d) d = i;
  }
  if (r != INT32_MAX) atomicMin(&s_read, r);
  if (d != INT32_MAX) atomicMin(&s_dec, d);
  __syncthreads();
  if (threadIdx.x != 0) return;
  int status = kOK, ep = -1;
  if (s_read != INT32_MAX) {
    ep = s_read;
    status = pg[ep].read_status;
  }
  job.n_out_pages = ep >= 0 ? ep + 1 : np;
  if (status == kOK && s_dec != INT32_MAX) {
    ep = s_dec;
    status = pg[ep].decode_status;
  }
  job.status = status;
  job.error_page = ep;
}

}
```

Baseline: 1362 GB/s.

## Spread per-job page scans across multiple blocks with two-pass chunk sums

Per-job setup kernels (tile scan, page chain, page list, nn scan, finalize) now launch a 2D grid with several 1024-thread blocks per job, each owning a 1024-page chunk. Chunk totals come from a separate sums kernel or from prefix recomputation, and the last finishing block combines results through atomics. This targets the serial single-block-per-job cost when one column has many pages (about 35k pages here). It adds an extra kernel launch, redundant prefix work, and atomic/fence coordination whose counters must be reset correctly between runs.

Result: faster. 1446 GB/s, median of 6 (+6.2%).

```diff
diff --git a/parquet-go_amd/csrc/pqg_common.h b/parquet-go_amd/csrc/pqg_common.h
--- a/parquet-go_amd/csrc/pqg_common.h
+++ b/parquet-go_amd/csrc/pqg_common.h
@@ -168,8 +168,24 @@
   int64_t blk_cap, blk_base;
   int64_t run_used, blk_used;
   int64_t item_base;
-  int32_t n_items, pad2;
-};
+  int32_t n_items;
+  int32_t second_dict;
+  int32_t fin_read, fin_dec, fin_done, nn_done;
+  unsigned long long nn_acc, parts_acc;
+};
+
+constexpr int kChunkBlock = 1024;
+constexpr int kChunkBlocks = 32;
+struct NnSums {
+  int64_t nn, parts;
+};
+struct NnJob {
+  int64_t base;
+  int64_t res;
+  int32_t cap;
+  int32_t np;
+};
+
 
 constexpr int kSplitMin = 65536;
 constexpr int kPart = 4096;
diff --git a/parquet-go_amd/csrc/pqg_levels.hip b/parquet-go_amd/csrc/pqg_levels.hip
--- a/parquet-go_amd/csrc/pqg_levels.hip
+++ b/parquet-go_amd/csrc/pqg_levels.hip
@@ -492,130 +492,138 @@
 __device__ void plan_parts_from(JobDev& job, int np, const PageDev* pp, const HStream* streams, const BlockDesc* blks,
                                 PartRec* parts, int64_t base);
 
-constexpr int kNnFastSeg = 12;
+__device__ __forceinline__ int nn_pages(const JobDev& job) {
+  const int np = job.num_pages < job.page_cap ? job.num_pages : job.page_cap;
+  return job.status == kCAPACITY ? 0 : np;
+}
+
+__device__ __forceinline__ void nn_page_counts(const PageDev* pp, int i, int np, const HStream* streams, int32_t* nn,
+                                               int32_t* kv, int32_t* vmode) {
+  const PageDev& pg = pp[i < np ? i : np - 1];
+  const int32_t f_type = pg.page_type, f_nn = pg.not_null, f_rs = pg.read_status, f_ds = pg.decode_status,
+                f_enc = pg.encoding, vm = pg.vmode;
+  *nn = *kv = 0;
+  *vmode = vm;
+  if (i >= np) return;
+  const bool data = f_type == 0 || f_type == 3;
+  *nn = data ? f_nn : 0;
+  int32_t k = 0;
+  if (!data || vm < 0) k = 0;
+  else if (f_rs != kOK || f_ds != kOK || vm == 3) k = 1;
+  else if (vm == 2 && f_enc != 0 && f_enc != 8) k = 1;
+  else if (f_nn <= kSplitMin) k = 1;
+  else {
+    int64_t c;
+    bool h;
+    k = (int32_t)part_n(pp[i], streams, &c, &h);
+  }
+  *kv = k;
+}
+
+__global__ void __launch_bounds__(1024) k_nn_scan_sums(JobDev* jobs, PageDev* pages, uint8_t* scratch,
+                                                       const HStream* streams, NnSums* sums, NnJob* njobs, int* ctr,
+                                                       int64_t parts_cap) {
+  __shared__ int64_t part[17];
+  const int j = blockIdx.x, y = blockIdx.y;
+  JobDev& job = jobs[j];
+  const int np = nn_pages(job);
+  const int nblk = (np + kChunkBlock - 1) / kChunkBlock;
+  const bool spread = nblk <= (int)gridDim.y, mine = spread && y < nblk;
+  int64_t ntot = 0, ktot = 0;
+  if (mine) {
+    int32_t nn, kv, vm;
+    nn_page_counts(pages + job.page_base, y * kChunkBlock + (int)threadIdx.x, np, streams, &nn, &kv, &vm);
+    block_excl_scan<1024>(nn, &ntot, part);
+    block_excl_scan<1024>(kv, &ktot, part);
+  }
+  if (threadIdx.x != 0) return;
+  if (mine) {
+    sums[(size_t)j * gridDim.y + y] = NnSums{ntot, ktot};
+    atomicAdd(&job.nn_acc, (unsigned long long)ntot);
+    atomicAdd(&job.parts_acc, (unsigned long long)ktot);
+  }
+  __threadfence();
+  if (atomicAdd(&job.nn_done, 1) != (int)gridDim.y - 1) return;
+  __threadfence();
+  if (j == 0) ctr[kCtrPartsCap] = (int)(parts_cap < INT32_MAX ? parts_cap : INT32_MAX);
+  if (!spread) {
+    njobs[j] = NnJob{0, 0, 0, -1};
+    return;
+  }
+  const int64_t carry = (int64_t)atomicAdd(&job.nn_acc, 0ull), parts_tot = (int64_t)atomicAdd(&job.parts_acc, 0ull);
+  const bool fail0 = job.status == kCAPACITY;
+  int cap = nn_job_tail(job, pages, scratch, np, carry, fail0);
+  int64_t base = 0;
+  if (!cap) {
+    base = atomicAdd(ctr + kCtrItems, (int)parts_tot);
+    if (base + parts_tot > parts_cap) {
+      job.status = kCAPACITY;
+      cap = 1;
+    }
+  }
+  job.item_base = base;
+  job.n_items = cap ? 0 : (int32_t)parts_tot;
+  njobs[j] = NnJob{base, fail0 ? 0 : parts_tot, cap, np};
+}
 
 __global__ void __launch_bounds__(1024) k_nn_scan(JobDev* jobs, PageDev* pages, uint8_t* scratch,
                                                   const HStream* streams, const BlockDesc* blks, int* ctr,
-                                                  PartRec* parts, int64_t parts_cap) {
+                                                  PartRec* parts, int64_t parts_cap, const NnSums* sums,
+                                                  const NnJob* njobs) {
   __shared__ int64_t part[17];
   __shared__ int s_cap;
   JobDev& job = jobs[blockIdx.x];
-  int np = job.num_pages < job.page_cap ? job.num_pages : job.page_cap;
-  if (job.status == kCAPACITY) np = 0;
-  if (np <= kNnFastSeg * 1024) {
-    __shared__ int64_t s_base, s_res;
-    __shared__ int s_big[256];
-    __shared__ int64_t s_boff[256];
+  const int y = blockIdx.y;
+  const NnJob nj = njobs[blockIdx.x];
+  if (nj.np >= 0) {
+    __shared__ int s_big[kChunkBlock];
+    __shared__ int64_t s_boff[kChunkBlock];
     __shared__ int s_nbig;
-    const int seg = (np + 1023) / 1024;
-    const int s0 = (int)threadIdx.x * seg;
+    const int np = nj.np;
+    if (nj.cap) {
+      for (int64_t k = nj.base + (int64_t)y * 1024 + threadIdx.x; k < nj.base + nj.res && k < parts_cap;
+           k += (int64_t)gridDim.y * 1024)
+        parts[k].vmode = -1;
+    }
+    if (y * kChunkBlock >= np) return;
     PageDev* pp = pages + job.page_base;
-    int32_t nnv[kNnFastSeg], kv[kNnFastSeg];
-    int8_t vm[kNnFastSeg];
-    int64_t nsum = 0, ksum = 0;
-    int32_t f_type[kNnFastSeg], f_nn[kNnFastSeg], f_rs[kNnFastSeg], f_ds[kNnFastSeg], f_enc[kNnFastSeg];
-#pragma unroll
-    for (int j = 0; j < kNnFastSeg; j++) {
-      const int i = np > 0 ? (s0 + j < np ? s0 + j : np - 1) : 0;
-      const PageDev& pg = pp[i];
-      f_type[j] = pg.page_type;
-      f_nn[j] = pg.not_null;
-      f_rs[j] = pg.read_status;
-      f_ds[j] = pg.decode_status;
-      f_enc[j] = pg.encoding;
-      vm[j] = (int8_t)pg.vmode;
-    }
-#pragma unroll
-    for (int j = 0; j < kNnFastSeg; j++) {
-      nnv[j] = kv[j] = 0;
-      if (j < seg && s0 + j < np) {
-        const bool data = f_type[j] == 0 || f_type[j] == 3;
-        nnv[j] = data ? f_nn[j] : 0;
-        int32_t k = 0;
-        if (!data || vm[j] < 0) k = 0;
-        else if (f_rs[j] != kOK || f_ds[j] != kOK || vm[j] == 3) k = 1;
-        else if (vm[j] == 2 && f_enc[j] != 0 && f_enc[j] != 8) k = 1;
-        else if (f_nn[j] <= kSplitMin) k = 1;
-        else {
-          int64_t c;
-          bool h;
-          k = (int32_t)part_n(pp[s0 + j], streams, &c, &h);
-        }
-        kv[j] = k;
-      }
-      nsum += nnv[j];
-      ksum += kv[j];
-    }
-    int64_t carry, ktot;
-    int64_t run = block_excl_scan<1024>(nsum, &carry, part);
-    int64_t koff = block_excl_scan<1024>(ksum, &ktot, part);
-    const bool fail0 = job.status == kCAPACITY;
-    if (threadIdx.x == 0) {
-      int cap = nn_job_tail(job, pages, scratch, np, carry, fail0);
-      int64_t base = 0;
-      if (!cap) {
-        base = atomicAdd(ctr + kCtrItems, (int)ktot);
-        if (base + ktot > parts_cap) {
-          job.status = kCAPACITY;
-          cap = 1;
-        }
-      }
-      job.item_base = base;
-      job.n_items = cap ? 0 : (int32_t)ktot;
-      s_base = base;
-      s_cap = cap;
-      s_nbig = 0;
-      s_res = fail0 ? 0 : ktot;
-      if (blockIdx.x == 0) ctr[kCtrPartsCap] = (int)(parts_cap < INT32_MAX ? parts_cap : INT32_MAX);
-    }
+    int64_t run = 0, koff = 0;
+    for (int q = 0; q < y; q++) {
+      const NnSums t = sums[(size_t)blockIdx.x * gridDim.y + q];
+      run += t.nn;
+      koff += t.parts;
+    }
+    const int i = y * kChunkBlock + (int)threadIdx.x;
+    int32_t nn, kv, vm;
+    nn_page_counts(pp, i, np, streams, &nn, &kv, &vm);
+    int64_t tot;
+    run += block_excl_scan<1024>(nn, &tot, part);
+    koff += block_excl_scan<1024>(kv, &tot, part);
+    if (i < np) pp[i].value_offset = run;
+    if (nj.cap) return;
+    if (threadIdx.x == 0) s_nbig = 0;
     __syncthreads();
-    if (s_cap) {
-      for (int64_t k = s_base + threadIdx.x; k < s_base + s_res && k < parts_cap; k += 1024) parts[k].vmode = -1;
-    }
-#pragma unroll
-    for (int j = 0; j < kNnFastSeg; j++)
-      if (j < seg && s0 + j < np) {
-        pp[s0 + j].value_offset = run;
-        run += nnv[j];
-      }
-    if (s_cap) return;
-    const int64_t base = s_base;
-    bool more = false;
-#pragma unroll
-    for (int j = 0; j < kNnFastSeg; j++) {
-      if (j < seg && s0 + j < np) {
-        if (kv[j] == 1) {
-          PartRec r;
-          r.pidx = (int32_t)(job.page_base + s0 + j);
-          r.p = 0;
-          r.np = 1;
-          r.v0 = 0;
-          r.b0 = 0;
-          r.vmode = vm[j];
-          r.chars = r.cstart = r.prel = 0;
-          parts[base + koff] = r;
-        } else if (kv[j] > 1) {
-          const int slot = atomicAdd(&s_nbig, 1);
-          if (slot < 256) {
-            s_big[slot] = s0 + j;
-            s_boff[slot] = koff;
-          } else {
-            more = true;
-          }
-        }
-        koff += kv[j];
-      }
-    }
-    const bool any_more = __syncthreads_or(more);
-    const int nbig = s_nbig < 256 ? s_nbig : 256;
-    if (!any_more) {
-      plan_split_pages(job, pp, streams, blks, parts, base, nbig, s_big, s_boff);
-      return;
+    if (kv == 1) {
+      PartRec r;
+      r.pidx = (int32_t)(job.page_base + i);
+      r.p = 0;
+      r.np = 1;
+      r.v0 = 0;
+      r.b0 = 0;
+      r.vmode = vm;
+      r.chars = r.cstart = r.prel = 0;
+      parts[nj.base + koff] = r;
+    } else if (kv > 1) {
+      const int slot = atomicAdd(&s_nbig, 1);
+      s_big[slot] = i;
+      s_boff[slot] = koff;
     }
     __syncthreads();
-    plan_parts_from(job, np, pp, streams, blks, parts, base);
+    plan_split_pages(job, pp, streams, blks, parts, nj.base, s_nbig, s_big, s_boff);
     return;
   }
+  int np = nn_pages(job);
+  if (y != 0) return;
   const int seg = (np + 1023) / 1024;
   const int s0 = (int)threadIdx.x * seg, s1 = s0 + seg < np ? s0 + seg : np;
   PageDev* pp = pages + job.page_base;
diff --git a/parquet-go_amd/csrc/pqg_runtime.hip b/parquet-go_amd/csrc/pqg_runtime.hip
--- a/parquet-go_amd/csrc/pqg_runtime.hip
+++ b/parquet-go_amd/csrc/pqg_runtime.hip
@@ -60,8 +60,10 @@
 __global__ void k_hybrid_walk(const PageDev* pages, const int* list, const int* total, HStream* streams,
                               RunEnt* runs, BlockDesc* blks, LongWalk* longs, int long_cap);
 __global__ void k_walk_long(const int* ctr, const LongWalk* longs, int long_cap, BlockDesc* blks);
+__global__ void k_nn_scan_sums(JobDev* jobs, PageDev* pages, uint8_t* scratch, const HStream* streams, NnSums* sums,
+                               NnJob* njobs, int* ctr, int64_t parts_cap);
 __global__ void k_nn_scan(JobDev* jobs, PageDev* pages, uint8_t* scratch, const HStream* streams, const BlockDesc* blks,
-                          int* ctr, PartRec* parts, int64_t parts_cap);
+                          int* ctr, PartRec* parts, int64_t parts_cap, const NnSums* sums, const NnJob* njobs);
 template <int Mode>
 __global__ void k_values(JobDev* jobs, PageDev* pages, const PartRec* parts, const int* total, int* queue,
                          uint8_t* value_arena, const HStream* streams, const RunEnt* runs, const BlockDesc* blks);
@@ -71,7 +73,7 @@
 __global__ void k_dict4(PageDev* pages, const int* total, int* queue, const VRec* recs, int big);
 __global__ void k_dict4_big(PageDev* pages, const int* total, int* queue, const VRec* recs);
 constexpr int kBigDictThreads = 512;
-__global__ void k_finalize(JobDev* jobs, int n_jobs, PageDev* pages);
+__global__ void k_finalize(JobDev* jobs, int n_jobs, const PageDev* pages);
 __global__ void k_str_dict(JobDev* jobs, PageDev* pages, int64_t* doffs_arena);
 __global__ void k_str_count(JobDev* jobs, PageDev* pages, PartRec* parts, const int* total, int* queue,
                             int64_t* offs_arena, const HStream* streams, const RunEnt* runs, const BlockDesc* blks);
@@ -187,6 +189,8 @@
   DevBuf parts, lev_long, lev_pieces, walk_long;
   int64_t parts_cap = 0, lev_long_cap = 0, lev_piece_cap = 0, walk_long_cap = 0;
   int64_t total_tiles = 0;
+  DevBuf nn_sums, nn_jobs;
+  int tile_blocks = 1, page_blocks = 1;
   JobDev* h_jobs = nullptr;
   int h_jobs_cap = 0;
   std::vector<pqg_chunk_job> cur;
@@ -299,7 +303,7 @@
                     &c->ok2slot, &c->order, &c->asm_seg, &c->offs_arena, &c->doffs_arena, &c->page_stage,
                     &c->blk_src, &c->blk_dst, &c->blk_meta, &c->tile_job, &c->sn_subs, &c->sn_segpage, &c->sn_F,
                     &c->blk_subs, &c->blk_segpage, &c->blk_F, &c->vrecs, &c->parts, &c->lev_long, &c->lev_pieces,
-                    &c->walk_long})
+                    &c->walk_long, &c->nn_sums, &c->nn_jobs})
     b->release();
   if (c->h_jobs) hipHostFree(c->h_jobs);
   hipStreamDestroy(c->stream);
@@ -449,6 +453,15 @@
       c->doffs_arena.grow(sizeof(int64_t) * (size_t)doffs_total + 64))
     return PQG_ERR_HIP;
   c->total_tiles = tile_total;
+  int64_t max_tiles = 0, max_pages = 0;
+  for (int i = 0; i < n; i++) {
+    max_tiles = std::max<int64_t>(max_tiles, c->plan[(size_t)i].n_tiles);
+    max_pages = std::max<int64_t>(max_pages, c->plan[(size_t)i].page_cap);
+  }
+  c->tile_blocks = (int)std::max<int64_t>(1, (max_tiles + kChunkBlock - 1) / kChunkBlock);
+  c->page_blocks = (int)std::min<int64_t>(kChunkBlocks, std::max<int64_t>(1, (max_pages + kChunkBlock - 1) / kChunkBlock));
+  if (c->nn_sums.grow(sizeof(NnSums) * (size_t)n * (size_t)c->page_blocks) || c->nn_jobs.grow(sizeof(NnJob) * (size_t)n))
+    return PQG_ERR_HIP;
   return hip_ok(hipMemcpyAsync(c->jobs.p, c->h_jobs, sizeof(JobDev) * (size_t)n, hipMemcpyHostToDevice, c->stream));
 }
 
@@ -498,23 +511,24 @@
     int64_t* cpos = (int64_t*)c->cand_pos.p;
     int* clist = (int*)c->cand_list.p;
     const int region = (int)((nt + kQShards - 1) / kQShards) * kCandPerTile;
-    hipLaunchKernelGGL(k_tile_jobs, dim3(n), dim3(256), 0, s, jobs, (int*)c->tile_job.p);
+    hipLaunchKernelGGL(k_tile_jobs, dim3(n, (unsigned)std::min(c->tile_blocks, 64)), dim3(256), 0, s, jobs, (int*)c->tile_job.p);
     hipLaunchKernelGGL(k_page_cands, dim3((unsigned)nt), dim3(256), 0, s, jobs, (const int*)c->tile_job.p, tcount, tokc,
                        cpos, clist, Q(7),
                        region);
     hipLaunchKernelGGL(k_cand_parse, dim3((unsigned)std::min<int64_t>((nt * kCandPerTile + 255) / 256, c->num_cus * 4)),
                        dim3(256), 0, s, jobs, (const int*)c->tile_job.p, clist, Q(7), region, tokc, cpos, cands);
   }
-  hipLaunchKernelGGL(k_tile_scan, dim3(n), dim3(1024), 0, s, jobs, tcount, tokc, toff, tokoff);
+  const dim3 tile_grid(n, (unsigned)c->tile_blocks), page_grid(n, (unsigned)c->page_blocks);
+  hipLaunchKernelGGL(k_tile_scan, tile_grid, dim3(1024), 0, s, jobs, tcount, tokc, toff, tokoff);
   if (nt > 0)
     hipLaunchKernelGGL(k_cand_link, dim3((unsigned)((nt * kCandPerTile + 255) / 256)), dim3(256), 0, s, jobs,
                        (const int*)c->tile_job.p, nt,
                        tcount, toff, tokoff, cands, (int*)c->succ.p, (int*)c->idx2slot.p, (int*)c->ok2slot.p);
-  hipLaunchKernelGGL(k_page_chain, dim3(n), dim3(1024), 0, s, jobs, pages, cands, (const int*)c->succ.p,
+  hipLaunchKernelGGL(k_page_chain, page_grid, dim3(1024), 0, s, jobs, pages, cands, (const int*)c->succ.p,
                      (const int*)c->idx2slot.p, (const int*)c->ok2slot.p, (int*)c->order.p);
   hipLaunchKernelGGL(k_scan_pages, dim3(n), dim3(64), 0, s, jobs, pages, n, 0, 0);
   if (c->timed) hipEventRecord(c->ev[1], s);
-  hipLaunchKernelGGL(k_page_list, dim3(n), dim3(1024), 0, s, jobs, pages, n, list,
+  hipLaunchKernelGGL(k_page_list, page_grid, dim3(1024), 0, s, jobs, pages, n, list,
                      (int)std::min<int64_t>(c->list_cap, INT32_MAX), ctr, ctr + 8);
   if (c->timed) hipEventRecord(c->ev[2], s);
   bool any_snappy = false, any_gzip = false;
@@ -569,7 +583,12 @@
   if (c->timed) hipEventRecord(c->ev[5], s);
   if (c->timed) hipEventRecord(c->ev[6], s);
   PartRec* parts = (PartRec*)c->parts.p;
-  hipLaunchKernelGGL(k_nn_scan, dim3(n), dim3(1024), 0, s, jobs, pages, scratch, streams, blks, ctr, parts, c->parts_cap);
+  NnSums* nsums = (NnSums*)c->nn_sums.p;
+  NnJob* njobs = (NnJob*)c->nn_jobs.p;
+  hipLaunchKernelGGL(k_nn_scan_sums, page_grid, dim3(1024), 0, s, jobs, pages, scratch, streams, nsums, njobs, ctr,
+                     c->parts_cap);
+  hipLaunchKernelGGL(k_nn_scan, page_grid, dim3(1024), 0, s, jobs, pages, scratch, streams, blks, ctr, parts, c->parts_cap,
+                     nsums, njobs);
   if (c->timed) hipEventRecord(c->ev[7], s);
   const int64_t items_cap = c->parts_cap;
   if (!c->any_w4) {
@@ -607,7 +626,7 @@
                        Q(kQueueStrDba), (uint8_t*)c->value_arena.p, offs);
   }
   if (c->timed) hipEventRecord(c->ev[9], s);
-  hipLaunchKernelGGL(k_finalize, dim3(n), dim3(1024), 0, s, jobs, n, pages);
+  hipLaunchKernelGGL(k_finalize, page_grid, dim3(1024), 0, s, jobs, n, pages);
   if (c->timed) hipEventRecord(c->ev[10], s);
   return hip_ok(hipGetLastError());
 }
diff --git a/parquet-go_amd/csrc/pqg_scan.hip b/parquet-go_amd/csrc/pqg_scan.hip
--- a/parquet-go_amd/csrc/pqg_scan.hip
+++ b/parquet-go_amd/csrc/pqg_scan.hip
@@ -210,7 +210,10 @@
 
 __global__ void __launch_bounds__(256) k_tile_jobs(const JobDev* jobs, int* tile_job) {
   const JobDev& job = jobs[blockIdx.x];
-  for (int64_t t = threadIdx.x; t < job.n_tiles; t += 256) tile_job[job.tile_base + t] = (int)blockIdx.x;
+  const int nt = job.n_tiles;
+  const int64_t tb = job.tile_base;
+  for (int64_t t = (int64_t)blockIdx.y * 256 + threadIdx.x; t < nt; t += (int64_t)gridDim.y * 256)
+    tile_job[tb + t] = (int)blockIdx.x;
 }
 
 __global__ void __launch_bounds__(256) k_page_cands(JobDev* jobs, const int* tile_job, int* tile_count, int* tile_okc,
@@ -325,41 +328,50 @@
 __global__ void __launch_bounds__(1024) k_tile_scan(JobDev* jobs, const int* tile_count, const int* tile_okc,
                                                     int* tile_off, int* tile_okoff) {
   __shared__ int64_t part[17];
-  __shared__ int ovf;
   JobDev& job = jobs[blockIdx.x];
   const int tid = threadIdx.x;
   if (job.scan_fallback == 2) return;
-  if (tid == 0) ovf = 0;
-  __syncthreads();
   const int nt = job.n_tiles;
+  const int nblk = (nt + kChunkBlock - 1) / kChunkBlock;
+  const int y = blockIdx.y;
+  if (y >= (nblk > 0 ? nblk : 1)) return;
   const int64_t tb = job.tile_base;
-  const int seg = (nt + 1023) / 1024;
-  const int s0 = tid * seg, s1 = min(nt, s0 + seg);
   int64_t sum = 0, oks = 0;
   bool bad = false;
-  for (int t = s0; t < s1; t++) {
-    int c = tile_count[tb + t];
+  for (int q = 0; q < y; q++) {
+    const int c = tile_count[tb + q * kChunkBlock + tid];
     bad |= c > kCandPerTile;
     sum += c;
-    oks += tile_okc[tb + t];
-  }
-  if (bad) ovf = 1;
-  int64_t total, ok_total;
-  int64_t ex = block_excl_scan<1024>(sum, &total, part);
-  int64_t exo = block_excl_scan<1024>(oks, &ok_total, part);
-  for (int t = s0; t < s1; t++) {
-    tile_off[tb + t] = (int)ex;
-    tile_okoff[tb + t] = (int)exo;
-    ex += tile_count[tb + t];
-    exo += tile_okc[tb + t];
-  }
+    oks += tile_okc[tb + q * kChunkBlock + tid];
+  }
+  const int t = y * kChunkBlock + tid;
+  int c = 0, o = 0;
+  if (t < nt) {
+    c = tile_count[tb + t];
+    o = tile_okc[tb + t];
+    bad |= c > kCandPerTile;
+  }
+  int64_t pre, opre, total, ok_total;
+  block_excl_scan<1024>(sum, &pre, part);
+  block_excl_scan<1024>(oks, &opre, part);
+  const int64_t ex = block_excl_scan<1024>(c, &total, part);
+  const int64_t exo = block_excl_scan<1024>(o, &ok_total, part);
+  if (t < nt) {
+    tile_off[tb + t] = (int)(pre + ex);
+    tile_okoff[tb + t] = (int)(opre + exo);
+  }
+  if (y != (nblk > 0 ? nblk : 1) - 1) return;
+  const int ovf = __syncthreads_or(bad);
   if (tid == 0) {
+    total += pre;
+    ok_total += opre;
     init_job_results(job);
     job.n_cands = (int32_t)min(total, (int64_t)INT32_MAX);
     job.n_ok = (int32_t)min(ok_total, (int64_t)INT32_MAX);
     job.scan_fallback = (ovf || total > INT32_MAX / 2) ? 1 : 0;
     job.brk = INT32_MAX;
     job.first_dict = INT32_MAX;
+    job.second_dict = INT32_MAX;
   }
 }
 
@@ -421,7 +433,10 @@
   succ[tile * kCandPerTile + s] = code;
   if (i == 0 && cd.pos != 0) atomicOr(&job.scan_fallback, 1);
   if (ok && !next_rank) atomicMin(&job.brk, r);
-  if (ok && cd.type == 2) atomicMin(&job.first_dict, r);
+  if (ok && cd.type == 2) {
+    const int was = atomicMin(&job.first_dict, r);
+    if (was != INT32_MAX) atomicMin(&job.second_dict, was > r ? was : r);
+  }
 }
 
 __device__ __forceinline__ bool dict_again(const Cand& c, bool dict_seen) {
@@ -433,49 +448,67 @@
                                                      int* order) {
   __shared__ int64_t part[17];
   __shared__ int s_n, s_mode, s_cut, s_status, s_dict, s_extra, s_nok;
-  const int j = blockIdx.x;
+  const int j = blockIdx.x, y = blockIdx.y;
   JobDev& job = jobs[j];
   const int tid = threadIdx.x;
-  const int64_t lim = job.tcs < job.data_len ? job.tcs : job.data_len;
-  if (job.scan_fallback) return;
-  if (job.tcs <= 0) return;
-  if (lim <= 0 || job.n_cands == 0) {
+  const int64_t tcs = job.tcs, data_len = job.data_len, tile_base = job.tile_base, page_base = job.page_base;
+  const int n_cands = job.n_cands, n_ok = job.n_ok, b = job.brk, d1 = job.first_dict, d2 = job.second_dict,
+            page_cap = job.page_cap;
+  const int64_t lim = tcs < data_len ? tcs : data_len;
+  if (tid == 0) s_mode = job.scan_fallback;
+  __syncthreads();
+  const bool fb = s_mode != 0;
+  __syncthreads();
+  if (fb) return;
+  if (tcs <= 0) return;
+  if (lim <= 0 || n_cands == 0) {
     if (tid == 0) job.scan_fallback = 1;
     return;
   }
-  const int64_t cb = job.tile_base * kCandPerTile;
+  const int64_t cb = tile_base * kCandPerTile;
   const int* i2s = idx2slot + cb;
   const int* o2s = ok2slot + cb;
-  const int b = job.brk;
-  const int d1 = job.first_dict;
-  const Cand& head = cands[cb + i2s[0]];
+  if ((int64_t)y * kChunkBlock > n_ok) return;
+  Cand spec;
+  const int slot0 = i2s[0];
+  const int slotb = (n_ok > 0 && b >= 0 && b < n_ok) ? o2s[b] : slot0;
+  {
+    const int k = y * kChunkBlock + tid;
+    spec = cands[cb + (n_ok > 0 ? o2s[k < n_ok ? k : n_ok - 1] : slot0)];
+  }
+  const int codeb = succ[cb + slotb];
+  int64_t slot_carry = 0, scratch_carry = 0;
+  if (y > 0) {
+    int64_t nv = 0, cp = 0;
+    for (int q = tid; q < y * kChunkBlock; q += kChunkBlock) {
+      const Cand& c = cands[cb + o2s[q]];
+      const int32_t ty = c.type, cs = c.status, cnv = c.num_values;
+      cp += c.comp;
+      if ((ty == 0 || ty == 3) && cs == kOK) nv += cnv;
+    }
+    block_excl_scan<1024>(nv, &slot_carry, part);
+    block_excl_scan<1024>(cp, &scratch_carry, part);
+  }
+  const Cand& head = cands[cb + slot0];
   if (tid == 0) {
-    s_cut = INT32_MAX;
+    s_cut = (head.status == kOK && d2 <= b) ? d2 : INT32_MAX;
     s_mode = 0;
     s_dict = -1;
     s_extra = -1;
     s_nok = 0;
-  }
-  __syncthreads();
-  if (head.status == kOK && d1 < b) {
-    for (int r = d1 + 1 + tid; r <= b; r += 1024)
-      if (cands[cb + o2s[r]].type == 2) atomicMin(&s_cut, r);
-  }
-  __syncthreads();
-  if (tid == 0) {
     int n = 0, mode = 0;
     if (head.status == kCOMPLEX) {
       mode = 2;
     } else if (head.status != kOK) {
       n = 1;
-      s_extra = i2s[0];
+      s_extra = slot0;
     } else {
       if (d1 <= b) s_dict = d1;
       if (s_cut != INT32_MAX) {
         n = s_cut + 1;
         s_nok = n;
       } else {
-        const int code = succ[cb + o2s[b]];
+        const int code = codeb;
         s_nok = b + 1;
         n = b + 1;
         if (code == kSuccMissing || code == kSuccComplex) {
@@ -490,13 +523,13 @@
             if (dict_again(t, d1 <= b)) s_cut = n;
             n++;
           } else {
-            int* ord = order + job.page_base;
-            for (int r = 0; r <= b && r < job.page_cap; r++) ord[r] = o2s[r];
+            mode = y == 0 ? 1 : 3;
+            int* ord = order + page_base;
+            for (int r = 0; mode == 1 && r <= b && r < page_cap; r++) ord[r] = o2s[r];
             bool dict_seen = d1 <= b;
             int k = b + 1, cur = code;
-            mode = 1;
-            for (;;) {
-              if (k >= job.page_cap) { mode = 2; break; }
+            while (mode == 1) {
+              if (k >= page_cap) { mode = 2; break; }
               const int sl = i2s[cur];
               const Cand& cd = cands[cb + sl];
               if (cd.status == kCOMPLEX) { mode = 2; break; }
@@ -522,18 +555,21 @@
     s_status = kOK;
   }
   __syncthreads();
-  if (s_mode == 2) return;
+  if (s_mode >= 2) return;
   const int n = s_n, mode = s_mode, cut = s_cut, nok = s_nok, extra = s_extra;
-  const int nw = n < job.page_cap ? n : job.page_cap;
-  int64_t slot_carry = 0, scratch_carry = 0;
+  const int nw = n < page_cap ? n : page_cap;
+  const int nblk = (n + kChunkBlock - 1) / kChunkBlock;
+  const bool spread = mode == 0 && nblk <= (int)gridDim.y;
+  if (spread ? y >= nblk : y != 0) return;
+  const int r0 = spread ? y * kChunkBlock : 0, r1 = spread ? min(n, r0 + kChunkBlock) : n;
   auto fetch = [&](int k, Cand& c) {
     const int kk = k < n ? k : n - 1;
-    const int sl = mode == 1 ? order[job.page_base + kk] : (kk < nok ? o2s[kk] : extra);
+    const int sl = mode == 1 ? order[page_base + kk] : (kk < nok ? o2s[kk] : extra);
     c = cands[cb + sl];
   };
-  Cand cur;
-  if (n > 0) fetch(tid, cur);
-  for (int b0 = 0; b0 < n; b0 += 1024) {
+  Cand cur = spec;
+  if (mode == 1 || min(r0 + tid, n - 1) >= nok) fetch(r0 + tid, cur);
+  for (int b0 = r0; b0 < r1; b0 += 1024) {
     const int k = b0 + tid;
     int64_t nv = 0, cp = 0;
     int st = kOK;
@@ -547,7 +583,7 @@
     const int64_t ex_nv = block_excl_scan<1024>(nv, &tot_nv, part);
     const int64_t ex_cp = block_excl_scan<1024>(cp, &tot_cp, part);
     Cand nxt;
-    if (b0 + 1024 < n) fetch(b0 + 1024 + tid, nxt);
+    if (b0 + 1024 < r1) fetch(b0 + 1024 + tid, nxt);
     if (k < nw) {
       PageDev pg;
       init_page(pg, j, cur.pos, cur.payload);
@@ -563,20 +599,20 @@
       pg.read_status = st;
       pg.slot_offset = slot_carry + ex_nv;
       if (cp > 0) pg.scratch_offset = scratch_carry + ex_cp;
-      pages[job.page_base + k] = pg;
+      pages[page_base + k] = pg;
     }
     slot_carry += tot_nv;
     scratch_carry += tot_cp;
     cur = nxt;
   }
   __syncthreads();
-  if (tid == 0) {
+  if (tid == 0 && r1 == n) {
     job.num_pages = n;
     job.dict_page = s_dict;
     job.scan_status = s_status;
     job.need_scratch = scratch_carry;
     job.num_slots = slot_carry;
-    if (n > job.page_cap || slot_carry > job.slot_cap || scratch_carry > job.scratch_cap) job.status = kCAPACITY;
+    if (n > page_cap || slot_carry > job.slot_cap || scratch_carry > job.scratch_cap) job.status = kCAPACITY;
   }
 }
 
@@ -850,19 +886,60 @@
 __global__ void __launch_bounds__(1024) k_page_list(JobDev* jobs, PageDev* pages, int n_jobs, int* list, int list_cap,
                                                     int* total, int* queues) {
   __shared__ int64_t part[17];
-  __shared__ int s_off;
-  const int j = blockIdx.x;
+  __shared__ int s_off, s_n;
+  const int j = blockIdx.x, y = blockIdx.y;
+  JobDev& job = jobs[j];
+  const int np0 = job.num_pages < job.page_cap ? job.num_pages : job.page_cap;
+  if (y > 0 && (int64_t)y * kChunkBlock >= np0) return;
+  struct F { int32_t type, usize, csize, nv; int64_t so; };
+  auto fetch = [&](int i, F& f) {
+    const PageDev& pg = pages[job.page_base + (i < np0 ? i : (np0 > 0 ? np0 - 1 : 0))];
+    f.type = pg.page_type;
+    f.usize = pg.usize;
+    f.csize = pg.csize;
+    f.nv = pg.num_values;
+    f.so = pg.scratch_offset;
+  };
+  auto bounds = [](const F& f, int64_t* nr, int64_t* nb) {
+    *nr = *nb = 0;
+    if (f.type == 0 || f.type == 3) {
+      const int64_t B = f.so >= 0 ? (int64_t)(uint32_t)f.usize : (int64_t)(uint32_t)f.csize;
+      *nr = B / 2 + 2;
+      *nb = (int64_t)(uint32_t)f.nv / kHBlock + *nr / kHBlockRuns + B / (kHBlockBytes / 2) + 3;
+    }
+  };
+  F cur;
+  fetch(y * kChunkBlock + (int)threadIdx.x, cur);
+  int64_t rc = 0, bc = 0;
+  if (y > 0) {
+    for (int q = threadIdx.x; q < y * kChunkBlock; q += kChunkBlock) {
+      F f;
+      fetch(q, f);
+      int64_t nr, nb;
+      bounds(f, &nr, &nb);
+      rc += nr;
+      bc += nb;
+    }
+    int64_t tot;
+    block_excl_scan<1024>(rc, &tot, part);
+    rc = tot;
+    block_excl_scan<1024>(bc, &tot, part);
+    bc = tot;
+  }
   auto pages_of = [&](int i) {
     int n = jobs[i].num_pages;
     if (n > jobs[i].page_cap) n = jobs[i].page_cap;
     if (jobs[i].status == kCAPACITY) n = 0;
     return n;
   };
+  int64_t before = 0, before_tot;
+  for (int i = threadIdx.x; i < j; i += kChunkBlock) before += pages_of(i);
+  block_excl_scan<1024>(before, &before_tot, part);
   if (threadIdx.x == 0) {
-    int off = 0;
-    for (int i = 0; i < j; i++) off += pages_of(i);
+    const int off = (int)before_tot;
     s_off = off;
-    if (j == n_jobs - 1) {
+    s_n = pages_of(j);
+    if (j == n_jobs - 1 && y == 0) {
       const int all = off + pages_of(j);
       *total = all < list_cap ? all : list_cap;
       for (int q = 0; q < 16; q++) queues[q] = 0;
@@ -871,33 +948,20 @@
   }
   __syncthreads();
   const int off = s_off;
-  JobDev& job = jobs[j];
-  const int n = pages_of(j);
-  int64_t rc = 0, bc = 0;
-  struct F { int32_t type, usize, csize, nv; int64_t so; };
-  auto fetch = [&](int i, F& f) {
-    const PageDev& pg = pages[job.page_base + (i < n ? i : n - 1)];
-    f.type = pg.page_type;
-    f.usize = pg.usize;
-    f.csize = pg.csize;
-    f.nv = pg.num_values;
-    f.so = pg.scratch_offset;
-  };
-  F cur;
-  if (n > 0) fetch((int)threadIdx.x, cur);
-  for (int b = 0; b < n; b += 1024) {
+  const int n = s_n;
+  const int nblk = (n + kChunkBlock - 1) / kChunkBlock;
+  const bool spread = nblk <= (int)gridDim.y;
+  if (spread ? y >= (nblk > 0 ? nblk : 1) : y != 0) return;
+  const int r0 = spread ? y * kChunkBlock : 0, r1 = spread ? min(n, r0 + kChunkBlock) : n;
+  for (int b = r0; b < r1; b += 1024) {
     const int i = b + threadIdx.x;
     int64_t nr = 0, nb = 0;
-    if (i < n && (cur.type == 0 || cur.type == 3)) {
-      const int64_t B = cur.so >= 0 ? (int64_t)(uint32_t)cur.usize : (int64_t)(uint32_t)cur.csize;
-      nr = B / 2 + 2;
-      nb = (int64_t)(uint32_t)cur.nv / kHBlock + nr / kHBlockRuns + B / (kHBlockBytes / 2) + 3;
-    }
+    if (i < n) bounds(cur, &nr, &nb);
     int64_t tr, tb;
     const int64_t er = block_excl_scan<1024>(nr, &tr, part);
     const int64_t eb = block_excl_scan<1024>(nb, &tb, part);
     F nxt;
-    if (b + 1024 < n) fetch(b + 1024 + (int)threadIdx.x, nxt);
+    if (b + 1024 < r1) fetch(b + 1024 + (int)threadIdx.x, nxt);
     if (i < n) {
       if (off + i < list_cap) list[off + i] = (int)(job.page_base + i);
       pages[job.page_base + i].run_off = rc + er;
@@ -907,9 +971,12 @@
     bc += tb;
     cur = nxt;
   }
-  if (threadIdx.x == 0) {
-    job.run_used = rc;
-    job.blk_used = bc;
+  if (threadIdx.x == 0 && r1 == n) {
+    job.fin_read = job.fin_dec = INT32_MAX;
+    job.fin_done = job.nn_done = 0;
+    job.nn_acc = job.parts_acc = 0;
+    atomicMax((unsigned long long*)&job.run_used, (unsigned long long)rc);
+    atomicMax((unsigned long long*)&job.blk_used, (unsigned long long)bc);
     if (rc > job.run_cap || bc > job.blk_cap) job.status = kCAPACITY;
   }
 }
diff --git a/parquet-go_amd/csrc/pqg_values.hip b/parquet-go_amd/csrc/pqg_values.hip
--- a/parquet-go_amd/csrc/pqg_values.hip
+++ b/parquet-go_amd/csrc/pqg_values.hip
@@ -841,7 +841,7 @@
 template __global__ void k_values<3>(JobDev*, PageDev*, const PartRec*, const int*, int*, uint8_t*, const HStream*,
                                     const RunEnt*, const BlockDesc*);
 
-__global__ void __launch_bounds__(1024) k_finalize(JobDev* jobs, int n_jobs, PageDev* pages) {
+__global__ void __launch_bounds__(1024) k_finalize(JobDev* jobs, int n_jobs, const PageDev* pages) {
   __shared__ int s_read, s_dec;
   JobDev& job = jobs[blockIdx.x];
   if (job.status == kCAPACITY) return;
@@ -854,7 +854,7 @@
   const PageDev* pg = pages + job.page_base;
   int r = INT32_MAX, d = INT32_MAX;
 #pragma unroll 8
-  for (int i = threadIdx.x; i < np; i += 1024) {
+  for (int i = blockIdx.y * 1024 + threadIdx.x; i < np; i += gridDim.y * 1024) {
     if (pg[i].read_status != kOK && i < r) r = i;
     if ((pg[i].page_type == 0 || pg[i].page_type == 3) && pg[i].decode_status != kOK && i < d) d = i;
   }
@@ -862,14 +862,20 @@
   if (d != INT32_MAX) atomicMin(&s_dec, d);
   __syncthreads();
   if (threadIdx.x != 0) return;
+  if (s_read != INT32_MAX) atomicMin(&job.fin_read, s_read);
+  if (s_dec != INT32_MAX) atomicMin(&job.fin_dec, s_dec);
+  __threadfence();
+  if (atomicAdd(&job.fin_done, 1) != (int)gridDim.y - 1) return;
+  __threadfence();
+  const int f_read = atomicMin(&job.fin_read, INT32_MAX), f_dec = atomicMin(&job.fin_dec, INT32_MAX);
   int status = kOK, ep = -1;
-  if (s_read != INT32_MAX) {
-    ep = s_read;
+  if (f_read != INT32_MAX) {
+    ep = f_read;
     status = pg[ep].read_status;
   }
   job.n_out_pages = ep >= 0 ? ep + 1 : np;
-  if (status == kOK && s_dec != INT32_MAX) {
-    ep = s_dec;
+  if (status == kOK && f_dec != INT32_MAX) {
+    ep = f_dec;
     status = pg[ep].decode_status;
   }
   job.status = status;
```
